# ekinakyurek/Long-Term-Recurrent-Convolutional-NN

Measured on AMD Instinct MI355X. Metric: training images/sec (VGG16+LSTM, COCO, batch 256) at 1/2/4/8 MI355X, higher is better.
Workload: dtype bf16

## Files before the change

### long-term-recurrent-convolutional-nn_amd/csrc/gemm.h

```cpp
#pragma once
#include <hip/hip_runtime.h>
#include <stdint.h>

enum { GEMM_A_PLAIN = 0, GEMM_A_CONV3 = 1 };
enum { GEMM_OUT_PLAIN = 0, GEMM_OUT_CONV = 1, GEMM_OUT_POOL = 2, GEMM_OUT_LSTM_FWD = 3, GEMM_OUT_LSTM_BWD = 4, GEMM_OUT_SMAX_TOPK = 5,
       GEMM_OUT_SMAX_GUMBEL = 6, GEMM_OUT_SMAX_PICK = 7 };

enum { SMAX_KC = 6, SMAX_REC = 16 };
enum { SMAX_MAX_NREC = 256 };
struct SmaxEpi {
    float *part;
    int nrec;
    float temp;
    uint32_t key0, key1;
    int current, S;
    const int32_t *tgt;
};

struct LstmEpi {
    int H;
    int64_t ld_a, ld_h;
    const float *Gx;
    const float *c_prev;
    const int *c_prev_idx;
    const float *c_new;
    float *c_out;
    void *acts;
    void *h_new;
    int gx_bcast;
    const int *gx_idx;
    float *h_f32;
    const float *dh_ext;
    float *dc;
    void *dz_out;
};
enum { GEMM_T_F32 = 0, GEMM_T_BF16 = 1, GEMM_T_F8 = 2 };

struct GemmArgs {
    int dtype;
    const void *A;
    int64_t lda;
    const void *B;
    int64_t ldb;
    void *C;
    int64_t ldc;
    int M, N, K;
    const float *bias;
    const float *scale;
    int c_f32;
    int beta;
    int c_is_zero;
    int relu;
    int a_mode, out_mode;
    int H, W, Cin;
    unsigned inv_w2, inv_h2;
    int wg_cap;
    LstmEpi lstm;
    SmaxEpi smax;
    int cfg_pref;
    int free_cus;
    int bg_cus;
    int *tile_ctr;
    unsigned long long *stamps;
    int splitk_forced;
    int splitk_no_reduce;
    int deterministic;
    int dbg;
    const void *zero_page;
    void *ws;
    size_t ws_bytes;
};

constexpr int kBgMinRows = 256, kBgMaxRows = 512;
inline bool bg_row_window(int rows) { return rows >= kBgMinRows && rows <= kBgMaxRows; }

hipError_t launch_gemm(hipStream_t stream, const GemmArgs &g);
hipError_t launch_gemm_nt(hipStream_t stream, const GemmArgs &g);

void gemm_debug_note_route(const char *route, int cfg);
const char *gemm_debug_last_route();

bool gemm_glds_eligible(const GemmArgs &g);
hipError_t launch_gemm_glds(hipStream_t stream, const GemmArgs &g);
int64_t gemm_glds_blocks(const GemmArgs &g);

int gemm_8p_config(const GemmArgs &g, int64_t *blocks);
int gemm_8p_splitk(const GemmArgs &g, int64_t *blocks);
hipError_t launch_gemm_8p(hipStream_t stream, const GemmArgs &g, int splitk = 1);
hipError_t launch_splitk_reduce(hipStream_t stream, const GemmArgs &g, int splits);

bool gemm_skinny_eligible(const GemmArgs &g);
hipError_t launch_gemm_skinny(hipStream_t stream, const GemmArgs &g);

bool conv64_eligible(int dtype, int Cin, int Cout, int H, int W);
hipError_t launch_conv64(hipStream_t stream, const void *in, const void *w, const float *bias, void *out, int N, int H, int W, int Cout,
                         int relu, int pool, const void *zero_page, float f8_inv_scale = 0.0f, int wg_cap = 0, unsigned long long *stamps = nullptr);
hipError_t launch_conv64_fused11(hipStream_t stream, const void *img16, const void *w11, const float *b11, const void *w,
                                 const float *bias, void *out, int N, int S, const void *zero_page, int wg_cap = 0, unsigned long long *stamps = nullptr);
hipError_t launch_conv64f(hipStream_t stream, const void *img16, const void *w11, const void *w, const float *bias, void *out, int N, int S,
                          const void *zero_page, int wg_cap = 0, unsigned long long *stamps = nullptr);
```

### long-term-recurrent-convolutional-nn_amd/csrc/gemm_8p.hip

```cpp
#include <type_traits>

#include "common.h"
#include "gemm.h"
#include "knob.h"
#include "philox.h"

namespace {

typedef __attribute__((address_space(3))) void lds_void;
typedef const __attribute__((address_space(1))) void glb_void;
typedef float f32x4v __attribute__((ext_vector_type(4)));

template <int N> __device__ __forceinline__ void wait_vmcnt() { asm volatile("s_waitcnt vmcnt(%0)" ::"n"(N) : "memory"); }
__device__ __forceinline__ void wait_lgkm0() { asm volatile("s_waitcnt lgkmcnt(0)" ::: "memory"); }

struct KStep {
    int tap, koff, kb;
};

template <int I, int N, class F> __device__ __forceinline__ void static_for(F &&f) {
    if constexpr (I < N) {
        f(std::integral_constant<int, I>{});
        static_for<I + 1, N>(f);
    }
}
template <int OFF> __device__ __forceinline__ uint4 lds_read16(unsigned addr) {
    uint4 r;
    asm volatile("ds_read_b128 %0, %1 offset:%2" : "=v"(r) : "v"(addr), "n"(OFF) : "memory");
    return r;
}

typedef int i32x8v __attribute__((ext_vector_type(8)));
__device__ __forceinline__ i32x8v pack8(const uint4 &lo, const uint4 &hi) {
    return i32x8v{(int)lo.x, (int)lo.y, (int)lo.z, (int)lo.w, (int)hi.x, (int)hi.y, (int)hi.z, (int)hi.w};
}
__device__ __forceinline__ unsigned pack_fp8x4(float a, float b, float c, float d) {
    a = fminf(fmaxf(a, -448.f), 448.f); b = fminf(fmaxf(b, -448.f), 448.f);
    c = fminf(fmaxf(c, -448.f), 448.f); d = fminf(fmaxf(d, -448.f), 448.f);
    unsigned w = 0;
    w = __builtin_amdgcn_cvt_pk_fp8_f32(a, b, w, false);
    w = __builtin_amdgcn_cvt_pk_fp8_f32(c, d, w, true);
    return w;
}

__device__ __forceinline__ float relu_bits(float x, int lo) {
    const int b = __builtin_bit_cast(int, x);
    return __builtin_bit_cast(float, b > lo ? b : lo);
}
__device__ __forceinline__ float sigm8p(float x) { return 1.0f / (1.0f + expf(-x)); }

template <int APW, int BPW> struct TileAddr {
    int m0, n0;
    unsigned a_voff[2][APW];
    unsigned a_mask[2][APW];
    unsigned b_voff[2][BPW];
};

template <int WM, int WN, int MT, int NT, int AMODE, bool SWAP, bool F8, int EPI = 0>
__device__ __forceinline__ bool gemm8p_tile(const GemmArgs &g, unsigned char *smem, const int tile, const int ntiles_xy, const int next_tile,
                                            TileAddr<WM * (2 * MT * 16) / 128, WN * (2 * NT * 16) / 128> &ta, const bool pre) {
    constexpr int ES = F8 ? 1 : 2;
    constexpr int KE = 128 / ES;
    static_assert(WM * WN == 8, "8 waves");
    constexpr int QM = MT * 16, QN = NT * 16;
    constexpr int WTM = 2 * QM, WTN = 2 * QN;
    constexpr int BM = WM * WTM, BN = WN * WTN;
    constexpr int A_BYTES = BM * 128, B_BYTES = BN * 128, BUF = A_BYTES + B_BYTES;
    constexpr int APW = BM / 128, BPW = BN / 128;
    static_assert(APW >= 1 && BPW >= 1 && APW * 128 == BM && BPW * 128 == BN, "tile must be a multiple of 128");
    constexpr int CPR = BN / 8;
    static_assert(CPR >= 16, "epilogue swizzle needs >= 16 chunks per row");
    const int tid = threadIdx.x, lane = tid & 63;
    const int wave = __builtin_amdgcn_readfirstlane(tid >> 6);
    const int wr = wave / WN, wc = wave % WN;
    const int grp = wave >> 2;
    auto stamp = [&](int k) {
        if (g.stamps && tid == 0) g.stamps[(size_t)tile * 8 + k] = k >= 6 ? __builtin_amdgcn_s_memrealtime() : __builtin_amdgcn_s_memtime();
    };
    stamp(7);
    stamp(0);
    const int M = g.M, N = g.N;
    const int tiles_n = (N + BN - 1) / BN;

    constexpr unsigned OOB = 0xFFFFFFFFu, NREC = 0xFFFFFF00u;
    const unsigned conv_back = (AMODE == GEMM_A_CONV3) ? (unsigned)((g.W + 1) * g.Cin * ES) : 0u;
    const unsigned char *Abase = reinterpret_cast<const unsigned char *>(g.A) - conv_back;
    const unsigned char *Bbase = reinterpret_cast<const unsigned char *>(g.B);
    auto rsrc_of = [](const unsigned char *base, bool live) {
        return __builtin_amdgcn_make_buffer_rsrc(const_cast<unsigned char *>(base), 0, live ? NREC : 0u, 0x00020000);
    };

    const int kpt = (AMODE == GEMM_A_CONV3) ? g.Cin / KE : g.K / KE;
    const int KT_all = (AMODE == GEMM_A_CONV3) ? 9 * kpt : kpt;
    const int kbeg = (int)((int64_t)KT_all * blockIdx.y / gridDim.y);
    const int KT = (int)((int64_t)KT_all * (blockIdx.y + 1) / gridDim.y) - kbeg;

    auto a_piece_row = [&](int hf, int j) {
        const int hr = (wave * APW + j) * 8;
        return (hr / QM) * WTM + hf * QM + (hr % QM);
    };
    auto b_piece_row = [&](int hf, int j) {
        const int hr = (wave * BPW + j) * 8;
        return (hr / QN) * WTN + hf * QN + (hr % QN);
    };
    auto setup = [&](int t, TileAddr<APW, BPW> &o) {
        int bid = t;
        {
            const int nwg = ntiles_xy, q = nwg >> 3, r = nwg & 7, xcd = bid & 7;
            bid = (xcd < r ? xcd * (q + 1) : r * (q + 1) + (xcd - r) * q) + (bid >> 3);
        }
        const int nt = bid % tiles_n, mt = bid / tiles_n;
        o.m0 = mt * BM;
        o.n0 = nt * BN;
#pragma unroll
        for (int hf = 0; hf < 2; ++hf) {
#pragma unroll
            for (int j = 0; j < APW; ++j) {
                const int row = a_piece_row(hf, j) + (lane >> 3);
                const int m = o.m0 + row;
                const int src_chunk = (lane & 7) ^ ((row >> 1) & 7);
                o.a_voff[hf][j] = OOB;
                o.a_mask[hf][j] = ~0u;
                if (m < M) {
                    if (AMODE == GEMM_A_CONV3) {
                        const PixDecode p = decode_pixel_fast(m, g.H, g.W, g.inv_w2, g.inv_h2);
                        o.a_voff[hf][j] = (unsigned)((uint64_t)((p.n * g.H + p.y) * g.W + p.x) * (uint64_t)(g.Cin * ES) + src_chunk * 16);
                        o.a_mask[hf][j] = (p.y == 0 ? 0x007u : 0u) | (p.y == g.H - 1 ? 0x1C0u : 0u) | (p.x == 0 ? 0x049u : 0u) |
                                          (p.x == g.W - 1 ? 0x124u : 0u) | ~0x1FFu;
                    } else {
                        o.a_voff[hf][j] = (unsigned)((uint64_t)m * (uint64_t)(g.lda * ES) + src_chunk * 16);
                    }
                }
            }
#pragma unroll
            for (int j = 0; j < BPW; ++j) {
                const int row = b_piece_row(hf, j) + (lane >> 3);
                const int n = o.n0 + row;
                const int src_chunk = (lane & 7) ^ ((row >> 1) & 7);
                o.b_voff[hf][j] = n < N ? (unsigned)((uint64_t)n * (uint64_t)(g.ldb * ES) + src_chunk * 16) : OOB;
            }
        }
    };

    auto kstep_of = [&](int kt) {
        KStep k;
        if (AMODE == GEMM_A_CONV3) {
            const int slice = kt / 9;
            k.tap = kt - 9 * slice;
            const int kh = k.tap / 3, kw = k.tap - 3 * kh;
            k.koff = ((kh - 1) * g.W + (kw - 1)) * g.Cin + slice * KE;
            k.kb = k.tap * g.Cin + slice * KE;
        } else {
            k.tap = 0;
            k.koff = kt * KE;
            k.kb = k.koff;
        }
        return k;
    };
    const unsigned char *Aflat = reinterpret_cast<const unsigned char *>(g.A);
    const unsigned char *Zp = reinterpret_cast<const unsigned char *>(g.zero_page) + (lane & 7) * 16;
    auto stage_a = [&](int buf, int hf, const KStep &k, bool live) {
        if constexpr (AMODE == GEMM_A_CONV3) {
            const __amdgpu_buffer_rsrc_t rs = rsrc_of(Abase, live);
            const int soff = (int)(conv_back + (unsigned)(k.koff * ES));
#pragma unroll
            for (int j = 0; j < APW; ++j) {
                const unsigned vo = ta.a_voff[hf][j] | (unsigned)__builtin_amdgcn_sbfe((int)ta.a_mask[hf][j], k.tap, 1);
                __builtin_amdgcn_raw_ptr_buffer_load_lds(rs, (lds_void *)(smem + buf * BUF + a_piece_row(hf, j) * 128), 16, (int)vo, soff, 0, 0);
            }
        } else {
#pragma unroll
            for (int j = 0; j < APW; ++j) {
                const bool ok = live && ta.a_voff[hf][j] != OOB;
                const unsigned char *src = ok ? Aflat + ((int64_t)ta.a_voff[hf][j] + (int64_t)k.koff * ES) : Zp;
                __builtin_amdgcn_global_load_lds((glb_void *)src, (lds_void *)(smem + buf * BUF + a_piece_row(hf, j) * 128), 16, 0, 0);
            }
        }
    };
    auto stage_b = [&](int buf, int hf, const KStep &k, bool live) {
        if constexpr (AMODE == GEMM_A_CONV3) {
            const __amdgpu_buffer_rsrc_t rs = rsrc_of(Bbase, live);
            const int soff = k.kb * ES;
#pragma unroll
            for (int j = 0; j < BPW; ++j)
                __builtin_amdgcn_raw_ptr_buffer_load_lds(rs, (lds_void *)(smem + buf * BUF + A_BYTES + b_piece_row(hf, j) * 128), 16,
                                                         (int)ta.b_voff[hf][j], soff, 0, 0);
        } else {
#pragma unroll
            for (int j = 0; j < BPW; ++j) {
                const bool ok = live && ta.b_voff[hf][j] != OOB;
                const unsigned char *src = ok ? Bbase + ((int64_t)ta.b_voff[hf][j] + (int64_t)k.kb * ES) : Zp;
                __builtin_amdgcn_global_load_lds((glb_void *)src, (lds_void *)(smem + buf * BUF + A_BYTES + b_piece_row(hf, j) * 128), 16, 0, 0);
            }
        }
    };

    unsigned fa[2], fb[2];
#pragma unroll
    for (int s = 0; s < 2; ++s) {
        const int kch = F8 ? 2 * (lane >> 4) + s : s * 4 + (lane >> 4);
        const unsigned fo = (lane & 15) * 128 + ((kch ^ (((lane & 15) >> 1) & 7)) << 4);
        const unsigned base = (unsigned)(uintptr_t)(__attribute__((address_space(3))) unsigned char *)smem;
        fa[s] = base + (wr * WTM) * 128 + fo;
        fb[s] = base + A_BYTES + (wc * WTN) * 128 + fo;
    }

    auto issue_first = [&]() {
        const KStep k0 = kstep_of(kbeg);
        stage_a(0, 0, k0, true);
        stage_b(0, 0, k0, true);
        stage_b(0, 1, k0, true);
        stage_a(0, 1, k0, true);
    };
    if (!pre) {
        setup(tile, ta);
        issue_first();
    }
    stamp(1);
    const int m0 = ta.m0, n0 = ta.n0;

    const bool staged = !F8 && EPI == 0 && !g.c_f32 && !g.beta && gridDim.y == 1 && (g.ldc % 8) == 0 && ((uintptr_t)g.C & 15) == 0 &&
                        (N % 8) == 0 && (!SWAP || (N % 4) == 0);
    const bool bias_init = staged && g.bias != nullptr;
    f32x4v acc[2][MT][2][NT];
#pragma unroll
    for (int b = 0; b < 2; ++b)
#pragma unroll
        for (int n = 0; n < NT; ++n) {
            f32x4v bv = f32x4v{0.f, 0.f, 0.f, 0.f};
            if (bias_init) {
                if constexpr (SWAP) {
                    const int col = n0 + wc * WTN + b * QN + n * 16 + (lane >> 4) * 4;
                    if (col < N) bv = *reinterpret_cast<const f32x4v *>(g.bias + col);
                } else {
                    const int col = n0 + wc * WTN + b * QN + n * 16 + (lane & 15);
                    const float sb = col < N ? g.bias[col] : 0.0f;
                    bv = f32x4v{sb, sb, sb, sb};
                }
            }
#pragma unroll
            for (int a = 0; a < 2; ++a)
#pragma unroll
                for (int i = 0; i < MT; ++i) acc[a][i][b][n] = bv;
        }

    uint4 af[MT][2], bf0[NT][2], bf1[NT][2];
    auto read_a = [&](int buf, auto mhc) {
        constexpr int mh = decltype(mhc)::value;
        const unsigned a0 = fa[0] + buf * BUF, a1 = fa[1] + buf * BUF;
        static_for<0, MT>([&](auto ic) {
            constexpr int i = decltype(ic)::value;
            af[i][0] = lds_read16<(mh * QM + i * 16) * 128>(a0);
            af[i][1] = lds_read16<(mh * QM + i * 16) * 128>(a1);
        });
    };
    auto read_b = [&](int buf, auto nhc, uint4 (&bf)[NT][2]) {
        constexpr int nh = decltype(nhc)::value;
        const unsigned b0 = fb[0] + buf * BUF, b1 = fb[1] + buf * BUF;
        static_for<0, NT>([&](auto ic) {
            constexpr int n = decltype(ic)::value;
            bf[n][0] = lds_read16<(nh * QN + n * 16) * 128>(b0);
            bf[n][1] = lds_read16<(nh * QN + n * 16) * 128>(b1);
        });
    };
    constexpr std::integral_constant<int, 0> I0{};
    constexpr std::integral_constant<int, 1> I1{};
#define MFMA_BODY(mh, nh, BF)                                                                                              \
    do {                                                                                                                   \
        if constexpr (F8) {                                                                                                \
            _Pragma("unroll") for (int i = 0; i < MT; ++i) _Pragma("unroll") for (int n = 0; n < NT; ++n) {                \
                const i32x8v av = pack8(af[i][0], af[i][1]);                                                               \
                const i32x8v bv = pack8(BF[n][0], BF[n][1]);                                                               \
                acc[mh][i][nh][n] = SWAP ? __builtin_amdgcn_mfma_scale_f32_16x16x128_f8f6f4(bv, av, acc[mh][i][nh][n], 0, 0, 0, 0, 0, 0) \
                                         : __builtin_amdgcn_mfma_scale_f32_16x16x128_f8f6f4(av, bv, acc[mh][i][nh][n], 0, 0, 0, 0, 0, 0); \
            }                                                                                                              \
        } else {                                                                                                           \
            _Pragma("unroll") for (int s = 0; s < 2; ++s) _Pragma("unroll") for (int i = 0; i < MT; ++i) _Pragma("unroll") for (int n = 0; \
                                                                                                                   n < NT; ++n) { \
                const bf16x8 av = __builtin_bit_cast(bf16x8, af[i][s]);                                                    \
                const bf16x8 bv = __builtin_bit_cast(bf16x8, BF[n][s]);                                                    \
                acc[mh][i][nh][n] = SWAP ? __builtin_amdgcn_mfma_f32_16x16x32_bf16(bv, av, acc[mh][i][nh][n], 0, 0, 0)     \
                                         : __builtin_amdgcn_mfma_f32_16x16x32_bf16(av, bv, acc[mh][i][nh][n], 0, 0, 0);    \
            }                                                                                                              \
        }                                                                                                                  \
    } while (0)
#define MFMA_PAIR(mh1, nh1, BF1, mh2, nh2, BF2, LGKM1)                                                                     \
    do {                                                                                                                   \
        __builtin_amdgcn_s_barrier();                                                                                      \
        asm volatile("s_waitcnt lgkmcnt(%0)" ::"n"(LGKM1) : "memory");                                                     \
        __builtin_amdgcn_sched_barrier(0);                                                                                 \
        __builtin_amdgcn_s_setprio(1);                                                                                     \
        MFMA_BODY(mh1, nh1, BF1);                                                                                          \
        __builtin_amdgcn_sched_barrier(0);                                                                                 \
        wait_lgkm0();                                                                                                      \
        __builtin_amdgcn_sched_barrier(0);                                                                                 \
        MFMA_BODY(mh2, nh2, BF2);                                                                                          \
        __builtin_amdgcn_s_setprio(0);                                                                                     \
        __builtin_amdgcn_sched_barrier(0);                                                                                 \
        __builtin_amdgcn_s_barrier();                                                                                      \
    } while (0)

    {
        wait_vmcnt<0>();
        __builtin_amdgcn_s_barrier();
        stamp(2);
        if (grp == 1) __builtin_amdgcn_s_barrier();
    }
    KStep kn = kstep_of(kbeg + (KT > 1 ? 1 : 0));
    auto k_tile = [&](int t, auto curc) {
        constexpr int cur = decltype(curc)::value, nxt = cur ^ 1;
        const bool live1 = t + 1 < KT;
        read_a(cur, I0);
        read_b(cur, I0, bf0);
        read_b(cur, I1, bf1);
        stage_a(nxt, 0, kn, live1);
        stage_b(nxt, 0, kn, live1);
        stage_b(nxt, 1, kn, live1);
        wait_vmcnt<APW + 2 * BPW>();
        MFMA_PAIR(0, 0, bf0, 0, 1, bf1, 2 * NT);
        read_a(cur, I1);
        stage_a(nxt, 1, kn, live1);
        wait_vmcnt<APW>();
        MFMA_PAIR(1, 1, bf1, 1, 0, bf0, 0);
        kn = kstep_of(kbeg + (t + 2 < KT ? t + 2 : 0));
    };
    for (int t = 0; t < KT; t += 2) {
        k_tile(t, I0);
        if (t + 1 < KT) k_tile(t + 1, I1);
    }
#undef MFMA_PAIR
#undef MFMA_BODY
    if (grp == 0) __builtin_amdgcn_s_barrier();
    wait_vmcnt<0>();
    __builtin_amdgcn_s_barrier();
    stamp(3);

    const int l15 = lane & 15, lq = lane >> 4;
    if constexpr (EPI == GEMM_OUT_LSTM_FWD || EPI == GEMM_OUT_LSTM_BWD) {
        constexpr int CPRF = BN / 4;
        static_assert(CPRF == 32, "LSTM epilogues are built for the 256 x 128 tile");
        const LstmEpi &e = g.lstm;
        const int H = e.H;
        typedef __bf16 bf16x4e __attribute__((ext_vector_type(4)));
        const int q8 = tid & 7, r64 = tid >> 3;
        const int u0 = (n0 >> 2) + 4 * q8;
        const bool uok = u0 < H;
        [[maybe_unused]] f32x4v cpv[4], gxv[4][4];
        if constexpr (EPI == GEMM_OUT_LSTM_FWD) {
            const f32x4v z4 = f32x4v{0.f, 0.f, 0.f, 0.f};
            if (e.gx_bcast) {
#pragma unroll
                for (int gt = 0; gt < 4; ++gt) gxv[0][gt] = uok ? *reinterpret_cast<const f32x4v *>(e.Gx + (int64_t)gt * H + u0) : z4;
            }
#pragma unroll
            for (int j = 0; j < 4; ++j) {
                const int row = m0 + r64 + 64 * j;
                const bool ok = uok && row < M;
                const int64_t grow = (ok && e.gx_idx) ? e.gx_idx[row] : row;
                if (ok && e.c_prev) {
                    const int64_t prow = e.c_prev_idx ? e.c_prev_idx[row] : row;
                    cpv[j] = *reinterpret_cast<const f32x4v *>(e.c_prev + prow * H + u0);
                } else {
                    cpv[j] = z4;
                }
#pragma unroll
                for (int gt = 0; gt < 4; ++gt) {
                    if (!e.gx_bcast) gxv[j][gt] = ok ? *reinterpret_cast<const f32x4v *>(e.Gx + grow * 4 * H + (int64_t)gt * H + u0) : z4;
                    else if (j > 0) gxv[j][gt] = gxv[0][gt];
                }
            }
        }
#pragma unroll
        for (int mh = 0; mh < 2; ++mh)
#pragma unroll
            for (int i = 0; i < MT; ++i)
#pragma unroll
                for (int nh = 0; nh < 2; ++nh)
#pragma unroll
                    for (int n = 0; n < NT; ++n) {
                        const int lrow = wr * WTM + mh * QM + i * 16 + l15;
                        const int ch = (wc * WTN + nh * QN + n * 16 + 4 * lq) >> 2;
                        *reinterpret_cast<f32x4v *>(smem + lrow * (BN * 4) + ((ch ^ (lrow & 31)) << 4)) = acc[mh][i][nh][n];
                    }
        __syncthreads();
        if constexpr (EPI == GEMM_OUT_LSTM_FWD) {
#pragma unroll
            for (int j = 0; j < 4; ++j) {
                const int lrow = r64 + 64 * j, row = m0 + lrow;
                if (!uok || row >= M) continue;
                f32x4v fv, iv, ov, gv, cn, hv;
#pragma unroll
                for (int k = 0; k < 4; ++k) {
                    const f32x4v a = *reinterpret_cast<const f32x4v *>(smem + lrow * (BN * 4) + (((4 * q8 + k) ^ (lrow & 31)) << 4));
                    const float f = sigm8p(a[0] + gxv[j][0][k]), in = sigm8p(a[1] + gxv[j][1][k]), o = sigm8p(a[2] + gxv[j][2][k]),
                                chg = tanhf(a[3] + gxv[j][3][k]);
                    const float c = cpv[j][k] * f + in * chg;
                    fv[k] = f; iv[k] = in; ov[k] = o; gv[k] = chg; cn[k] = c;
                    hv[k] = o * tanhf(c);
                }
                if (e.acts) {
                    bf16_t *ac = reinterpret_cast<bf16_t *>(e.acts) + (int64_t)row * e.ld_a + u0;
                    bf16x4e t;
#pragma unroll
                    for (int k = 0; k < 4; ++k) t[k] = (bf16_t)fv[k];
                    *reinterpret_cast<bf16x4e *>(ac) = t;
#pragma unroll
                    for (int k = 0; k < 4; ++k) t[k] = (bf16_t)iv[k];
                    *reinterpret_cast<bf16x4e *>(ac + H) = t;
#pragma unroll
                    for (int k = 0; k < 4; ++k) t[k] = (bf16_t)ov[k];
                    *reinterpret_cast<bf16x4e *>(ac + 2 * H) = t;
#pragma unroll
                    for (int k = 0; k < 4; ++k) t[k] = (bf16_t)gv[k];
                    *reinterpret_cast<bf16x4e *>(ac + 3 * H) = t;
                }
                *reinterpret_cast<f32x4v *>(e.c_out + (int64_t)row * H + u0) = cn;
                bf16x4e hb;
#pragma unroll
                for (int k = 0; k < 4; ++k) hb[k] = (bf16_t)hv[k];
                *reinterpret_cast<bf16x4e *>(reinterpret_cast<bf16_t *>(e.h_new) + (int64_t)row * e.ld_h + u0) = hb;
                if (e.h_f32) *reinterpret_cast<f32x4v *>(e.h_f32 + (int64_t)row * H + u0) = hv;
            }
            return false;
        }
        for (int idx = tid; idx < BM * CPRF; idx += 512) {
            const int lrow = idx / CPRF, ch = idx - lrow * CPRF;
            const int row = m0 + lrow, col0 = n0 + 4 * ch;
            if (row >= M || col0 >= N) continue;
            const f32x4v a = *reinterpret_cast<const f32x4v *>(smem + lrow * (BN * 4) + ((ch ^ (lrow & 31)) << 4));
            {
                const int u = col0;
                const int64_t o = (int64_t)row * H + u;
                const f32x4v dhe = *reinterpret_cast<const f32x4v *>(e.dh_ext + o), cn = *reinterpret_cast<const f32x4v *>(e.c_new + o),
                             dci = *reinterpret_cast<const f32x4v *>(e.dc + o);
                f32x4v cp = f32x4v{0.f, 0.f, 0.f, 0.f};
                if (e.c_prev) cp = *reinterpret_cast<const f32x4v *>(e.c_prev + o);
                const bf16_t *ac = reinterpret_cast<const bf16_t *>(e.acts) + (int64_t)row * e.ld_a + u;
                const bf16x4e fv = *reinterpret_cast<const bf16x4e *>(ac), iv = *reinterpret_cast<const bf16x4e *>(ac + H),
                              ov = *reinterpret_cast<const bf16x4e *>(ac + 2 * H), gv = *reinterpret_cast<const bf16x4e *>(ac + 3 * H);
                bf16x4e zf, zi, zo, zg;
                f32x4v dco;
#pragma unroll
                for (int r = 0; r < 4; ++r) {
                    const float dh = a[r] + dhe[r];
                    const float f = (float)fv[r], in = (float)iv[r], og = (float)ov[r], gg = (float)gv[r];
                    const float tc = tanhf(cn[r]);
                    const float dov = dh * tc;
                    const float dcv = dci[r] + dh * og * (1.0f - tc * tc);
                    zf[r] = (bf16_t)(dcv * cp[r] * f * (1.0f - f));
                    zi[r] = (bf16_t)(dcv * gg * in * (1.0f - in));
                    zo[r] = (bf16_t)(dov * og * (1.0f - og));
                    zg[r] = (bf16_t)(dcv * in * (1.0f - gg * gg));
                    dco[r] = dcv * f;
                }
                bf16_t *z = reinterpret_cast<bf16_t *>(e.dz_out) + (int64_t)row * e.ld_a + u;
                *reinterpret_cast<bf16x4e *>(z) = zf;
                *reinterpret_cast<bf16x4e *>(z + H) = zi;
                *reinterpret_cast<bf16x4e *>(z + 2 * H) = zo;
                *reinterpret_cast<bf16x4e *>(z + 3 * H) = zg;
                *reinterpret_cast<f32x4v *>(e.dc + o) = dco;
            }
        }
        return false;
    }
    if constexpr (EPI == GEMM_OUT_SMAX_TOPK || EPI == GEMM_OUT_SMAX_GUMBEL || EPI == GEMM_OUT_SMAX_PICK) {
        static_assert(BM == 256 && BN == 256 && SWAP && !F8, "built for the 256 x 256 tile");
        constexpr bool GUM = EPI == GEMM_OUT_SMAX_GUMBEL, PICK = EPI == GEMM_OUT_SMAX_PICK;
        const SmaxEpi &e = g.smax;
        const int srow = tid >> 1, part = tid & 1;
        float m_run = -INFINITY, s_run = 0.0f;
        float tv[SMAX_KC];
        int ti[SMAX_KC];
#pragma unroll
        for (int k = 0; k < SMAX_KC; ++k) {
            tv[k] = -INFINITY;
            ti[k] = 0x7FFFFFFF;
        }
        float gs = -INFINITY, gz = -INFINITY;
        int gc = 0x7FFFFFFF;
        [[maybe_unused]] int tcol = -1;
        [[maybe_unused]] float zt = -INFINITY;
        if constexpr (PICK) tcol = m0 + srow < M ? e.tgt[m0 + srow] : -1;
#pragma unroll
        for (int h = 0; h < 2; ++h) {
            if ((wc >> 1) == h) {
#pragma unroll
                for (int nh = 0; nh < 2; ++nh)
#pragma unroll
                    for (int n = 0; n < NT; ++n) {
                        const int lcol = (wc & 1) * WTN + nh * QN + n * 16 + 4 * lq;
                        const int col = n0 + h * 128 + lcol;
                        f32x4v bias = f32x4v{0.f, 0.f, 0.f, 0.f};
                        const bool cok = col < N;
                        if (g.bias && cok) bias = *reinterpret_cast<const f32x4v *>(g.bias + col);
#pragma unroll
                        for (int mh = 0; mh < 2; ++mh)
#pragma unroll
                            for (int i = 0; i < MT; ++i) {
                                const int lrow = wr * WTM + mh * QM + i * 16 + l15;
                                f32x4v a = acc[mh][i][nh][n] + bias;
                                if (!cok) a = f32x4v{-INFINITY, -INFINITY, -INFINITY, -INFINITY};
                                *reinterpret_cast<f32x4v *>(smem + lrow * 512 + (((lcol >> 2) ^ (lrow & 31)) << 4)) = a;
                            }
                    }
            }
            __syncthreads();
            const unsigned char *rowp = smem + srow * 512;
            const int sw = srow & 31;
            auto cid = [&](int c) { return (c & 7) | (part << 3) | ((c >> 3) << 4); };
            float cm = -INFINITY;
#pragma unroll
            for (int c = 0; c < 16; ++c) {
                const f32x4v x = *reinterpret_cast<const f32x4v *>(rowp + ((cid(c) ^ sw) << 4));
                cm = fmaxf(cm, fmaxf(fmaxf(x[0], x[1]), fmaxf(x[2], x[3])));
            }
            if (cm > m_run) {
                s_run *= __expf(m_run - cm);
                m_run = cm;
            }
            if (cm != -INFINITY) {
                float s4[4] = {0.f, 0.f, 0.f, 0.f};
#pragma unroll 4
                for (int c = 0; c < 16; ++c) {
                    const f32x4v x = *reinterpret_cast<const f32x4v *>(rowp + ((cid(c) ^ sw) << 4));
#pragma unroll
                    for (int k = 0; k < 4; ++k) s4[k] += __expf(x[k] - m_run);
                    if constexpr (GUM) {
                        const float thr = e.temp > 0.0f ? m_run - GUMBEL_PRUNE * e.temp : m_run;
                        if (fmaxf(fmaxf(x[0], x[1]), fmaxf(x[2], x[3])) >= thr) {
                            const int cbase = n0 + h * 128 + 4 * cid(c);
                            if (e.temp > 0.0f) {
                                const int grow = m0 + srow, gii = grow / e.S;
                                const Philox4 rnd = philox4x32_10((uint32_t)(cbase >> 2), (uint32_t)e.current, (uint32_t)(grow - gii * e.S), (uint32_t)gii,
                                                                  e.key0, e.key1);
#pragma unroll
                                for (int k = 0; k < 4; ++k)
                                    if (x[k] >= thr) {
                                        const float sc = x[k] / e.temp + gumbel_of(rnd.x[k]);
                                        if (sc > gs) { gs = sc; gc = cbase + k; gz = x[k]; }
                                    }
                            } else {
#pragma unroll
                                for (int k = 0; k < 4; ++k)
                                    if (x[k] > gs) { gs = x[k]; gc = cbase + k; gz = x[k]; }
                            }
                        }
                    } else if constexpr (PICK) {
                        const int d = tcol - (n0 + h * 128 + 4 * cid(c));
                        if ((unsigned)d < 4u) zt = d == 0 ? x[0] : d == 1 ? x[1] : d == 2 ? x[2] : x[3];
                    } else if (fmaxf(fmaxf(x[0], x[1]), fmaxf(x[2], x[3])) > tv[SMAX_KC - 1]) {
                        const int cbase = n0 + h * 128 + 4 * cid(c);
#pragma unroll
                        for (int k = 0; k < 4; ++k) {
                            const float xv = x[k];
                            if (xv > tv[SMAX_KC - 1]) {
                                float cv = xv;
                                int ci = cbase + k;
                                bool ins = false;
#pragma unroll
                                for (int j = 0; j < SMAX_KC; ++j) {
                                    ins = ins || cv > tv[j];
                                    if (ins) {
                                        const float ov = tv[j];
                                        const int oi = ti[j];
                                        tv[j] = cv; ti[j] = ci;
                                        cv = ov; ci = oi;
                                    }
                                }
                            }
                        }
                    }
                }
                s_run += (s4[0] + s4[1]) + (s4[2] + s4[3]);
            }
            __syncthreads();
        }
        const int row = m0 + srow;
        if (PICK && row < M) {
            float *rec = e.part + ((int64_t)row * e.nrec + (2 * (n0 >> 8) + part)) * SMAX_REC;
            *reinterpret_cast<f32x4v *>(rec) = f32x4v{m_run, s_run, zt, 0.0f};
        } else if (GUM && row < M) {
            float *rec = e.part + ((int64_t)row * e.nrec + (2 * (n0 >> 8) + part)) * SMAX_REC;
            *reinterpret_cast<f32x4v *>(rec) = f32x4v{m_run, s_run, gs, __int_as_float(gc)};
            rec[4] = gz;
        } else if (row < M) {
            float *rec = e.part + ((int64_t)row * e.nrec + (2 * (n0 >> 8) + part)) * SMAX_REC;
            *reinterpret_cast<f32x4v *>(rec) = f32x4v{m_run, s_run, tv[0], tv[1]};
            *reinterpret_cast<f32x4v *>(rec + 4) = f32x4v{tv[2], tv[3], tv[4], tv[5]};
            *reinterpret_cast<f32x4v *>(rec + 8) = f32x4v{__int_as_float(ti[0]), __int_as_float(ti[1]), __int_as_float(ti[2]), __int_as_float(ti[3])};
            *reinterpret_cast<f32x4v *>(rec + 12) = f32x4v{__int_as_float(ti[4]), __int_as_float(ti[5]), 0.0f, 0.0f};
        }
        return false;
    }
    if constexpr (F8) {
        constexpr int CSTR = BN, CPR8 = BN / 16, RPL = 256 / BN > 1 ? 256 / BN : 1;
        auto swz = [](int r) { return (r / RPL) & (CPR8 - 1); };
        if (!SWAP) {
            float scp[2][NT], biasp[2][NT];
#pragma unroll
            for (int nh = 0; nh < 2; ++nh)
#pragma unroll
                for (int n = 0; n < NT; ++n) {
                    const int col = n0 + wc * WTN + nh * QN + n * 16 + l15;
                    scp[nh][n] = (g.scale && col < N) ? g.scale[col] : 1.0f;
                    biasp[nh][n] = (g.bias && col < N) ? g.bias[col] : 0.0f;
                }
#pragma unroll
            for (int mh = 0; mh < 2; ++mh)
#pragma unroll
                for (int i = 0; i < MT; ++i)
#pragma unroll
                    for (int nh = 0; nh < 2; ++nh)
#pragma unroll
                        for (int n = 0; n < NT; ++n) {
                            const int lcol = wc * WTN + nh * QN + n * 16 + l15;
                            const float sc = scp[nh][n];
                            const float bias = biasp[nh][n];
                            const f32x4v a = acc[mh][i][nh][n];
                            float v = fmaxf(fmaxf(a[0], a[1]), fmaxf(a[2], a[3])) * sc + bias;
                            if (g.relu) v = fmaxf(v, 0.0f);
                            const int prow = (wr * WTM + mh * QM + i * 16) / 4 + lq;
                            const int pos = ((lcol >> 4) ^ swz(prow)) * 16 + (lcol & 15);
                            smem[prow * CSTR + pos] = (unsigned char)(pack_fp8x4(v, v, 0.f, 0.f) & 0xFF);
                        }
        } else {
            f32x4v biasv[2][NT], scv[2][NT];
#pragma unroll
            for (int nh = 0; nh < 2; ++nh)
#pragma unroll
                for (int n = 0; n < NT; ++n) {
                    const int col = n0 + wc * WTN + nh * QN + n * 16 + lq * 4;
                    biasv[nh][n] = f32x4v{0.f, 0.f, 0.f, 0.f};
                    scv[nh][n] = f32x4v{1.f, 1.f, 1.f, 1.f};
                    if (g.bias && col < N) biasv[nh][n] = *reinterpret_cast<const f32x4v *>(g.bias + col);
                    if (g.scale && col < N) scv[nh][n] = *reinterpret_cast<const f32x4v *>(g.scale + col);
                }
#pragma unroll
            for (int nh = 0; nh < 2; ++nh)
#pragma unroll
                for (int n = 0; n < NT; ++n) {
                    const int lcol = wc * WTN + nh * QN + n * 16 + lq * 4;
                    const f32x4v bias = biasv[nh][n], sc = scv[nh][n];
#pragma unroll
                    for (int mh = 0; mh < 2; ++mh)
#pragma unroll
                        for (int i = 0; i < MT; ++i) {
                            f32x4v a = acc[mh][i][nh][n] * sc + bias;
                            if (g.relu) {
#pragma unroll
                                for (int r = 0; r < 4; ++r) a[r] = fmaxf(a[r], 0.0f);
                            }
                            const int lrow = wr * WTM + mh * QM + i * 16 + l15;
                            const int pos = ((lcol >> 4) ^ swz(lrow)) * 16 + (lcol & 15);
                            *reinterpret_cast<unsigned *>(smem + lrow * CSTR + pos) = pack_fp8x4(a[0], a[1], a[2], a[3]);
                        }
                }
        }
        __syncthreads();
        const int rows_out = SWAP ? BM : BM / 4;
        unsigned char *C8 = reinterpret_cast<unsigned char *>(g.C);
        for (int idx = tid; idx < rows_out * CPR8; idx += 512) {
            const int lrow = idx / CPR8, ch = idx - lrow * CPR8;
            const int col = n0 + ch * 16;
            if (col >= N) continue;
            int64_t off;
            if (!SWAP) {
                const int prow = (m0 >> 2) + lrow;
                if (prow >= (M >> 2)) continue;
                off = (int64_t)prow * g.ldc + col;
            } else {
                const int row = m0 + lrow;
                if (row >= M) continue;
                if (g.out_mode == GEMM_OUT_CONV) {
                    const PixDecode p = decode_pixel_fast(row, g.H, g.W, g.inv_w2, g.inv_h2);
                    off = (((int64_t)p.n * g.H + p.y) * g.W + p.x) * g.ldc + col;
                } else {
                    off = (int64_t)row * g.ldc + col;
                }
            }
            typedef unsigned u32x4 __attribute__((ext_vector_type(4)));
            __builtin_nontemporal_store(*reinterpret_cast<const u32x4 *>(smem + lrow * CSTR + ((ch ^ swz(lrow)) << 4)),
                                        reinterpret_cast<u32x4 *>(C8 + off));
        }
        return false;
    }
    if (staged) {
        constexpr int CSTR = BN * 2;
        const int relu_lo = g.relu ? 0 : (int)0x80000000;
        unsigned char *const cst = smem + (SWAP ? 0 : BUF);
        static_assert(SWAP || (BM / 4) * BN * 2 <= BUF, "pooled tile fits one ring buffer");
        typedef short s16x2 __attribute__((ext_vector_type(2)));
        const s16x2 relu_lo2 = g.relu ? s16x2{0, 0} : s16x2{(short)0x8000, (short)0x8000};
        if (!SWAP) {
#pragma unroll
            for (int mh = 0; mh < 2; ++mh)
#pragma unroll
                for (int i = 0; i < MT; ++i)
#pragma unroll
                    for (int nh = 0; nh < 2; ++nh)
#pragma unroll
                        for (int n = 0; n < NT; ++n) {
                            const int lcol = wc * WTN + nh * QN + n * 16 + l15;
                            const f32x4v a = acc[mh][i][nh][n];
                            const float v = relu_bits(fmaxf(fmaxf(a[0], a[1]), fmaxf(a[2], a[3])), relu_lo);
                            const int prow = (wr * WTM + mh * QM + i * 16) / 4 + lq;
                            const int pos = ((lcol >> 3) ^ (prow & 15)) * 16 + (lcol & 7) * 2;
                            *reinterpret_cast<bf16_t *>(cst + prow * CSTR + pos) = (bf16_t)v;
                        }
        } else {
#pragma unroll
            for (int nh = 0; nh < 2; ++nh)
#pragma unroll
                for (int n = 0; n < NT; ++n) {
                    const int lcol = wc * WTN + nh * QN + n * 16 + lq * 4;
#pragma unroll
                    for (int mh = 0; mh < 2; ++mh)
#pragma unroll
                        for (int i = 0; i < MT; ++i) {
                            const f32x4v a = acc[mh][i][nh][n];
                            typedef short s16x4 __attribute__((ext_vector_type(4)));
                            typedef __bf16 bf16x4c __attribute__((ext_vector_type(4)));
                            uint2 pk = __builtin_bit_cast(uint2, __builtin_convertvector(a, bf16x4c));
                            asm volatile("" : "+v"(pk.x), "+v"(pk.y));
                            const s16x2 r0 = __builtin_elementwise_max(__builtin_bit_cast(s16x2, pk.x), relu_lo2),
                                        r1 = __builtin_elementwise_max(__builtin_bit_cast(s16x2, pk.y), relu_lo2);
                            const int lrow = wr * WTM + mh * QM + i * 16 + l15;
                            const int pos = ((lcol >> 3) ^ (lrow & 15)) * 16 + (lcol & 7) * 2;
                            *reinterpret_cast<s16x4 *>(cst + lrow * CSTR + pos) = s16x4{r0[0], r0[1], r1[0], r1[1]};
                        }
                }
        }
        __syncthreads();
        stamp(4);
        constexpr int rows_out = SWAP ? BM : BM / 4;
        bf16_t *Cb = reinterpret_cast<bf16_t *>(g.C);
        typedef unsigned u32x4 __attribute__((ext_vector_type(4)));
        constexpr int ITER = rows_out * CPR / 512;
        static_assert(ITER * 512 == rows_out * CPR, "whole passes of the workgroup");
        const bool early = !SWAP && next_tile >= 0;
        int tid_e = tid;
        asm volatile("" : "+v"(tid_e));
        auto store_chunk = [&](int k, const u32x4 &v) {
            const int idx = tid_e + 512 * k;
            const int lrow = idx / CPR, ch = idx - lrow * CPR;
            const int col = n0 + ch * 8;
            if (col >= N) return;
            int64_t off;
            if (!SWAP) {
                const int prow = (m0 >> 2) + lrow;
                if (prow >= (M >> 2)) return;
                off = (int64_t)prow * g.ldc + col;
            } else {
                const int row = m0 + lrow;
                if (row >= M) return;
                if (g.out_mode == GEMM_OUT_CONV) {
                    const PixDecode p = decode_pixel_fast(row, g.H, g.W, g.inv_w2, g.inv_h2);
                    off = (((int64_t)p.n * g.H + p.y) * g.W + p.x) * g.ldc + col;
                } else {
                    off = (int64_t)row * g.ldc + col;
                }
            }
            __builtin_nontemporal_store(v, reinterpret_cast<u32x4 *>(Cb + off));
        };
        auto read_chunk = [&](int k) {
            const int idx = tid_e + 512 * k, lrow = idx / CPR, ch = idx - lrow * CPR;
            return *reinterpret_cast<const u32x4 *>(cst + lrow * CSTR + ((ch ^ (lrow & 15)) << 4));
        };
        if (early) {
            setup(next_tile, ta);
            issue_first();
        }
        constexpr int HB = ITER > 4 ? 4 : ITER;
        static_assert(ITER % HB == 0, "whole batches");
        for (int kb = 0; kb < ITER; kb += HB) {
            u32x4 chunk[HB];
#pragma unroll
            for (int k = 0; k < HB; ++k) chunk[k] = read_chunk(kb + k);
#pragma unroll
            for (int k = 0; k < HB; ++k) store_chunk(kb + k, chunk[k]);
        }
        stamp(5);
        stamp(6);
        return early;
    }

    if (gridDim.y > 1) {
        if constexpr (SWAP) {
            float *slab = reinterpret_cast<float *>(g.ws) + (size_t)blockIdx.y * M * N;
#pragma unroll
            for (int mh = 0; mh < 2; ++mh)
#pragma unroll
                for (int i = 0; i < MT; ++i)
#pragma unroll
                    for (int nh = 0; nh < 2; ++nh)
#pragma unroll
                        for (int n = 0; n < NT; ++n) {
                            const int row = m0 + wr * WTM + mh * QM + i * 16 + l15, col0 = n0 + wc * WTN + nh * QN + n * 16 + 4 * lq;
                            if (row < M && col0 < N) *reinterpret_cast<f32x4v *>(slab + (size_t)row * N + col0) = acc[mh][i][nh][n];
                        }
        }
        return false;
    }

    bool early_b = false;
    if (next_tile >= 0 && gridDim.y == 1 && !(g.dbg & 16)) {
        setup(next_tile, ta);
        issue_first();
        early_b = true;
    }
#pragma unroll
    for (int mh = 0; mh < 2; ++mh)
#pragma unroll
        for (int i = 0; i < MT; ++i)
#pragma unroll
            for (int nh = 0; nh < 2; ++nh)
#pragma unroll
                for (int n = 0; n < NT; ++n) {
                    const f32x4v a = acc[mh][i][nh][n];
                    const int rb = m0 + wr * WTM + mh * QM + i * 16, cb = n0 + wc * WTN + nh * QN + n * 16;
                    if (!SWAP) {
                        const int col = cb + l15, row = rb + 4 * lq;
                        if (col >= N || row >= M) continue;
                        float v = fmaxf(fmaxf(a[0], a[1]), fmaxf(a[2], a[3])) + (g.bias ? g.bias[col] : 0.0f);
                        if (g.relu) v = fmaxf(v, 0.0f);
                        const int64_t off = (int64_t)(row >> 2) * g.ldc + col;
                        if (g.c_f32)
                            reinterpret_cast<float *>(g.C)[off] = v;
                        else
                            reinterpret_cast<bf16_t *>(g.C)[off] = (bf16_t)v;
                        continue;
                    }
                    const int row = rb + l15, col0 = cb + 4 * lq;
                    if (row >= M || col0 >= N) continue;
                    int64_t off0;
                    if (g.out_mode == GEMM_OUT_CONV) {
                        const PixDecode p = decode_pixel_fast(row, g.H, g.W, g.inv_w2, g.inv_h2);
                        off0 = (((int64_t)p.n * g.H + p.y) * g.W + p.x) * g.ldc + col0;
                    } else {
                        off0 = (int64_t)row * g.ldc + col0;
                    }
                    const bool vec = g.c_f32 && col0 + 3 < N && ((off0 & 3) == 0) && (((uintptr_t)g.C & 15) == 0);
                    if (vec) {
                        f32x4v v = a;
                        if (g.bias) v += *reinterpret_cast<const f32x4v *>(g.bias + col0);
                        float *c = reinterpret_cast<float *>(g.C) + off0;
                        if (g.beta) v += *reinterpret_cast<const f32x4v *>(c);
                        if (g.relu) {
#pragma unroll
                            for (int r = 0; r < 4; ++r) v[r] = fmaxf(v[r], 0.0f);
                        }
                        *reinterpret_cast<f32x4v *>(c) = v;
                        continue;
                    }
#pragma unroll
                    for (int r = 0; r < 4; ++r) {
                        if (col0 + r >= N) continue;
                        float v = a[r] + (g.bias ? g.bias[col0 + r] : 0.0f);
                        if (g.c_f32) {
                            float *c = reinterpret_cast<float *>(g.C) + off0 + r;
                            if (g.beta) v += *c;
                            if (g.relu) v = fmaxf(v, 0.0f);
                            *c = v;
                        } else {
                            bf16_t *c = reinterpret_cast<bf16_t *>(g.C) + off0 + r;
                            if (g.beta) v += (float)*c;
                            if (g.relu) v = fmaxf(v, 0.0f);
                            *c = (bf16_t)v;
                        }
                    }
                }
    return early_b;
}

template <int WM, int WN, int MT, int NT, int AMODE, bool SWAP, bool F8, int EPI = 0>
__global__ __launch_bounds__(512) void gemm8p_kernel(const GemmArgs g) {
    extern __shared__ __attribute__((aligned(16))) unsigned char smem[];
    constexpr int BM = WM * MT * 32, BN = WN * NT * 32;
    const int ntiles = ((g.M + BM - 1) / BM) * ((g.N + BN - 1) / BN);
    TileAddr<BM / 128, BN / 128> ta;
    if (g.tile_ctr == nullptr || gridDim.y > 1) {
        bool pre = false;
        for (int tile = blockIdx.x; tile < ntiles; tile += gridDim.x) {
            const int next = (!(g.dbg & 8) && tile + (int)gridDim.x < ntiles) ? tile + (int)gridDim.x : -1;
            pre = gemm8p_tile<WM, WN, MT, NT, AMODE, SWAP, F8, EPI>(g, smem, tile, ntiles, next, ta, pre);
            if (!pre && tile + (int)gridDim.x < ntiles) __syncthreads();
        }
        return;
    }
    auto pull = [&]() -> int {
        const int q0 = blockIdx.x & 7;
        for (int k = 0; k < 8; ++k) {
            const int q = (q0 + k) & 7;
            const int nq = (ntiles - q + 7) >> 3;
            if (nq <= 0) continue;
            const int i = atomicAdd(g.tile_ctr + q, 1);
            if (i < nq) return 8 * i + q;
        }
        return -1;
    };
    int *slot = g.tile_ctr + 8 + 2 * blockIdx.x;
    const int lane = threadIdx.x & 63;
    auto publish = [&](int *p) {
        const int old = __hip_atomic_exchange(p, pull(), __ATOMIC_RELAXED, __HIP_MEMORY_SCOPE_AGENT);
        asm volatile("s_waitcnt vmcnt(0)" ::"v"(old) : "memory");
    };
    auto fetch = [&](int *p) -> int {
        int t = 0;
        if (lane == 0) t = __hip_atomic_fetch_add(p, 0, __ATOMIC_RELAXED, __HIP_MEMORY_SCOPE_AGENT);
        return __builtin_amdgcn_readfirstlane(t);
    };
    int par = 0;
    if (threadIdx.x == 0) publish(slot);
    __syncthreads();
    int tile = fetch(slot);
    while (tile >= 0) {
        par ^= 1;
        if (threadIdx.x == 0) publish(slot + par);
        (void)gemm8p_tile<WM, WN, MT, NT, AMODE, SWAP, F8, EPI>(g, smem, tile, ntiles, -1, ta, false);
        __syncthreads();
        tile = fetch(slot + par);
    }
}

template <int WM, int WN, int MT, int NT, int AMODE, bool SWAP, bool F8 = false, int EPI = 0> hipError_t launch_one(hipStream_t s, const GemmArgs &g, int splitk) {
    constexpr int BM = WM * MT * 32, BN = WN * NT * 32;
    constexpr int ring = 2 * (BM + BN) * 128, ctile = EPI == GEMM_OUT_SMAX_TOPK || EPI == GEMM_OUT_SMAX_GUMBEL || EPI == GEMM_OUT_SMAX_PICK ? BM * 512 : BM * BN * (EPI ? 4 : 2);
    constexpr int lds = ring > ctile ? ring : ctile;
    static_assert(lds <= 160 * 1024, "LDS budget");
    static LdsAttrMask attr_done{0};
    auto kern = gemm8p_kernel<WM, WN, MT, NT, AMODE, SWAP, F8, EPI>;
    if (hipError_t e = set_max_lds(reinterpret_cast<const void *>(kern), lds, attr_done); e != hipSuccess) return e;
    const int64_t blocks = (int64_t)cdiv(g.M, BM) * cdiv(g.N, BN);
    if (blocks <= 0 || blocks > 0x7FFFFFFF) return hipErrorInvalidValue;
    int64_t grid = blocks;
    if (g.wg_cap >= 8 && grid > g.wg_cap && g.tile_ctr && splitk == 1) {
        grid = g.wg_cap & ~7;
    } else if (g.wg_cap >= 8 && grid > g.wg_cap) {
        const int64_t cap = g.wg_cap & ~7, rounds = (blocks + cap - 1) / cap;
        grid = (((blocks + rounds - 1) / rounds) + 7) & ~7ll;
        if (grid > cap) grid = cap;
    }
    hipLaunchKernelGGL(kern, dim3((unsigned)grid, (unsigned)splitk), dim3(512), lds, s, g);
    return hipGetLastError();
}

template <int AMODE, bool SWAP, bool F8 = false> hipError_t dispatch(hipStream_t s, const GemmArgs &g, int cfg, int splitk) {
    switch (cfg) {
        case 0: return launch_one<2, 4, 4, 2, AMODE, SWAP, F8>(s, g, splitk);
        case 1: return launch_one<4, 2, 2, 2, AMODE, SWAP, F8>(s, g, splitk);
        case 2: return launch_one<4, 2, 4, 2, AMODE, SWAP, F8>(s, g, splitk);
        default: return hipErrorInvalidValue;
    }
}

}

static bool gemm_8p_f8_ok(const GemmArgs &g) {
    if (g.dtype != GEMM_T_F8 || !g.zero_page || g.a_mode != GEMM_A_CONV3 || g.out_mode == GEMM_OUT_PLAIN) return false;
    if (((uintptr_t)g.A & 15) || ((uintptr_t)g.B & 15) || ((uintptr_t)g.C & 15) || (g.ldb % 16) || (g.ldc % 16) || (g.N % 16)) return false;
    if (g.Cin % 128 || g.K != 9 * g.Cin || (g.H & 1) || (g.W & 1) || g.H <= 0 || g.W <= 0 || g.M % (g.H * g.W)) return false;
    if ((int64_t)g.M * g.Cin >= (1ll << 31) || (int64_t)g.N * g.ldb >= (1ll << 31)) return false;
    if (g.c_f32 || g.beta || (g.out_mode == GEMM_OUT_POOL && (g.M & 3))) return false;
    return true;
}

int gemm_8p_config(const GemmArgs &g, int64_t *blocks) {
    if (g.dtype == GEMM_T_F8) {
        if (!gemm_8p_f8_ok(g)) return -1;
    } else if (g.dtype != GEMM_T_BF16 || !gemm_glds_eligible(g)) {
        return -1;
    }
    {
        const int64_t es = g.dtype == GEMM_T_F8 ? 1 : 2;
        const int64_t a_bytes = (g.a_mode == GEMM_A_CONV3 ? (int64_t)g.M * g.Cin + (int64_t)(g.W + 1) * g.Cin : (int64_t)g.M * g.lda) * es;
        if (a_bytes >= 0xFFFF0000ll || (int64_t)g.N * g.ldb * es >= 0xFFFF0000ll) return -1;
    }
    if ((g.M < 256 && g.dtype != GEMM_T_F8) || g.N < 128) return -1;
    const int ke = g.dtype == GEMM_T_F8 ? 128 : 64;
    const int kt = (g.a_mode == GEMM_A_CONV3) ? 9 * (g.Cin / ke) : g.K / ke;
    if (kt < 2) return -1;
    const int64_t b0 = (int64_t)cdiv(g.M, 256) * cdiv(g.N, 256), b1 = (int64_t)cdiv(g.M, 256) * cdiv(g.N, 128);
    int cfg = (g.N > 128 && (b0 >= 200 || g.N % 256 == 0 || g.N > 384)) ? 0 : 1;
    if (cfg == 0 && ((b0 < 200 && b1 >= 200) || (b0 < 128 && b1 >= 128))) cfg = 1;
    if (g.cfg_pref == 2 && g.N >= 128) cfg = 1;
    if (g.free_cus > 0 && g.N > 128 && b0 <= g.free_cus && b1 > g.free_cus) cfg = 0;
    *blocks = cfg == 0 ? b0 : b1;
    if (cfg == 1 && g.N <= 128 && cdiv(g.M, 512) >= 400) {
        cfg = 2;
        *blocks = cdiv(g.M, 512);
    }
    return cfg;
}

int gemm_8p_splitk(const GemmArgs &g, int64_t *blocks) {
    if (g.dtype != GEMM_T_BF16 || !gemm_glds_eligible(g) || g.M < 256 || g.N < 128 || (g.N % 4)) return 0;
    const bool conv = g.a_mode == GEMM_A_CONV3 && g.out_mode != GEMM_OUT_PLAIN && !g.c_f32 && !g.beta && (g.M & 3) == 0;
    if (!conv && (g.a_mode != GEMM_A_PLAIN || g.out_mode != GEMM_OUT_PLAIN)) return 0;
    if (!g.ws || (g.ldc % 4) || ((uintptr_t)g.C & 15)) return 0;
    const int kt = conv ? 9 * (g.Cin / 64) : g.K / 64;
    const int64_t b1 = (int64_t)cdiv(g.M, 256) * cdiv(g.N, 128);
    int s = (int)((g.free_cus > 0 ? g.free_cus : 256) / b1);
    const int min_slice = conv ? 12 : 8;
    if (s > kt / min_slice) s = kt / min_slice;
    if (s > 16) s = 16;
    while (s >= 2 && (size_t)s * g.M * g.N * sizeof(float) > g.ws_bytes) --s;
    if (s < 2) return 0;
    *blocks = b1 * s;
    return s;
}

namespace {
template <typename T> __global__ void splitk_reduce_kernel(const float *ws, int S, int M, int N, const float *bias, int beta, int relu,
                                                            void *C, int64_t ldc, int c_f32) {
    const int n4 = N >> 2;
    const int64_t total = (int64_t)M * n4;
    for (int64_t idx = (int64_t)blockIdx.x * blockDim.x + threadIdx.x; idx < total; idx += (int64_t)gridDim.x * blockDim.x) {
        const int m = (int)(idx / n4), c4 = (int)(idx - (int64_t)m * n4) * 4;
        f32x4v v = *reinterpret_cast<const f32x4v *>(ws + (size_t)m * N + c4);
        for (int s = 1; s < S; ++s) v += *reinterpret_cast<const f32x4v *>(ws + ((size_t)s * M + m) * N + c4);
        if (bias) v += *reinterpret_cast<const f32x4v *>(bias + c4);
        if (c_f32) {
            float *c = reinterpret_cast<float *>(C) + (int64_t)m * ldc + c4;
            if (beta) v += *reinterpret_cast<const f32x4v *>(c);
            if (relu)
                for (int r = 0; r < 4; ++r) v[r] = fmaxf(v[r], 0.0f);
            *reinterpret_cast<f32x4v *>(c) = v;
        } else {
            T *c = reinterpret_cast<T *>(C) + (int64_t)m * ldc + c4;
            for (int r = 0; r < 4; ++r) {
                float x = v[r] + (beta ? to_f32(c[r]) : 0.0f);
                if (relu) x = fmaxf(x, 0.0f);
                c[r] = from_f32<T>(x);
            }
        }
    }
}
__global__ void splitk_reduce_conv_kernel(const float *ws, int S, int M, int N, const float *bias, int relu, bf16_t *C, int64_t ldc, int H,
                                          int W, int pool) {
    typedef __bf16 bf16x4 __attribute__((ext_vector_type(4)));
    const int n4 = N >> 2;
    const int64_t total = (int64_t)(M >> 2) * n4;
    for (int64_t idx = (int64_t)blockIdx.x * blockDim.x + threadIdx.x; idx < total; idx += (int64_t)gridDim.x * blockDim.x) {
        const int w = (int)(idx / n4), c4 = (int)(idx - (int64_t)w * n4) * 4;
        const f32x4v b = bias ? *reinterpret_cast<const f32x4v *>(bias + c4) : f32x4v{0.f, 0.f, 0.f, 0.f};
        f32x4v best = f32x4v{0.f, 0.f, 0.f, 0.f};
#pragma unroll
        for (int sub = 0; sub < 4; ++sub) {
            const int m = 4 * w + sub;
            f32x4v v = *reinterpret_cast<const f32x4v *>(ws + (size_t)m * N + c4);
            for (int s = 1; s < S; ++s) v += *reinterpret_cast<const f32x4v *>(ws + ((size_t)s * M + m) * N + c4);
            v += b;
            if (relu)
                for (int r = 0; r < 4; ++r) v[r] = fmaxf(v[r], 0.0f);
            if (pool) {
                if (sub == 0) best = v;
                else
                    for (int r = 0; r < 4; ++r) best[r] = fmaxf(best[r], v[r]);
            } else {
                const PixDecode p = decode_pixel(m, H, W);
                bf16_t *c = C + (((int64_t)p.n * H + p.y) * W + p.x) * ldc + c4;
                bf16x4 o;
                for (int r = 0; r < 4; ++r) o[r] = (bf16_t)v[r];
                *reinterpret_cast<bf16x4 *>(c) = o;
            }
        }
        if (pool) {
            bf16x4 o;
            for (int r = 0; r < 4; ++r) o[r] = (bf16_t)best[r];
            *reinterpret_cast<bf16x4 *>(C + (int64_t)w * ldc + c4) = o;
        }
    }
}
}

hipError_t launch_splitk_reduce(hipStream_t stream, const GemmArgs &g, int splits) {
    if (g.a_mode == GEMM_A_CONV3) {
        const int64_t total = (int64_t)(g.M >> 2) * (g.N >> 2);
        const int grid = (int)((total + 255) / 256 > 2048 ? 2048 : (total + 255) / 256);
        hipLaunchKernelGGL(splitk_reduce_conv_kernel, dim3(grid), dim3(256), 0, stream, reinterpret_cast<const float *>(g.ws), splits, g.M, g.N,
                           g.bias, g.relu, reinterpret_cast<bf16_t *>(g.C), g.ldc, g.H, g.W, g.out_mode == GEMM_OUT_POOL ? 1 : 0);
        return hipGetLastError();
    }
    const int64_t total = (int64_t)g.M * (g.N >> 2);
    const int grid = (int)((total + 255) / 256 > 2048 ? 2048 : (total + 255) / 256);
    hipLaunchKernelGGL(splitk_reduce_kernel<bf16_t>, dim3(grid), dim3(256), 0, stream, reinterpret_cast<const float *>(g.ws), splits, g.M,
                       g.N, g.bias, g.beta, g.relu, g.C, g.ldc, g.c_f32);
    return hipGetLastError();
}

hipError_t launch_gemm_8p(hipStream_t stream, const GemmArgs &g0, int splitk) {
    GemmArgs g = g0;
    const int epi = g0.out_mode;
    if (epi == GEMM_OUT_LSTM_FWD || epi == GEMM_OUT_LSTM_BWD) {
        g.out_mode = GEMM_OUT_PLAIN;
        g.cfg_pref = 2;
    }
    if (epi == GEMM_OUT_SMAX_TOPK || epi == GEMM_OUT_SMAX_GUMBEL || epi == GEMM_OUT_SMAX_PICK) {
        static_assert(SMAX_KC == 6 && SMAX_REC == 16, "record layout of the epilogue's four 16-byte stores");
        g.out_mode = GEMM_OUT_PLAIN;
        g.c_f32 = 1;
        g.C = g.smax.part;
        g.ldc = g.N;
        if (g.dtype != GEMM_T_BF16 || g.a_mode != GEMM_A_PLAIN || splitk > 1 || (g.N & 3) || g.M < 256 || g.N < 256 || !g.smax.part ||
            g.smax.nrec != 2 * cdiv(g.N, 256) || ((uintptr_t)g.smax.part & 15) || (g.bias && ((uintptr_t)g.bias & 15)) || !gemm_glds_eligible(g))
            return hipErrorInvalidValue;
        g.dbg = knob_int("LRCN_DBG", 0);
        g.inv_w2 = g.inv_h2 = 0;
        gemm_debug_note_route(nullptr, 0);
        if (epi == GEMM_OUT_SMAX_GUMBEL) {
            if (g.smax.S < 1 || !(g.smax.temp >= 0.0f)) return hipErrorInvalidValue;
            return launch_one<2, 4, 4, 2, GEMM_A_PLAIN, true, false, GEMM_OUT_SMAX_GUMBEL>(stream, g, 1);
        }
        if (epi == GEMM_OUT_SMAX_PICK) {
            if (!g.smax.tgt) return hipErrorInvalidValue;
            return launch_one<2, 4, 4, 2, GEMM_A_PLAIN, true, false, GEMM_OUT_SMAX_PICK>(stream, g, 1);
        }
        return launch_one<2, 4, 4, 2, GEMM_A_PLAIN, true, false, GEMM_OUT_SMAX_TOPK>(stream, g, 1);
    }
    g.dbg = knob_int("LRCN_DBG", 0);
    g.inv_w2 = g.inv_h2 = 0;
    if ((g.a_mode == GEMM_A_CONV3 || g.out_mode == GEMM_OUT_CONV || g.out_mode == GEMM_OUT_POOL) && g.W >= 4 && g.H >= 4) {
        const uint64_t wmax = (uint64_t)((g.M + 511) >> 2) + 128, dmax = (uint64_t)(g.W > g.H ? g.W : g.H) >> 1;
        if (wmax * dmax < (1ull << 32)) {
            g.inv_w2 = fastdiv_inv((unsigned)g.W >> 1);
            g.inv_h2 = fastdiv_inv((unsigned)g.H >> 1);
        }
    }
    int64_t blocks = 0;
    int cfg = gemm_8p_config(g, &blocks);
    if (cfg < 0) return hipErrorInvalidValue;
    gemm_debug_note_route(nullptr, splitk > 1 ? splitk : cfg);
    if (epi == GEMM_OUT_LSTM_FWD || epi == GEMM_OUT_LSTM_BWD) {
        if (g.dtype != GEMM_T_BF16 || g.a_mode != GEMM_A_PLAIN || splitk > 1 || cfg != 1 || (g.N & 3) ||
            (!g.lstm.acts && epi == GEMM_OUT_LSTM_BWD) || g.lstm.H < 1 || (g.lstm.H & 3) || (g.lstm.ld_a & 3))
            return hipErrorInvalidValue;
        return epi == GEMM_OUT_LSTM_FWD ? launch_one<4, 2, 2, 2, GEMM_A_PLAIN, true, false, GEMM_OUT_LSTM_FWD>(stream, g, 1)
                                               : launch_one<4, 2, 2, 2, GEMM_A_PLAIN, true, false, GEMM_OUT_LSTM_BWD>(stream, g, 1);
    }
    if (splitk > 1) {
        if (!g.splitk_forced && gemm_8p_splitk(g, &blocks) != splitk) return hipErrorInvalidValue;
        hipError_t e = g.a_mode == GEMM_A_CONV3 ? dispatch<GEMM_A_CONV3, true>(stream, g, 1, splitk) : dispatch<GEMM_A_PLAIN, true>(stream, g, 1, splitk);
        if (e != hipSuccess) return e;
        if (g.splitk_no_reduce) return hipSuccess;
        return launch_splitk_reduce(stream, g, splitk);
    } else {
        splitk = 1;
    }
    const bool swap = g.out_mode != GEMM_OUT_POOL;
    if (g.dtype == GEMM_T_F8)
        return swap ? dispatch<GEMM_A_CONV3, true, true>(stream, g, cfg, 1) : dispatch<GEMM_A_CONV3, false, true>(stream, g, cfg, 1);
    if (g.a_mode == GEMM_A_CONV3)
        return swap ? dispatch<GEMM_A_CONV3, true>(stream, g, cfg, splitk) : dispatch<GEMM_A_CONV3, false>(stream, g, cfg, splitk);
    return swap ? dispatch<GEMM_A_PLAIN, true>(stream, g, cfg, splitk) : dispatch<GEMM_A_PLAIN, false>(stream, g, cfg, splitk);
}
```

### long-term-recurrent-convolutional-nn_amd/csrc/gemm_route.hip

```cpp
#include <cstdio>

#include "common.h"
#include "gemm.h"
#include "knob.h"

static thread_local char g_route[48] = "";
static thread_local int g_route_cfg = -1;
void gemm_debug_note_route(const char *route, int cfg) {
    if (route) {
        if (cfg >= 0) snprintf(g_route, sizeof(g_route), "%s:%d", route, cfg);
        else snprintf(g_route, sizeof(g_route), "%s", route);
    } else {
        g_route_cfg = cfg;
    }
}
const char *gemm_debug_last_route() { return g_route; }

constexpr int kFree8pMinPct = 75;
constexpr int kBgMinCols = 512;

static int64_t blocks_8p(const GemmArgs &g) {
    int64_t b = 0;
    return gemm_8p_config(g, &b) >= 0 ? b : 0;
}
static GemmArgs bg_args(const GemmArgs &g) {
    GemmArgs h = g;
    h.cfg_pref = 2;
    return h;
}
static bool bg_fits(const GemmArgs &g) {
    if (g.bg_cus <= 0 || g.a_mode != GEMM_A_PLAIN || !bg_row_window(g.M) || g.N < kBgMinCols) return false;
    const int64_t b = blocks_8p(bg_args(g));
    return b > 0 && b <= 2 * g.bg_cus;
}

static hipError_t launch_gemm_routed(hipStream_t stream, const GemmArgs &g, const char **route) {
    if (g.dtype == GEMM_T_F8) {
        if (g.M <= 0 || !g.A || !g.B || !g.C || blocks_8p(g) == 0) return hipErrorInvalidValue;
        *route = "8p-f8";
        return launch_gemm_8p(stream, g);
    }
    if (g.M <= 0 || g.N <= 0 || g.K <= 0 || !g.A || !g.B || !g.C) return hipErrorInvalidValue;
    const char glds = knob_char("LRCN_GLDS"), p8 = knob_char("LRCN_8P");
    const bool glds_on = glds != '0', p8_on = glds_on && p8 != '0';
    const bool skinny_ok = glds_on && !knob_off("LRCN_SKINNY") && gemm_skinny_eligible(g);
    const bool splitk_on = p8_on && !knob_off("LRCN_8P_SPLITK");
    const int splitk_min = knob_int("LRCN_8P_SPLITK_MIN", 96);

    const int64_t b8 = p8_on ? blocks_8p(g) : 0;
    const bool fills_free = g.free_cus > 0 && b8 * 100 >= (int64_t)g.free_cus * kFree8pMinPct && b8 <= g.free_cus;
    if (b8 > 0 && (p8 == 'f' || b8 >= 128 || fills_free)) { *route = "8p"; return launch_gemm_8p(stream, g); }
    if (p8_on && bg_fits(g)) { *route = "8p-bg"; return launch_gemm_8p(stream, bg_args(g)); }
    if (p8_on && skinny_ok && g.M <= 128) { *route = "skinny"; return launch_gemm_skinny(stream, g); }
    int64_t bsk = 0;
    const int sk = splitk_on ? gemm_8p_splitk(g, &bsk) : 0;
    if (sk > 1 && bsk >= splitk_min) { *route = "8p-splitk"; return launch_gemm_8p(stream, g, sk); }
    const int64_t bgl = glds_on && gemm_glds_eligible(g) ? gemm_glds_blocks(g) : 0;
    if (bgl > 0 && (glds == 'f' || bgl >= 96)) { *route = "glds"; return launch_gemm_glds(stream, g); }
    if (skinny_ok) { *route = "skinny-last"; return launch_gemm_skinny(stream, g); }
    if (bgl >= 16) { *route = "glds-small"; return launch_gemm_glds(stream, g); }

    const int ce = g.dtype == GEMM_T_BF16 ? 8 : 4;
    if (((uintptr_t)g.A & 15) || ((uintptr_t)g.B & 15) || (g.ldb % ce)) return hipErrorInvalidValue;
    if (g.a_mode == GEMM_A_CONV3) {
        const int bk = g.dtype == GEMM_T_BF16 ? 64 : 32;
        if (g.Cin % bk || g.K != 9 * g.Cin || (g.H & 1) || (g.W & 1) || g.M % (g.H * g.W)) return hipErrorInvalidValue;
    } else if (g.lda % ce) {
        return hipErrorInvalidValue;
    }
    if (g.out_mode != GEMM_OUT_PLAIN && ((g.H & 1) || (g.W & 1) || g.H <= 0 || g.W <= 0)) return hipErrorInvalidValue;
    if (g.out_mode == GEMM_OUT_POOL && (g.beta || (g.M & 3))) return hipErrorInvalidValue;
    *route = "gemm_nt";
    return launch_gemm_nt(stream, g);
}

hipError_t launch_gemm(hipStream_t stream, const GemmArgs &g) {
    const char *route = "?";
    g_route_cfg = -1;
    const hipError_t e = launch_gemm_routed(stream, g, &route);
    gemm_debug_note_route(route, g_route_cfg);
    return e;
}
```

### long-term-recurrent-convolutional-nn_amd/csrc/lrcn_api.hip

```cpp
#include <algorithm>
#include <cmath>
#include <cstring>

#include "ctx.h"
#include "../../include/lrcn_varlen.h"

static thread_local std::string g_create_err;
using namespace lrcn_impl;

constexpr int kBgWgsPerFreeCu = 4;

int lrcn_impl::gemm(lrcn_ctx *c, int dtype, const void *A, int64_t lda, const void *B, int64_t ldb, void *C, int64_t ldc, int M, int N,
         int K, const float *bias, bool c_f32, bool beta, bool relu, bool c_is_zero, bool on_wg_stream) {
    GemmArgs g{};
    g.dtype = dtype;
    g.A = A;
    g.lda = lda;
    g.B = B;
    g.ldb = ldb;
    g.C = C;
    g.ldc = ldc;
    g.M = M;
    g.N = N;
    g.K = gemm_k(dtype, lda, ldb, K);
    g.bias = bias;
    g.c_f32 = c_f32;
    g.beta = beta;
    g.c_is_zero = c_is_zero;
    g.relu = relu;
    g.a_mode = GEMM_A_PLAIN;
    g.out_mode = GEMM_OUT_PLAIN;
    g.zero_page = c->zero_page;
    g.deterministic = c->opt_det;
    g.ws = on_wg_stream ? c->wg_ws : c->gemm_ws;
    g.ws_bytes = c->gemm_ws_bytes;
    if (!lstm_alone(c)) {
        const int free_cus = std::max(c->ncu - c->vgg_wg_cap, 0);
        if (c->cur_B < kBgMinRows) {
            g.free_cus = free_cus;
        } else {
            g.bg_cus = free_cus;
            if (free_cus >= 8) g.wg_cap = free_cus * kBgWgsPerFreeCu;
        }
    }
    hipError_t e = launch_gemm(on_wg_stream ? c->wg_stream : c->stream, g);
    if (e != hipSuccess) FAIL(c, LRCN_EHIP, "gemm M=%d N=%d K=%d: %s", M, N, K, hipGetErrorString(e));
    if (knob_char("LRCN_TRACE_ROUTES") == '1') {
        fprintf(stderr, "gemm M=%d N=%d K=%d %s-> %s\n", M, N, K, on_wg_stream ? "(wg stream) " : "", gemm_debug_last_route());
    }
    return LRCN_OK;
}

namespace {

DropSpec make_drop(const lrcn_dropout *d, int which) {
    DropSpec s{};
    s.which = which;
    if (d) {
        s.p = d->pdrop;
        s.seed = d->seed;
        s.mask = which == 1 ? d->mask1 : d->mask2;
        if (s.mask) s.p = 0.0f;
    }
    return s;
}

void ctx_sizes(const lrcn_ctx *c, int64_t sz[9]);
struct ShadowSet {
    void *W1x, *W1h, *W1xT, *W1hT, *W2x, *W2h, *W2xT, *W2hT, *Wpd, *WpT, *Wcd, *WeT, *Wod, *WoT;
};
ShadowSet cur_shadows(const lrcn_ctx *c) {
    return ShadowSet{c->W1x, c->W1h, c->W1xT, c->W1hT, c->W2x, c->W2h, c->W2xT, c->W2hT, c->Wpd, c->WpT, c->Wcd, c->WeT, c->Wod, c->WoT};
}
ShadowSet alt_shadows(const lrcn_ctx *c) {
    void *const *a = c->alt;
    return ShadowSet{a[0], a[1], a[2], a[3], a[4], a[5], a[6], a[7], a[8], a[9], a[10], a[11], a[12], a[13]};
}
void swap_shadow_sets(lrcn_ctx *c) {
    void **cur[14] = {&c->W1x, &c->W1h, &c->W1xT, &c->W1hT, &c->W2x, &c->W2h, &c->W2xT, &c->W2hT, &c->Wpd, &c->WpT, &c->Wcd, &c->WeT, &c->Wod, &c->WoT};
    for (int i = 0; i < 14; ++i) std::swap(*cur[i], c->alt[i]);
    if (c->alt_gi[0]) {
        std::swap(c->W1h_gi, c->alt_gi[0]);
        std::swap(c->W2h_gi, c->alt_gi[1]);
    }
}
int ensure_alt_shadows(lrcn_ctx *c) {
    if (c->alt[0]) return LRCN_OK;
    const size_t es = c->esz;
    const int E = c->E, H1 = c->H1, H2 = c->H2, h = c->h, V = c->V, X1 = c->X1;
    const size_t bytes[14] = {es * 4 * H1 * c->ldX1, es * 4 * H1 * c->ldH1, es * X1 * c->ld4H1, es * H1 * c->ld4H1,
                              es * 4 * H2 * c->ldH2, es * 4 * H2 * c->ldH2, es * H2 * c->ld4H2, es * H2 * c->ld4H2,
                              es * h * c->ldH1, es * H1 * c->ldh, es * h * LRCN_CNNOUT, es * V * c->ldE, es * V * c->ldH2, es * H2 * c->ldV};
    (void)E;
    for (int i = 0; i < 14; ++i) DALLOC(c, c->alt[i], bytes[i]);
    return LRCN_OK;
}
int ensure_gi_sets(lrcn_ctx *c) {
    const bool two = c->nl == 2;
    if (!c->W1h_gi) DALLOC(c, c->W1h_gi, c->esz * 4 * c->H1 * c->ldH1);
    if (two && !c->W2h_gi) DALLOC(c, c->W2h_gi, c->esz * 4 * c->H2 * c->ldH2);
    if (c->opt_fused) {
        if (!c->alt_gi[0]) DALLOC(c, c->alt_gi[0], c->esz * 4 * c->H1 * c->ldH1);
        if (two && !c->alt_gi[1]) DALLOC(c, c->alt_gi[1], c->esz * 4 * c->H2 * c->ldH2);
    }
    return LRCN_OK;
}

void plan_matrices(const lrcn_ctx *c, const float *const p[9], const ShadowSet &w, bool b, PrepPlan &plan, int only_a = -1, int only_b = -1,
                   void *const *gi = nullptr) {
    const int E = c->E, H1 = c->H1, H2 = c->H2, h = c->h, V = c->V, X1 = c->X1;
    const bool two = c->nl == 2;
    auto add = [&](int k, int R, int C, int cs, void *dA, int64_t ldA, void *dB, int64_t ldB, void *tA, int64_t ldtA, void *tB, int64_t ldtB) {
        if (only_a >= 0 && k != only_a && k != only_b) return;
        PrepDesc &d = plan.d[plan.n++];
        d = PrepDesc{};
        d.src = p[k]; d.R = R; d.C = C; d.cs = cs;
        d.dA = dA; d.ldA = ldA; d.dB = dB; d.ldB = ldB;
        d.tA = tA; d.ldtA = ldtA; d.tB = tB; d.ldtB = ldtB;
    };
    (void)E;
    auto with_gi = [&](int k, void *dst, int64_t ld, int H) {
        if (!dst || (only_a >= 0 && k != only_a && k != only_b)) return;
        PrepDesc &d = plan.d[plan.n - 1];
        d.dG = dst; d.ldG = ld; d.giH = H;
    };
    add(0, 4 * H1, X1 + H1, X1, w.W1x, c->ldX1, w.W1h, c->ldH1, b ? w.W1xT : nullptr, c->ld4H1, b ? w.W1hT : nullptr, c->ld4H1);
    with_gi(0, gi ? gi[0] : nullptr, c->ldH1, H1);
    if (two) {
        add(2, 4 * H2, 2 * H2, H2, w.W2x, c->ldH2, w.W2h, c->ldH2, b ? w.W2xT : nullptr, c->ld4H2, b ? w.W2hT : nullptr, c->ld4H2);
        with_gi(2, gi ? gi[1] : nullptr, c->ldH2, H2);
        add(4, h, H1, H1, w.Wpd, c->ldH1, nullptr, 0, b ? w.WpT : nullptr, c->ldh, nullptr, 0);
    }
    add(5, h, LRCN_CNNOUT, LRCN_CNNOUT, w.Wcd, LRCN_CNNOUT, nullptr, 0, nullptr, 0, nullptr, 0);
    add(6, E, V, V, nullptr, 0, nullptr, 0, w.WeT, c->ldE, nullptr, 0);
    add(7, V, H2, H2, w.Wod, c->ldH2, nullptr, 0, b ? w.WoT : nullptr, c->ldV, nullptr, 0);
}

const int kGradGroup[LRCN_GRAD_GROUPS][2] = {{7, 8}, {2, 3}, {4, 5}, {0, 1}, {6, 6}};

int adam_fused(lrcn_ctx *c, float *const p[9], const float *const g[9], float *const m[9], float *const v[9], int group, int step, float lr,
               float b1, float b2, float eps, hipStream_t st) {
    int r = ensure_alt_shadows(c);
    if (r) return r;
    int64_t sz[9];
    ctx_sizes(c, sz);
    PrepPlan plan{};
    const int ka = group < 0 ? -1 : kGradGroup[group][0], kb = group < 0 ? -1 : kGradGroup[group][1];
    if (c->gi_live && (r = ensure_gi_sets(c))) return r;
    plan_matrices(c, p, alt_shadows(c), true, plan, ka, kb, c->gi_live ? c->alt_gi : nullptr);
    for (int i = 0; i < plan.n; ++i) {
        PrepDesc &d = plan.d[i];
        int k = 0;
        while (k < 9 && p[k] != d.src) ++k;
        d.g = g[k]; d.m = m[k]; d.v = v[k];
    }
    for (int k : {1, 3, 8}) {
        if (sz[k] == 0 || (group >= 0 && k != ka && k != kb)) continue;
        PrepDesc &d = plan.d[plan.n++];
        d = PrepDesc{};
        d.src = p[k]; d.g = g[k]; d.m = m[k]; d.v = v[k];
        d.R = 1; d.C = (int)sz[k]; d.cs = (int)sz[k];
    }
    k_adam_shadows(st, c->dt, plan, step, lr, b1, b2, eps);
    KCHK(c, "adam (fused with the shadow pass)");
    return LRCN_OK;
}
void fused_update_done(lrcn_ctx *c, float *const p[9]) {
    swap_shadow_sets(c);
    for (int k = 0; k < 9; ++k) c->shadow_p[k] = p[k];
    c->shadow_valid = true;
    c->shadow_has_gi = c->gi_live && c->alt_gi[0] != nullptr;
}

bool lstm_epi_on(lrcn_ctx *c, int B) {
    const char k = knob_char("LRCN_LSTM_EPI");
    return c->dt == GEMM_T_BF16 && !lstm_alone(c) && bg_row_window(B) && !(c->H1 & 3) && !(c->H2 & 3) && (k == '1' || k == 'f');
}
bool lstm_epi_bwd_on(lrcn_ctx *c, int B, int H) {
    return lstm_epi_on(c, B) && knob_char("LRCN_LSTM_EPI") == '1' && H >= 128;
}
auto rec_gemm(lrcn_ctx *c) {
    return [c](const void *A, int64_t lda, const void *B, int64_t ldb, float *C, int64_t ldc, int M, int N, int K, bool beta, bool c_is_zero) {
        return gemm(c, c->dt, A, lda, B, ldb, C, ldc, M, N, K, nullptr, true, beta, false, c_is_zero);
    };
}

int lstm_layer_fwd(lrcn_ctx *c, int S, int B, int H, int64_t ldH, int64_t ld4H, float *Gx, const void *Wh, void *acts,
                   float *Call, void *Hall, const void *Wh_gi = nullptr) {
    const int dt = c->dt;
    const bool epi = !lstm_fused_on(dt, B, H, ldH, ld4H) && Wh_gi && lstm_epi_on(c, B);
    SegScope seg(c, LRCN_SEG_REC_FWD, c->stream, (double)(S - 1) * 4.0 * H * H * c->esz);
    if (!epi) {
        if (int r = lstm_recurrence_fwd(c, lstm_alone(c), rec_gemm(c), S, B, H, ldH, ld4H, Gx, Wh, acts, Call, Hall)) return r;
        KCHK(c, "lstm_layer_fwd");
        return LRCN_OK;
    }
    k_lstm_fwd(c->stream, dt, Gx, 4 * H, nullptr, B, H, acts, ld4H, Call, Hall, ldH, nullptr);
    for (int s = 1; s < S; ++s) {
        GemmArgs g{};
        g.dtype = dt;
        g.A = boff(Hall, (int64_t)(s - 1) * B * ldH, c->esz); g.lda = ldH;
        g.B = Wh_gi; g.ldb = ldH;
        g.M = B; g.N = 4 * H; g.K = (int)ldH;
        g.a_mode = GEMM_A_PLAIN;
        g.out_mode = GEMM_OUT_LSTM_FWD;
        g.zero_page = c->zero_page;
        g.lstm.H = H; g.lstm.ld_a = ld4H; g.lstm.ld_h = ldH;
        g.lstm.Gx = Gx + (int64_t)s * B * 4 * H;
        g.lstm.c_prev = Call + (int64_t)(s - 1) * B * H;
        g.lstm.c_out = Call + (int64_t)s * B * H;
        g.lstm.acts = boff(acts, (int64_t)s * B * ld4H, c->esz);
        g.lstm.h_new = boff(Hall, (int64_t)s * B * ldH, c->esz);
        hipError_t e = launch_gemm_8p(c->stream, g);
        if (e != hipSuccess) FAIL(c, LRCN_EHIP, "lstm fwd step (GEMM + cell epilogue): %s", hipGetErrorString(e));
    }
    KCHK(c, "lstm_layer_fwd");
    return LRCN_OK;
}

int lstm_layer_bwd(lrcn_ctx *c, int S, int B, int H, int64_t ld4H, const void *acts, const float *Call, const float *dHall,
                   const void *WhT, void *dZ) {
    const int dt = c->dt;
    const bool fused = lstm_fused_on(dt, B, H, ld64(H), ld4H);
    SegScope seg(c, LRCN_SEG_REC_BWD, c->stream, (double)(S - 1) * 4.0 * H * H * c->esz);
    if (!fused && lstm_epi_bwd_on(c, B, H)) {
        k_lstm_bwd(c->stream, dt, boff(acts, (int64_t)(S - 1) * B * ld4H, c->esz), ld4H, S > 1 ? Call + (int64_t)(S - 2) * B * H : nullptr,
                   Call + (int64_t)(S - 1) * B * H, dHall + (int64_t)(S - 1) * B * H, H, nullptr, 0, c->dc, 1, B, H,
                   boff(dZ, (int64_t)(S - 1) * B * ld4H, c->esz), ld4H);
        for (int s = S - 1; s >= 1; --s) {
            GemmArgs g{};
            g.dtype = dt;
            g.A = boff(dZ, (int64_t)s * B * ld4H, c->esz); g.lda = ld4H;
            g.B = WhT; g.ldb = ld4H;
            g.M = B; g.N = H; g.K = (int)ld4H;
            g.a_mode = GEMM_A_PLAIN;
            g.out_mode = GEMM_OUT_LSTM_BWD;
            g.zero_page = c->zero_page;
            g.lstm.H = H; g.lstm.ld_a = ld4H;
            g.lstm.acts = const_cast<char *>(boff(acts, (int64_t)(s - 1) * B * ld4H, c->esz));
            g.lstm.c_prev = s > 1 ? Call + (int64_t)(s - 2) * B * H : nullptr;
            g.lstm.c_new = Call + (int64_t)(s - 1) * B * H;
            g.lstm.dh_ext = dHall + (int64_t)(s - 1) * B * H;
            g.lstm.dc = c->dc;
            g.lstm.dz_out = boff(dZ, (int64_t)(s - 1) * B * ld4H, c->esz);
            hipError_t e = launch_gemm_8p(c->stream, g);
            if (e != hipSuccess) FAIL(c, LRCN_EHIP, "lstm bwd step (GEMM + cell epilogue): %s", hipGetErrorString(e));
        }
        KCHK(c, "lstm_layer_bwd (epilogue)");
        return LRCN_OK;
    }
    {
        const int nsl = knob_int("LRCN_BWD_SLABS", 0);
        const int Kp = (int)round_up64(4 * H, 64);
        if (!fused && nsl >= 2 && nsl <= 8 && dt == GEMM_T_BF16 && !lstm_alone(c) && bg_row_window(B) && !(H & 3) && H >= 128 &&
            Kp / 64 >= 8 * nsl && Kp <= ld4H && (size_t)nsl * B * H * sizeof(float) <= c->gemm_ws_bytes && c->gemm_ws) {
            float *slabs = reinterpret_cast<float *>(c->gemm_ws);
            for (int s = S - 1; s >= 0; --s) {
                k_lstm_bwd(c->stream, dt, boff(acts, (int64_t)s * B * ld4H, c->esz), ld4H, s ? Call + (int64_t)(s - 1) * B * H : nullptr,
                           Call + (int64_t)s * B * H, dHall + (int64_t)s * B * H, H, slabs, s < S - 1, c->dc, s == S - 1, B, H,
                           boff(dZ, (int64_t)s * B * ld4H, c->esz), ld4H, nsl);
                if (s > 0) {
                    GemmArgs g{};
                    g.dtype = dt;
                    g.A = boff(dZ, (int64_t)s * B * ld4H, c->esz); g.lda = ld4H;
                    g.B = WhT; g.ldb = ld4H;
                    g.M = B; g.N = H; g.K = Kp;
                    g.C = slabs; g.ldc = H; g.c_f32 = 1;
                    g.a_mode = GEMM_A_PLAIN; g.out_mode = GEMM_OUT_PLAIN;
                    g.zero_page = c->zero_page;
                    g.ws = c->gemm_ws; g.ws_bytes = c->gemm_ws_bytes;
                    g.cfg_pref = 2;
                    g.splitk_forced = 1; g.splitk_no_reduce = 1;
                    hipError_t e = launch_gemm_8p(c->stream, g, nsl);
                    if (e != hipSuccess) FAIL(c, LRCN_EHIP, "lstm bwd step (split-K slabs): %s", hipGetErrorString(e));
                }
            }
            KCHK(c, "lstm_layer_bwd (K slices summed by the cell kernel)");
            return LRCN_OK;
        }
    }
    if (int r = lstm_recurrence_bwd(c, lstm_alone(c), rec_gemm(c), S, B, H, ld4H, acts, Call, dHall, WhT, dZ)) return r;
    KCHK(c, fused ? "lstm_layer_bwd (fused)" : "lstm_layer_bwd");
    return LRCN_OK;
}

int check_shapes(lrcn_ctx *c, int T, int B, int norm_B) {
    if (T < 0 || T + 1 > c->maxS) FAIL(c, LRCN_EINVAL, "T=%d outside [0,%d]", T, c->maxS - 1);
    if (B < 1 || B > c->maxB) FAIL(c, LRCN_EINVAL, "B=%d outside [1,%d]", B, c->maxB);
    if (norm_B < 1) FAIL(c, LRCN_EINVAL, "norm_B=%d must be >= 1", norm_B);
    return LRCN_OK;
}

int upload_lens(lrcn_ctx *c, const int32_t *lens, int B) {
    if (!c->lens_dev) DALLOC(c, c->lens_dev, sizeof(int32_t) * (size_t)c->maxB);
    if (!c->lens_pin)
        HIPCHK(c, hipHostMalloc((void **)&c->lens_pin, sizeof(int32_t) * (size_t)c->maxB * lrcn_ctx::kLenSlots, hipHostMallocDefault));
    for (auto &e : c->lens_up)
        if (!e) HIPCHK(c, hipEventCreateWithFlags(&e, hipEventDisableTiming));
    const int k = c->lens_slot;
    c->lens_slot = (k + 1) % lrcn_ctx::kLenSlots;
    HIPCHK(c, hipEventSynchronize(c->lens_up[k]));
    int32_t *slot = c->lens_pin + (size_t)k * c->maxB;
    std::memcpy(slot, lens, sizeof(int32_t) * (size_t)B);
    HIPCHK(c, hipMemcpyAsync(c->lens_dev, slot, sizeof(int32_t) * (size_t)B, hipMemcpyHostToDevice, c->stream));
    HIPCHK(c, hipEventRecord(c->lens_up[k], c->stream));
    return LRCN_OK;
}

int loss_impl(lrcn_ctx *c, const float *const p[9], const float *feats, const int32_t *tokens, int T, int B, int norm_B,
              const lrcn_dropout *drop, float *const grads[9], float *logits_out, const int32_t *lens = nullptr, int64_t norm_tokens = 0) {
    int r = check_shapes(c, T, B, norm_B);
    if (r) return r;
    if (lens) {
        if (norm_tokens < 1) FAIL(c, LRCN_EINVAL, "norm_tokens=%lld must be >= 1", (long long)norm_tokens);
        for (int b = 0; b < B; ++b)
            if (lens[b] < 0 || lens[b] > T) FAIL(c, LRCN_EINVAL, "lens[%d]=%d outside [0,%d]", b, lens[b], T);
    }
    if (drop && (drop->pdrop < 0.0f || drop->pdrop >= 1.0f)) FAIL(c, LRCN_EINVAL, "pdrop=%g outside [0,1)", drop->pdrop);
    if (drop && c->nl == 2 && ((drop->mask1 == nullptr) != (drop->mask2 == nullptr))) FAIL(c, LRCN_EINVAL, "mask1/mask2 must both be set");
    const int dt = c->dt, E = c->E, H1 = c->H1, H2 = c->H2, h = c->h, V = c->V, X1 = c->X1;
    const int S = T + 1, M = S * B;
    const size_t es = c->esz;
    hipStream_t st = c->stream;
    const bool bwd = grads != nullptr, two = c->nl == 2;
    if (bwd && (!grads[0] || !grads[1] || !grads[5] || !grads[6] || !grads[7] || !grads[8] || (two && (!grads[2] || !grads[3] || !grads[4]))))
        FAIL(c, LRCN_EINVAL, "null gradient tensor");
    const DropSpec d1 = make_drop(drop, 1), d2 = make_drop(drop, 2);
    const DropSpec none{};

    c->cur_B = B;
    const bool epi = lstm_epi_on(c, B) && !lstm_fused_on(c->dt, B, H1, c->ldH1, c->ld4H1);
    r = prepare_weights(c, p, bwd, false, epi);
    if (r) return r;
    if (lens) {
        if ((r = upload_lens(c, lens, B))) return r;
        k_build_tokens_var(st, tokens, c->lens_dev, T, B, V, c->tok_in, c->tok_tgt, c->logp);
    } else {
        k_build_tokens(st, tokens, T, B, V, c->tok_in, c->tok_tgt, c->logp);
    }
    const bool beside_vgg = !lstm_alone(c) && B >= kBgMinRows;
    const bool par = knob_set("LRCN_WG_STREAM") ? !knob_off("LRCN_WG_STREAM") : !beside_vgg;
    const bool xfork = two && par;
    auto image_embedding = [&](hipStream_t s_, bool on_wg) -> int {
        k_transpose(s_, dt, 1, feats, B, LRCN_CNNOUT, B, c->F, LRCN_CNNOUT, 0);
        return gemm(c, dt, c->F, LRCN_CNNOUT, c->Wcd, LRCN_CNNOUT, c->xcnn, c->ldh, B, h, LRCN_CNNOUT, nullptr, true, false, false, false, on_wg);
    };
    int rx = LRCN_OK;
    if (xfork) {
        HIPCHK(c, hipEventRecord(c->xc_fork, st));
        HIPCHK(c, hipStreamWaitEvent(c->wg_stream, c->xc_fork, 0));
        rx = image_embedding(c->wg_stream, true);
        (void)hipEventRecord(c->xc_done, c->wg_stream);
    } else {
        rx = image_embedding(st, false);
        if (rx) return rx;
    }
    auto first_layer = [&]() -> int {
        {
            SegScope seg(c, LRCN_SEG_EMBED_GATHER, st, 2.0 * M * E * es);
            k_embed_gather(st, dt, c->WeT, c->ldE, c->tok_in, S, B, E, two ? d1 : none, c->Xemb, c->ldX1);
        }
        if (!two) k_concat_x2(st, dt, c->Xemb, c->ldX1, c->xcnn, c->ldh, S, B, E, h, d1);
        GEMM(c, dt, c->Xemb, c->ldX1, c->W1x, c->ldX1, c->G1, 4 * H1, M, 4 * H1, X1, p[1], true);
        return lstm_layer_fwd(c, S, B, H1, c->ldH1, c->ld4H1, c->G1, c->W1h, c->A1, c->C1, c->H1all, epi ? c->W1h_gi : nullptr);
    };
    r = first_layer();
    if (xfork) {
        if (hipStreamWaitEvent(st, c->xc_done, 0) != hipSuccess) (void)hipStreamSynchronize(c->wg_stream);
        if (rx) return rx;
    }
    if (r) return r;
    const void *Htop = c->H1all;
    if (two) {
        GEMM(c, dt, c->H1all, c->ldH1, c->Wpd, c->ldH1, c->X2, c->ldH2, M, h, H1, nullptr, false);
        k_concat_x2(st, dt, c->X2, c->ldH2, c->xcnn, c->ldh, S, B, h, h, d2);
        GEMM(c, dt, c->X2, c->ldH2, c->W2x, c->ldH2, c->G2, 4 * H2, M, 4 * H2, H2, p[3], true);
        r = lstm_layer_fwd(c, S, B, H2, c->ldH2, c->ld4H2, c->G2, c->W2h, c->A2, c->C2, c->H2all, epi ? c->W2h_gi : nullptr);
        if (r) return r;
        Htop = c->H2all;
    }
    GEMM(c, dt, Htop, c->ldH2, c->Wod, c->ldH2, c->Logits, c->ldV, M, V, H2, p[8], true);
    if (logits_out) {
        for (int s = 0; s < S; ++s)
            k_transpose_f32(st, c->Logits + (int64_t)s * B * c->ldV, c->ldV, B, V, logits_out + (int64_t)s * B * V, B);
    }
    const float scale = (float)(1.0 / (lens ? (double)norm_tokens : (double)norm_B * (double)S));
    if (c->opt_det && !c->logp_rows) DALLOC(c, c->logp_rows, sizeof(double) * (size_t)c->maxS * c->maxB);
    (lens ? k_softmax_xent_masked : k_softmax_xent)(st, dt, c->Logits, c->ldV, c->tok_tgt, M, V, scale, c->logp, bwd ? c->dLog : nullptr, c->ldV,
                                                    c->opt_det ? c->logp_rows : nullptr);
    c->last_norm = norm_B;
    c->last_S = S;
    c->last_tokens = lens ? norm_tokens : 0;
    KCHK(c, "forward");
    if (!bwd) return LRCN_OK;

    const int64_t ldM = ld64(M), ldB = ld64(B);
    auto tr = [&](TrPlan &pl, const void *src, int64_t ld_src, int R, int C, void *dst, int shift) {
        TrDesc &d = pl.d[pl.n++];
        d.src = src; d.ld_src = ld_src; d.R = R; d.C = C; d.dst = dst; d.ld_dst = ldM; d.shift = shift;
    };
    hipStream_t sw = par ? c->wg_stream : st;
    int nfork = 0;
    auto fork = [&]() -> int {
        if (!par) return LRCN_OK;
        HIPCHK(c, hipEventRecord(c->wg_fork[nfork], st));
        HIPCHK(c, hipStreamWaitEvent(sw, c->wg_fork[nfork], 0));
        ++nfork;
        return LRCN_OK;
    };
#define FORK()                  \
    do {                        \
        int _r = fork();        \
        if (_r) return _r;      \
    } while (0)
    auto backward = [&]() -> int {
        FORK();
        {
            TrPlan pl{};
            tr(pl, c->dLog, c->ldV, M, V, c->TA, 0);
            tr(pl, Htop, c->ldH2, M, H2, c->TB, 0);
            k_transpose_multi(sw, dt, pl);
        }
        GEMM(c, dt, c->TA, ldM, c->TB, ldM, grads[7], H2, V, H2, M, nullptr, true, false, false, false, par);
        k_colsum(sw, dt, c->dLog, c->ldV, M, V, grads[8], c->opt_det);
        HIPCHK(c, hipEventRecord(c->grad_ev[0], sw));
        GEMM(c, dt, c->dLog, c->ldV, c->WoT, c->ldV, two ? c->dH2all : c->dH1all, H2, M, H2, V, nullptr, true);
        if (two) {
            r = lstm_layer_bwd(c, S, B, H2, c->ld4H2, c->A2, c->C2, c->dH2all, c->W2hT, c->dZ2);
            if (r) return r;
            FORK();
            {
                TrPlan pl{};
                tr(pl, c->dZ2, c->ld4H2, M, 4 * H2, c->TA, 0);
                tr(pl, c->X2, c->ldH2, M, H2, c->TB, 0);
                tr(pl, c->H2all, c->ldH2, M - B, H2, boff(c->TB, (int64_t)H2 * ldM, es), M > B ? B : 0);
                k_transpose_multi(sw, dt, pl);
            }
            GEMM(c, dt, c->TA, ldM, c->TB, ldM, grads[2], 2 * H2, 4 * H2, 2 * H2, M, nullptr, true, false, false, false, par);
            k_colsum(sw, dt, c->dZ2, c->ld4H2, M, 4 * H2, grads[3], c->opt_det);
        }
        HIPCHK(c, hipEventRecord(c->grad_ev[1], sw));
        if (two) {
            GEMM(c, dt, c->dZ2, c->ld4H2, c->W2xT, c->ld4H2, c->dX2, c->ldH2, M, H2, 4 * H2, nullptr, false);
            k_dx2_mask_reduce(st, dt, c->dX2, c->ldH2, S, B, h, h, d2, c->dxcnn, c->ldh);
            FORK();
            {
                TrPlan pl{};
                tr(pl, c->dX2, c->ldH2, M, h, c->TA, 0);
                tr(pl, c->H1all, c->ldH1, M, H1, c->TB, 0);
                k_transpose_multi(sw, dt, pl);
            }
            GEMM(c, dt, c->TA, ldM, c->TB, ldM, grads[4], H1, h, H1, M, nullptr, true, false, false, false, par);
            GEMM(c, dt, c->dX2, c->ldH2, c->WpT, c->ldh, c->dH1all, H1, M, H1, h, nullptr, true);
            k_transpose(sw, dt, 1, c->dxcnn, c->ldh, B, h, c->dxcT, ldB, 0);
            k_cast_rows(sw, dt, feats, B, LRCN_CNNOUT, B, c->FT, ldB);
            GEMM(c, dt, c->dxcT, ldB, c->FT, ldB, grads[5], LRCN_CNNOUT, h, LRCN_CNNOUT, B, nullptr, true, false, false, false, par);
            HIPCHK(c, hipEventRecord(c->grad_ev[2], sw));
        }
        r = lstm_layer_bwd(c, S, B, H1, c->ld4H1, c->A1, c->C1, c->dH1all, c->W1hT, c->dZ1);
        if (r) return r;
        FORK();
        {
            TrPlan pl{};
            tr(pl, c->dZ1, c->ld4H1, M, 4 * H1, c->TA, 0);
            tr(pl, c->Xemb, c->ldX1, M, X1, c->TB, 0);
            tr(pl, c->H1all, c->ldH1, M - B, H1, boff(c->TB, (int64_t)X1 * ldM, es), M > B ? B : 0);
            k_transpose_multi(sw, dt, pl);
        }
        GEMM(c, dt, c->TA, ldM, c->TB, ldM, grads[0], X1 + H1, 4 * H1, X1 + H1, M, nullptr, true, false, false, false, par);
        k_colsum(sw, dt, c->dZ1, c->ld4H1, M, 4 * H1, grads[1], c->opt_det);
        HIPCHK(c, hipEventRecord(c->grad_ev[3], sw));
        GEMM(c, dt, c->dZ1, c->ld4H1, c->W1xT, c->ld4H1, c->dXemb, c->ldX1, M, X1, 4 * H1, nullptr, true);
        if (!two) {
            k_dx2_mask_reduce(st, GEMM_T_F32, c->dXemb, c->ldX1, S, B, E, h, d1, c->dxcnn, c->ldh);
            FORK();
            k_transpose(sw, dt, 1, c->dxcnn, c->ldh, B, h, c->dxcT, ldB, 0);
            k_cast_rows(sw, dt, feats, B, LRCN_CNNOUT, B, c->FT, ldB);
            GEMM(c, dt, c->dxcT, ldB, c->FT, ldB, grads[5], LRCN_CNNOUT, h, LRCN_CNNOUT, B, nullptr, true, false, false, false, par);
            HIPCHK(c, hipEventRecord(c->grad_ev[2], sw));
        }
        SegScope seg_eg(c, LRCN_SEG_EMBED_GRAD, st, 4.0 * M * E + 4.0 * (double)V * E);
        if (c->emb_rows_out) {
            if (M > c->emb_rows_cap) FAIL(c, LRCN_EINVAL, "embedding-row buffer holds %d rows, this call has %d", c->emb_rows_cap, M);
            k_embed_rows_export(st, c->dXemb, c->ldX1, S, B, E, two ? d1 : none, c->emb_rows_out);
            HIPCHK(c, hipMemcpyAsync(c->emb_tok_out, c->tok_in, sizeof(int32_t) * (size_t)M, hipMemcpyDeviceToDevice, st));
        } else {
            if (!c->dWe_rm) DALLOC(c, c->dWe_rm, sizeof(float) * (size_t)V * c->ldE);
            unsigned long long *keys = nullptr;
            if (c->opt_det) {
                if (!c->sort_keys) DALLOC(c, c->sort_keys, sizeof(unsigned long long) * (size_t)c->maxS * c->maxB);
                keys = c->sort_keys;
            }
            const bool done = k_embed_scatter_rm(st, c->dXemb, c->ldX1, c->tok_in, S, B, E, V, two ? d1 : none, c->dWe_rm, c->ldE, grads[6], keys);
            if (!done && c->opt_det) FAIL(c, LRCN_EINVAL, "LRCN_OPT_DETERMINISTIC supports (T+1)*B <= 8192 rows per call (got %d)", M);
            if (!done) {
                HIPCHK(c, hipMemsetAsync(grads[6], 0, sizeof(float) * (size_t)V * E, st));
                k_embed_scatter(st, c->dXemb, c->ldX1, c->tok_in, S, B, E, V, two ? d1 : none, grads[6]);
            }
        }
        HIPCHK(c, hipEventRecord(c->grad_ev[4], st));
        return LRCN_OK;
    };
    r = backward();
    if (par && nfork > 0) {
        const hipError_t e1 = hipEventRecord(c->wg_done, sw);
        const hipError_t e2 = e1 == hipSuccess ? hipStreamWaitEvent(st, c->wg_done, 0) : e1;
        if (e2 != hipSuccess) {
            (void)hipStreamSynchronize(sw);
            if (!r) FAIL(c, LRCN_EHIP, "joining the weight-gradient stream: %s", hipGetErrorString(e2));
        }
    }
    if (r) return r;
#undef FORK
    KCHK(c, "backward");
    return LRCN_OK;
}

int fetch_loss(lrcn_ctx *c, double *out) {
    double s[2] = {0.0, 0.0};
    HIPCHK(c, hipMemcpyAsync(s, c->logp, 2 * sizeof(double), hipMemcpyDeviceToHost, c->stream));
    HIPCHK(c, hipStreamSynchronize(c->stream));
    if (s[1] != 0.0) {
        HIPCHK(c, hipMemsetAsync(c->logp + 1, 0, sizeof(double), c->stream));
        FAIL(c, LRCN_EINVAL, "a token id was outside [0, V=%d) (ids are 0-based at the ABI: eos=0, bos=1, unk=2; the reference raises BoundsError, lrcn.jl:556/569)", c->V);
    }
    if (out) *out = -s[0] / (c->last_tokens > 0 ? (double)c->last_tokens : (double)c->last_norm * (double)c->last_S);
    return LRCN_OK;
}

void ctx_sizes(const lrcn_ctx *c, int64_t sz[9]) { lrcn_param_sizes_n(c->nl, c->E, c->H1, c->H2, c->V, sz); }


bool dp_force_pipeline() {
    return knob_char("LRCN_DP_FORCE_PIPELINE") == '1';
}

int ensure_buckets(lrcn_ctx *c) {
    if (!c->comm_stream) {
        HIPCHK(c, hipStreamCreateWithFlags(&c->comm_stream, hipStreamNonBlocking));
        c->comm_stream_owned = true;
    }
    for (int g = 0; g < LRCN_GRAD_GROUPS; ++g) {
        c->bucket[g] = c->comm_stream;
        if (!c->bucket_done[g]) HIPCHK(c, hipEventCreateWithFlags(&c->bucket_done[g], hipEventDisableTiming));
        if (!c->ar_done[g]) HIPCHK(c, hipEventCreateWithFlags(&c->ar_done[g], hipEventDisableTiming));
    }
    return LRCN_OK;
}

int allreduce_group(lrcn_ctx *c, float *const grads[9], int group) {
    int64_t sz[9];
    ctx_sizes(c, sz);
    hipStream_t s = c->comm_stream;
    HIPCHK(c, hipStreamWaitEvent(s, c->grad_ev[group], 0));
    if (c->comm && (comm_world(c->comm) > 1 || dp_force_pipeline())) {
        char err[256] = "";
        const int k0 = kGradGroup[group][0], k1 = kGradGroup[group][1];
        int rc = 0;
        if (k0 == k1 || sz[k1] == 0) {
            rc = comm_allreduce_f32(c->comm, grads[k0], (size_t)sz[k0], s, err, sizeof(err));
        } else if (sz[k0] == 0) {
            rc = comm_allreduce_f32(c->comm, grads[k1], (size_t)sz[k1], s, err, sizeof(err));
        } else if (grads[k0] + sz[k0] == grads[k1]) {
            rc = comm_allreduce_f32(c->comm, grads[k0], (size_t)(sz[k0] + sz[k1]), s, err, sizeof(err));
        } else {
            comm_group_begin(c->comm);
            rc = comm_allreduce_f32(c->comm, grads[k0], (size_t)sz[k0], s, err, sizeof(err));
            if (!rc) rc = comm_allreduce_f32(c->comm, grads[k1], (size_t)sz[k1], s, err, sizeof(err));
            comm_group_end(c->comm);
        }
        if (rc) FAIL(c, LRCN_EHIP, "%s", err);
    }
    HIPCHK(c, hipEventRecord(c->ar_done[group], s));
    HIPCHK(c, hipStreamWaitEvent(c->bucket[group], c->ar_done[group], 0));
    c->bucket_pending[group] = true;
    return LRCN_OK;
}

int join_buckets(lrcn_ctx *c) {
    for (int g = 0; g < LRCN_GRAD_GROUPS; ++g)
        if (c->bucket_pending[g]) {
            HIPCHK(c, hipEventRecord(c->bucket_done[g], c->bucket[g]));
            HIPCHK(c, hipStreamWaitEvent(c->stream, c->bucket_done[g], 0));
            c->bucket_pending[g] = false;
        }
    return LRCN_OK;
}

}

int lrcn_impl::prepare_weights(lrcn_ctx *c, const float *const p[9], bool need_bwd, bool cat, bool gi, bool cat_perm,
                    bool dec_tables) {
    const int dt = c->dt, H1 = c->H1, H2 = c->H2, X1 = c->X1;
    if (!p[0] || !p[1] || !p[5] || !p[6] || !p[7] || !p[8] || (c->nl == 2 && (!p[2] || !p[3] || !p[4]))) FAIL(c, LRCN_EINVAL, "null parameter tensor");
    hipStream_t st = c->stream;
    const bool two = c->nl == 2;
    if (gi || dec_tables) {
        int rg = ensure_gi_sets(c);
        if (rg) return rg;
        if (gi) c->gi_live = true;
    }
    if (dec_tables) gi = true;
    if (c->opt_fused && c->shadow_valid && !cat && (!gi || c->shadow_has_gi)) {
        bool same = true;
        for (int k = 0; k < 9; ++k) same = same && c->shadow_p[k] == p[k];
        if (same) return LRCN_OK;
    }
    c->shadow_valid = false;
    c->refresh_groups = 0;
    PrepPlan plan{};
    void *const gi_cur[2] = {c->W1h_gi, c->W2h_gi};
    plan_matrices(c, p, cur_shadows(c), need_bwd, plan, -1, -1, gi ? gi_cur : nullptr);
    if (dec_tables && c->nl == 2) {
        const int64_t ld = c->ldh + c->ldH2;
        PrepDesc &a = plan.d[plan.n++];
        a = PrepDesc{};
        a.src = p[2]; a.R = 4 * H2; a.C = 2 * H2; a.cs = c->h; a.dA = c->dec_W2c; a.ldA = ld; a.permH = H2;
        PrepDesc &b = plan.d[plan.n++];
        b = PrepDesc{};
        b.src = p[2]; b.R = 4 * H2; b.C = 2 * H2; b.cs = H2; b.dB = boff(c->dec_W2c, c->ldh, c->esz); b.ldB = ld; b.permH = H2;
    }
    if (cat) {
        auto add = [&](const float *src, int R, int C, int cs, void *dA, int64_t ldA, void *dB, int64_t ldB, int permH) {
            PrepDesc &d = plan.d[plan.n++];
            d = PrepDesc{};
            d.src = src; d.R = R; d.C = C; d.cs = cs; d.dA = dA; d.ldA = ldA; d.dB = dB; d.ldB = ldB;
            d.permH = cat_perm ? permH : 0;
        };
        add(p[0], 4 * H1, X1 + H1, X1, c->W1cat, c->ldXH1, boff(c->W1cat, c->ldX1, c->esz), c->ldXH1, H1);
        if (two) add(p[2], 4 * H2, 2 * H2, H2, c->W2cat, c->ldXH2, boff(c->W2cat, c->ldH2, c->esz), c->ldXH2, H2);
    }
    k_prepare_weights(st, dt, plan);
    KCHK(c, "prepare_weights");
    return LRCN_OK;
}

int lrcn_impl::step_internal(lrcn_ctx *c, const float *const p[9], int B, const DropSpec &d2, bool h_ready) {
    const int dt = c->dt, E = c->E, H1 = c->H1, H2 = c->H2, h = c->h, V = c->V, X1 = c->X1;
    hipStream_t st = c->stream;
    const bool two = c->nl == 2;
    if (!two) k_concat_x2(st, dt, c->st_x, c->ldX1, c->xcnn, c->ldh, 1, B, E, h, d2);
    if (!h_ready) k_cast_rows(st, dt, c->st_f32[0], H1, B, H1, c->st_h1, c->ldH1);
    GEMM(c, dt, c->st_x, c->ldX1, c->W1x, c->ldX1, c->st_g, 4 * H1, B, 4 * H1, X1, p[1], true);
    GEMM(c, dt, c->st_h1, c->ldH1, c->W1h, c->ldH1, c->st_g, 4 * H1, B, 4 * H1, H1, nullptr, true, true);
    k_lstm_fwd(st, dt, c->st_g, 4 * H1, c->st_f32[1], B, H1, c->st_a, c->ld4H1, c->st_f32[1], c->st_h1, c->ldH1, c->st_f32[0]);
    if (!two) {
        GEMM(c, dt, c->st_h1, c->ldH1, c->Wod, c->ldH2, c->st_logits, c->ldV, B, V, H2, p[8], true);
        KCHK(c, "step (1 layer)");
        return LRCN_OK;
    }
    GEMM(c, dt, c->st_h1, c->ldH1, c->Wpd, c->ldH1, c->st_x2, c->ldH2, B, h, H1, nullptr, false);
    k_concat_x2(st, dt, c->st_x2, c->ldH2, c->xcnn, c->ldh, 1, B, h, h, d2);
    if (!h_ready) k_cast_rows(st, dt, c->st_f32[2], H2, B, H2, c->st_h2, c->ldH2);
    GEMM(c, dt, c->st_x2, c->ldH2, c->W2x, c->ldH2, c->st_g, 4 * H2, B, 4 * H2, H2, p[3], true);
    GEMM(c, dt, c->st_h2, c->ldH2, c->W2h, c->ldH2, c->st_g, 4 * H2, B, 4 * H2, H2, nullptr, true, true);
    k_lstm_fwd(st, dt, c->st_g, 4 * H2, c->st_f32[3], B, H2, c->st_a, c->ld4H2, c->st_f32[3], c->st_h2, c->ldH2, c->st_f32[2]);
    GEMM(c, dt, c->st_h2, c->ldH2, c->Wod, c->ldH2, c->st_logits, c->ldV, B, V, H2, p[8], true);
    KCHK(c, "step");
    return LRCN_OK;
}

extern "C" {

const char *lrcn_version(void) { return "lrcn-hip 0.4 (gfx950)"; }
int lrcn_abi_version(void) { return LRCN_ABI_VERSION; }

int lrcn_set_option(lrcn_ctx *c, int option, int64_t value) {
    if (!c) return LRCN_EINVAL;
    switch (option) {
    case LRCN_OPT_FUSED_UPDATE:
        if (value != 0 && value != 1) FAIL(c, LRCN_EINVAL, "LRCN_OPT_FUSED_UPDATE takes 0 or 1");
        c->opt_fused = value != 0;
        c->shadow_valid = false;
        c->fused_groups = 0;
        if (c->opt_fused) {
            DeviceGuard dg(c);
            return ensure_alt_shadows(c);
        }
        return LRCN_OK;
    case LRCN_OPT_DETERMINISTIC:
        if (value != 0 && value != 1) FAIL(c, LRCN_EINVAL, "LRCN_OPT_DETERMINISTIC takes 0 or 1");
        c->opt_det = value != 0;
        return LRCN_OK;
    case LRCN_OPT_CONV_CHUNK_BYTES:
        if (value < 0) FAIL(c, LRCN_EINVAL, "LRCN_OPT_CONV_CHUNK_BYTES must be >= 0");
        c->conv_chunk_bytes = value;
        return LRCN_OK;
    default:
        FAIL(c, LRCN_EINVAL, "unknown option %d", option);
    }
}

int lrcn_params_touched(lrcn_ctx *c) {
    if (!c) return LRCN_EINVAL;
    c->shadow_valid = false;
    c->fused_groups = 0;
    c->refresh_groups = 0;
    return LRCN_OK;
}

const char *lrcn_last_error(const lrcn_ctx *ctx) { return ctx ? ctx->err.c_str() : g_create_err.c_str(); }

int lrcn_param_sizes_n(int n_layers, int E, int H1, int H2, int V, int64_t s[9]) {
    if (E < 1 || H1 < 1 || H2 < 2 || (H2 & 1) || V < 3 || !s) return LRCN_EINVAL;
    if (n_layers != 0 && n_layers != 1 && n_layers != 2) return LRCN_EINVAL;
    const int h = H2 / 2;
    if (n_layers == 1) {
        if (H1 != H2) return LRCN_EINVAL;
        s[0] = (int64_t)(E + h + H1) * 4 * H1;
        s[2] = s[3] = s[4] = 0;
    } else {
        s[0] = (int64_t)(E + H1) * 4 * H1;
        s[2] = (int64_t)(2 * H2) * 4 * H2;
        s[3] = 4 * H2;
        s[4] = (int64_t)H1 * h;
    }
    s[1] = 4 * H1;
    s[5] = (int64_t)LRCN_CNNOUT * h;
    s[6] = (int64_t)V * E;
    s[7] = (int64_t)H2 * V;
    s[8] = V;
    return LRCN_OK;
}
int lrcn_param_sizes(int E, int H1, int H2, int V, int64_t s[9]) { return lrcn_param_sizes_n(2, E, H1, H2, V, s); }

int lrcn_malloc(void **p, size_t bytes) { return hipMalloc(p, bytes ? bytes : 16) == hipSuccess ? LRCN_OK : LRCN_ENOMEM; }
int lrcn_free(void *p) { return hipFree(p) == hipSuccess ? LRCN_OK : LRCN_EHIP; }
int lrcn_memcpy_h2d(void *d, const void *s, size_t n) { return hipMemcpy(d, s, n, hipMemcpyHostToDevice) == hipSuccess ? LRCN_OK : LRCN_EHIP; }
int lrcn_memcpy_d2h(void *d, const void *s, size_t n) { return hipMemcpy(d, s, n, hipMemcpyDeviceToHost) == hipSuccess ? LRCN_OK : LRCN_EHIP; }

void lrcn_destroy(lrcn_ctx *c) {
    if (!c) return;
    DeviceGuard dg(c);
    (void)hipDeviceSynchronize();
    for (void *p : c->allocs) (void)hipFree(p);
    if (c->sc_arena) (void)hipFree(c->sc_arena);
    for (auto &e : c->grad_ev)
        if (e) (void)hipEventDestroy(e);
    for (auto &e : c->wg_fork)
        if (e) (void)hipEventDestroy(e);
    if (c->wg_done) (void)hipEventDestroy(c->wg_done);
    if (c->xc_fork) (void)hipEventDestroy(c->xc_fork);
    if (c->xc_done) (void)hipEventDestroy(c->xc_done);
    if (c->pin) (void)hipHostFree(c->pin);
    if (c->lens_pin) (void)hipHostFree(c->lens_pin);
    for (auto &e : c->lens_up)
        if (e) (void)hipEventDestroy(e);
    if (c->wg_stream && c->wg_stream_owned) (void)hipStreamDestroy(c->wg_stream);
    if (c->copy_stream) (void)hipStreamDestroy(c->copy_stream);
    for (int j = 0; j < lrcn_ctx::kStage; ++j) {
        if (c->up_done[j]) (void)hipEventDestroy(c->up_done[j]);
        if (c->rd_done[j]) (void)hipEventDestroy(c->rd_done[j]);
    }
    comm_destroy(c->comm);
    for (auto &e : c->bucket_done)
        if (e) (void)hipEventDestroy(e);
    for (auto &e : c->ar_done)
        if (e) (void)hipEventDestroy(e);
    if (c->comm_stream && c->comm_stream_owned) (void)hipStreamDestroy(c->comm_stream);
    for (auto &sp : c->seg)
        for (auto &e : sp.ev) {
            (void)hipEventDestroy(e.first);
            (void)hipEventDestroy(e.second);
        }
    for (auto &e : c->prof_ev) {
        (void)hipEventDestroy(e.first);
        (void)hipEventDestroy(e.second);
    }
    delete c;
}

int lrcn_create(const lrcn_config *cfg, lrcn_ctx **out) {
    if (!cfg || !out) {
        g_create_err = "null argument";
        return LRCN_EINVAL;
    }
    *out = nullptr;
    int64_t sz[9];
    if (lrcn_param_sizes_n(cfg->n_layers, cfg->E, cfg->H1, cfg->H2, cfg->V, sz) != LRCN_OK || cfg->max_B < 1 || cfg->max_T < 0 ||
        cfg->max_T > LRCN_MAX_T || (cfg->lstm_dtype != LRCN_F32 && cfg->lstm_dtype != LRCN_BF16) ||
        (cfg->vgg_dtype != LRCN_F32 && cfg->vgg_dtype != LRCN_BF16 && cfg->vgg_dtype != LRCN_FP8) || cfg->max_images < 0) {
        g_create_err = "invalid lrcn_config (need E,H1>=1, even H2>=2, V>=3, max_B>=1, 0<=max_T<=28, lstm_dtype in {F32,BF16}, vgg_dtype in {F32,BF16,FP8}, n_layers in {0,1,2} with H1 == H2 when n_layers == 1)";
        return LRCN_EINVAL;
    }
    int ndev = 0;
    if (hipGetDeviceCount(&ndev) != hipSuccess || cfg->device < 0 || cfg->device >= ndev) {
        g_create_err = "no such HIP device (is a GPU visible?)";
        return LRCN_EHIP;
    }
    lrcn_ctx *c = new lrcn_ctx();
    c->cfg = *cfg;
    DeviceGuard dg(c);
    {
        int cur = -1;
        if (hipGetDevice(&cur) != hipSuccess || cur != cfg->device) {
            g_create_err = "hipSetDevice failed";
            delete c;
            return LRCN_EHIP;
        }
    }
    c->opt_det = knob_char("LRCN_DETERMINISTIC") == '1';
    if (hipDeviceGetAttribute(&c->ncu, hipDeviceAttributeMultiprocessorCount, cfg->device) != hipSuccess || c->ncu < 1) c->ncu = 256;
    c->dt = cfg->lstm_dtype == LRCN_BF16 ? GEMM_T_BF16 : GEMM_T_F32;
    c->vdt = cfg->vgg_dtype == LRCN_F32 ? GEMM_T_F32 : GEMM_T_BF16;
    c->vgg_fp8 = cfg->vgg_dtype == LRCN_FP8;
    c->esz = c->dt == GEMM_T_BF16 ? 2 : 4;
    c->vesz = c->vdt == GEMM_T_BF16 ? 2 : 4;
    c->E = cfg->E; c->H1 = cfg->H1; c->H2 = cfg->H2; c->h = cfg->H2 / 2; c->V = cfg->V;
    c->nl = cfg->n_layers == 1 ? 1 : 2;
    c->X1 = c->nl == 1 ? c->E + c->h : c->E;
    c->maxB = cfg->max_B; c->maxS = cfg->max_T + 1;
    const int E = c->E, H1 = c->H1, H2 = c->H2, h = c->h, V = c->V, B = c->maxB, S = c->maxS;
    const int64_t M = (int64_t)S * B;
    const int X1 = c->X1;
    c->ldX1 = ld64(X1);
    c->ldE = ld64(E); c->ldH1 = ld64(H1); c->ldH2 = ld64(H2); c->ldh = ld64(h); c->ld4H1 = ld64(4 * H1); c->ld4H2 = ld64(4 * H2);
    c->ldV = ld64(V); c->ldM = ld64(M); c->ldB = ld64(B);
    const size_t es = c->esz;
    int rc = [&]() -> int {
        c->ldXH1 = c->ldX1 + c->ldH1; c->ldXH2 = 2 * c->ldH2;
        DALLOC(c, c->W1cat, es * 4 * H1 * c->ldXH1); DALLOC(c, c->W2cat, es * 4 * H2 * c->ldXH2);
        DALLOC(c, c->st_xh1, es * B * c->ldXH1);     DALLOC(c, c->st_xh2, es * B * c->ldXH2);
        DALLOC(c, c->W1x, es * 4 * H1 * c->ldX1);  DALLOC(c, c->W1h, es * 4 * H1 * c->ldH1);
        DALLOC(c, c->W1xT, es * X1 * c->ld4H1);    DALLOC(c, c->W1hT, es * H1 * c->ld4H1);
        DALLOC(c, c->W2x, es * 4 * H2 * c->ldH2);  DALLOC(c, c->W2h, es * 4 * H2 * c->ldH2);
        DALLOC(c, c->W2xT, es * H2 * c->ld4H2);    DALLOC(c, c->W2hT, es * H2 * c->ld4H2);
        DALLOC(c, c->Wpd, es * h * c->ldH1);       DALLOC(c, c->WpT, es * H1 * c->ldh);
        DALLOC(c, c->Wcd, es * h * LRCN_CNNOUT);   DALLOC(c, c->WeT, es * V * c->ldE);
        DALLOC(c, c->Wod, es * V * c->ldH2);       DALLOC(c, c->WoT, es * H2 * c->ldV);
        DALLOC(c, c->tok, sizeof(int32_t) * M);    DALLOC(c, c->tok_in, sizeof(int32_t) * M);
        DALLOC(c, c->tok_tgt, sizeof(int32_t) * M);
        DALLOC(c, c->F, es * B * LRCN_CNNOUT);     DALLOC(c, c->FT, es * LRCN_CNNOUT * c->ldB);
        DALLOC(c, c->xcnn, sizeof(float) * B * c->ldh);
        DALLOC(c, c->Xemb, es * M * c->ldX1);
        DALLOC(c, c->G1, sizeof(float) * M * 4 * H1); DALLOC(c, c->A1, es * M * c->ld4H1);
        DALLOC(c, c->C1, sizeof(float) * M * H1);     DALLOC(c, c->H1all, es * M * c->ldH1);
        DALLOC(c, c->X2, es * M * c->ldH2);
        DALLOC(c, c->G2, sizeof(float) * M * 4 * H2); DALLOC(c, c->A2, es * M * c->ld4H2);
        DALLOC(c, c->C2, sizeof(float) * M * H2);     DALLOC(c, c->H2all, es * M * c->ldH2);
        DALLOC(c, c->Logits, sizeof(float) * M * c->ldV);
        DALLOC(c, c->dLog, es * M * c->ldV);
        DALLOC(c, c->dZ1, es * M * c->ld4H1);      DALLOC(c, c->dZ2, es * M * c->ld4H2);
        DALLOC(c, c->dX2, es * M * c->ldH2);
        DALLOC(c, c->dH1all, sizeof(float) * M * H1); DALLOC(c, c->dH2all, sizeof(float) * M * H2);
        DALLOC(c, c->dXemb, sizeof(float) * M * c->ldX1);
        const int Hm = H1 > H2 ? H1 : H2;
        DALLOC(c, c->dhrec, sizeof(float) * B * Hm); DALLOC(c, c->dc, sizeof(float) * B * Hm);
        DALLOC(c, c->dxcnn, sizeof(float) * B * c->ldh); DALLOC(c, c->dxcT, es * h * c->ldB);
        int64_t ra = 4 * Hm; if (V > ra) ra = V;
        int64_t rb = 2 * H2; if (X1 + H1 > rb) rb = X1 + H1;
        DALLOC(c, c->TA, es * ra * c->ldM);        DALLOC(c, c->TB, es * rb * c->ldM);
        DALLOC(c, c->logp, sizeof(double) * 2);
        DALLOC(c, c->zero_page, 256);
        if (hipMemset(c->zero_page, 0, 256) != hipSuccess) return LRCN_EHIP;
        for (auto &e : c->grad_ev)
            if (hipEventCreateWithFlags(&e, hipEventDisableTiming) != hipSuccess) return LRCN_EHIP;
        c->gemm_ws_bytes = 48u << 20;
        DALLOC(c, c->gemm_ws, c->gemm_ws_bytes);
        DALLOC(c, c->wg_ws, c->gemm_ws_bytes);
        if (hipStreamCreateWithFlags(&c->wg_stream, hipStreamNonBlocking) != hipSuccess) return LRCN_EHIP;
        for (auto &e : c->wg_fork)
            if (hipEventCreateWithFlags(&e, hipEventDisableTiming) != hipSuccess) return LRCN_EHIP;
        if (hipEventCreateWithFlags(&c->wg_done, hipEventDisableTiming) != hipSuccess) return LRCN_EHIP;
        if (hipEventCreateWithFlags(&c->xc_fork, hipEventDisableTiming) != hipSuccess) return LRCN_EHIP;
        if (hipEventCreateWithFlags(&c->xc_done, hipEventDisableTiming) != hipSuccess) return LRCN_EHIP;
        if (cfg->max_images > 0) DALLOC(c, c->vgg_ws, c->gemm_ws_bytes);
        for (int i = 0; i < 4; ++i) {
            DALLOC(c, c->st_f32[i], sizeof(float) * B * Hm);
            DALLOC(c, c->st2_f32[i], sizeof(float) * B * Hm);
        }
        DALLOC(c, c->st_h1, es * B * c->ldH1);     DALLOC(c, c->st_h2, es * B * c->ldH2);
        DALLOC(c, c->st_x, es * B * c->ldX1);      DALLOC(c, c->st_x2, es * B * c->ldH2);
        DALLOC(c, c->st_a, es * B * (c->ld4H1 > c->ld4H2 ? c->ld4H1 : c->ld4H2));
        DALLOC(c, c->st_g, sizeof(float) * B * 4 * Hm);
        DALLOC(c, c->st_logits, sizeof(float) * B * c->ldV); DALLOC(c, c->st_prob, sizeof(float) * B * c->ldV);
        int64_t io = (int64_t)B * (V > 4 * Hm ? V : 4 * Hm); if (io < (int64_t)B * (X1 + Hm)) io = (int64_t)B * (X1 + Hm);
        DALLOC(c, c->st_io, sizeof(float) * io);
        DALLOC(c, c->st_topi, sizeof(int32_t) * B * 32); DALLOC(c, c->st_topv, sizeof(float) * B * 32);
        DALLOC(c, c->st_parent, sizeof(int32_t) * B);
        for (int i = 0; i < 2; ++i) DALLOC(c, c->bs_seq[i], sizeof(int32_t) * B * LRCN_BEAM_MAXLEN);
        DALLOC(c, c->bs_last, sizeof(int32_t) * B);      DALLOC(c, c->bs_done, sizeof(int32_t) * B);
        DALLOC(c, c->bs_ndone, sizeof(int32_t) * 4);     DALLOC(c, c->bs_res_tok, sizeof(int32_t) * B * LRCN_BEAM_MAXLEN);
        DALLOC(c, c->bs_res_len, sizeof(int32_t) * B);   DALLOC(c, c->bs_p, sizeof(float) * B);
        DALLOC(c, c->bs_res_p, sizeof(float) * B);
        if (cfg->max_images > 0) {
            const int64_t N = cfg->max_images;
            const size_t ve = c->vesz;
            if (c->vdt != GEMM_T_BF16) DALLOC(c, c->im2col, ve * N * 224 * 224 * 32);
            DALLOC(c, c->actA, ve * N * 224 * 224 * 64);
            if (c->vdt == GEMM_T_BF16) DALLOC(c, c->img16, 2 * (N * 228 * 228 * 3 + 8));
            DALLOC(c, c->actB, ve * N * 112 * 112 * 128);
            DALLOC(c, c->f6, ve * N * 4096);
            DALLOC(c, c->featsRM, sizeof(float) * N * 4096);
            if (c->vgg_fp8) DALLOC(c, c->amax_dev, sizeof(float) * 16);
        }
        return LRCN_OK;
    }();
    if (rc) {
        g_create_err = c->err;
        lrcn_destroy(c);
        return rc;
    }
    *out = c;
    return LRCN_OK;
}

int lrcn_vgg_set_wg_cap(lrcn_ctx *c, int cap) {
    DeviceGuard dg(c);
    if (!c) return LRCN_EINVAL;
    if (cap < 0 || (cap > 0 && cap < 8)) FAIL(c, LRCN_EINVAL, "wg_cap=%d must be 0 (off) or >= 8", cap);
    c->vgg_wg_cap = cap;
    return LRCN_OK;
}

int lrcn_set_stream(lrcn_ctx *c, void *s) {
    DeviceGuard dg(c);
    if (!c) return LRCN_EINVAL;
    c->stream = reinterpret_cast<hipStream_t>(s);
    return LRCN_OK;
}
int lrcn_set_wg_stream(lrcn_ctx *c, void *s) {
    DeviceGuard dg(c);
    if (!c || !s) return LRCN_EINVAL;
    if (c->wg_stream) {
        HIPCHK(c, hipStreamSynchronize(c->wg_stream));
        if (c->wg_stream_owned) (void)hipStreamDestroy(c->wg_stream);
    }
    c->wg_stream = reinterpret_cast<hipStream_t>(s);
    c->wg_stream_owned = false;
    return LRCN_OK;
}
int lrcn_sync(lrcn_ctx *c) {
    if (!c) return LRCN_EINVAL;
    DeviceGuard dg(c);
    return fetch_loss(c, nullptr);
}

int lrcn_init_weights(lrcn_ctx *c, float *const p[9], uint64_t seed) {
    DeviceGuard dg(c);
    if (!c || !p) return LRCN_EINVAL;
    int64_t sz[9];
    ctx_sizes(c, sz);
    const int E = c->E, H1 = c->H1, H2 = c->H2, h = c->h, V = c->V;
    const int rows[9] = {c->X1 + H1, 1, 2 * H2, 1, H1, LRCN_CNNOUT, V, H2, 1};
    const int cols[9] = {4 * H1, 4 * H1, 4 * H2, 4 * H2, h, h, E, V, V};
    for (int k = 0; k < 9; ++k) {
        if (sz[k] == 0) continue;
        if (!p[k]) FAIL(c, LRCN_EINVAL, "null parameter tensor %d", k);
        if (k == 1 || k == 3 || k == 8) {
            k_fill(c->stream, p[k], sz[k], 0.0f);
            if (k != 8) k_fill(c->stream, p[k], k == 1 ? H1 : H2, 1.0f);
        } else {
            k_init_uniform(c->stream, p[k], sz[k], (float)std::sqrt(2.0 / ((double)rows[k] + (double)cols[k])), seed, k);
        }
    }
    KCHK(c, "init_weights");
    c->shadow_valid = false;
    c->fused_groups = 0;
    return LRCN_OK;
}

int lrcn_loss(lrcn_ctx *c, const float *const p[9], const float *feats, const int32_t *tokens, int T, int B, int norm_B,
              const lrcn_dropout *drop, double *loss_host) {
    DeviceGuard dg(c);
    if (!c || !p || !feats || (!tokens && T > 0)) return LRCN_EINVAL;
    int r = loss_impl(c, p, feats, tokens, T, B, norm_B, drop, nullptr, nullptr);
    if (r) return r;
    return loss_host ? fetch_loss(c, loss_host) : LRCN_OK;
}

int lrcn_loss_grad(lrcn_ctx *c, const float *const p[9], const float *feats, const int32_t *tokens, int T, int B, int norm_B,
                   const lrcn_dropout *drop, float *const grads[9], double *loss_host) {
    DeviceGuard dg(c);
    if (!c || !p || !feats || (!tokens && T > 0) || !grads) return LRCN_EINVAL;
    int r = loss_impl(c, p, feats, tokens, T, B, norm_B, drop, grads, nullptr);
    if (r) return r;
    return loss_host ? fetch_loss(c, loss_host) : LRCN_OK;
}

int lrcn_loss_var(lrcn_ctx *c, const float *const p[9], const float *feats, const int32_t *tokens, const int32_t *lens, int T, int B,
                  int64_t norm_tokens, const lrcn_dropout *drop, double *loss_host) {
    DeviceGuard dg(c);
    if (!c || !p || !feats || (!tokens && T > 0)) return LRCN_EINVAL;
    if (!lens) FAIL(c, LRCN_EINVAL, "lens is NULL");
    int r = loss_impl(c, p, feats, tokens, T, B, 1, drop, nullptr, nullptr, lens, norm_tokens);
    if (r) return r;
    return loss_host ? fetch_loss(c, loss_host) : LRCN_OK;
}

int lrcn_loss_grad_var(lrcn_ctx *c, const float *const p[9], const float *feats, const int32_t *tokens, const int32_t *lens, int T, int B,
                       int64_t norm_tokens, const lrcn_dropout *drop, float *const grads[9], double *loss_host) {
    DeviceGuard dg(c);
    if (!c || !p || !feats || (!tokens && T > 0) || !grads) return LRCN_EINVAL;
    if (!lens) FAIL(c, LRCN_EINVAL, "lens is NULL");
    int r = loss_impl(c, p, feats, tokens, T, B, 1, drop, grads, nullptr, lens, norm_tokens);
    if (r) return r;
    return loss_host ? fetch_loss(c, loss_host) : LRCN_OK;
}

int lrcn_grad_group_wait(lrcn_ctx *c, int group, void *stream) {
    DeviceGuard dg(c);
    if (!c || group < 0 || group >= LRCN_GRAD_GROUPS) return LRCN_EINVAL;
    HIPCHK(c, hipStreamWaitEvent(reinterpret_cast<hipStream_t>(stream), c->grad_ev[group], 0));
    return LRCN_OK;
}

int lrcn_last_loss(lrcn_ctx *c, double *loss_host) {
    DeviceGuard dg(c);
    if (!c || !loss_host) return LRCN_EINVAL;
    return fetch_loss(c, loss_host);
}

int lrcn_forward_logits(lrcn_ctx *c, const float *const p[9], const float *feats, const int32_t *tokens, int T, int B,
                        float *logits_out) {
    DeviceGuard dg(c);
    if (!c || !p || !feats || (!tokens && T > 0) || !logits_out) return LRCN_EINVAL;
    return loss_impl(c, p, feats, tokens, T, B, B, nullptr, nullptr, logits_out);
}

int lrcn_adam_update(lrcn_ctx *c, float *const p[9], const float *const g[9], float *const m[9], float *const v[9], int step,
                     float lr, float b1, float b2, float eps) {
    DeviceGuard dg(c);
    if (!c || !p || !g || !m || !v || step < 1) return LRCN_EINVAL;
    c->fused_groups = 0;
    int64_t nparam = 0;
    {
        int64_t szp[9];
        ctx_sizes(c, szp);
        for (int k = 0; k < 9; ++k) nparam += szp[k];
    }
    SegScope seg(c, LRCN_SEG_UPDATE, c->stream, 28.0 * (double)nparam);
    if (c->opt_fused) {
        c->shadow_valid = false;
        int r = adam_fused(c, p, g, m, v, -1, step, lr, b1, b2, eps, c->stream);
        if (r) return r;
        fused_update_done(c, p);
        return LRCN_OK;
    }
    c->shadow_valid = false;
    AdamTensors t;
    int64_t sz[9];
    ctx_sizes(c, sz);
    for (int k = 0; k < 9; ++k) {
        t.w[k] = p[k];
        t.g[k] = g[k];
        t.m[k] = m[k];
        t.v[k] = v[k];
        t.n[k] = sz[k];
    }
    k_adam(c->stream, t, step, lr, b1, b2, eps);
    KCHK(c, "adam");
    return LRCN_OK;
}

int lrcn_adam_update_group(lrcn_ctx *c, float *const p[9], const float *const g[9], float *const m[9], float *const v[9], int group,
                           int step, float lr, float b1, float b2, float eps, void *stream) {
    DeviceGuard dg(c);
    if (!c || !p || !g || !m || !v || step < 1) return LRCN_EINVAL;
    if (group < 0 || group >= LRCN_GRAD_GROUPS) FAIL(c, LRCN_EINVAL, "group=%d outside [0,%d)", group, LRCN_GRAD_GROUPS);
    int64_t szg[9];
    ctx_sizes(c, szg);
    SegScope seg(c, LRCN_SEG_UPDATE, stream ? reinterpret_cast<hipStream_t>(stream) : c->stream,
                 28.0 * (double)(szg[kGradGroup[group][0]] + (kGradGroup[group][1] != kGradGroup[group][0] ? szg[kGradGroup[group][1]] : 0)));
    if (c->opt_fused) {
        if (step != c->fused_step) {
            c->fused_groups = 0;
            c->fused_step = step;
        }
        c->shadow_valid = false;
        int r = adam_fused(c, p, g, m, v, group, step, lr, b1, b2, eps, stream ? reinterpret_cast<hipStream_t>(stream) : c->stream);
        if (r) {
            c->fused_groups = 0;
            return r;
        }
        c->fused_groups |= 1u << group;
        if (c->fused_groups == (1u << LRCN_GRAD_GROUPS) - 1) {
            c->fused_groups = 0;
            fused_update_done(c, p);
        }
        return LRCN_OK;
    }
    c->shadow_valid = false;
    AdamTensors t;
    int64_t sz[9];
    ctx_sizes(c, sz);
    for (int k = 0; k < 9; ++k) {
        const bool in = k == kGradGroup[group][0] || k == kGradGroup[group][1];
        t.w[k] = p[k];
        t.g[k] = g[k];
        t.m[k] = m[k];
        t.v[k] = v[k];
        t.n[k] = in ? sz[k] : 0;
    }
    k_adam(stream ? reinterpret_cast<hipStream_t>(stream) : c->stream, t, step, lr, b1, b2, eps);
    KCHK(c, "adam (group)");
    return LRCN_OK;
}

int lrcn_refresh_shadows_group(lrcn_ctx *c, const float *const p[9], int group, void *stream) {
    DeviceGuard dg(c);
    if (!c || !p) return LRCN_EINVAL;
    if (group < 0 || group >= LRCN_GRAD_GROUPS) FAIL(c, LRCN_EINVAL, "group=%d outside [0,%d)", group, LRCN_GRAD_GROUPS);
    if (!c->opt_fused) FAIL(c, LRCN_ESTATE, "lrcn_refresh_shadows_group needs LRCN_OPT_FUSED_UPDATE = 1 (the second shadow set)");
    int r = ensure_alt_shadows(c);
    if (r) return r;
    if (c->refresh_groups == 0) c->shadow_valid = false;
    PrepPlan plan{};
    if (c->gi_live && (r = ensure_gi_sets(c))) return r;
    plan_matrices(c, p, alt_shadows(c), true, plan, kGradGroup[group][0], kGradGroup[group][1], c->gi_live ? c->alt_gi : nullptr);
    if (plan.n > 0) {
        k_prepare_weights(stream ? reinterpret_cast<hipStream_t>(stream) : c->stream, c->dt, plan);
        KCHK(c, "refresh_shadows_group");
    }
    c->refresh_groups |= 1u << group;
    if (c->refresh_groups == (1u << LRCN_GRAD_GROUPS) - 1) {
        c->refresh_groups = 0;
        float *pp[9];
        for (int k = 0; k < 9; ++k) pp[k] = const_cast<float *>(p[k]);
        fused_update_done(c, pp);
    }
    return LRCN_OK;
}

int lrcn_adam_update_flat(lrcn_ctx *c, float *w, const float *g, float *m, float *v, int64_t n, int step, float lr, float b1, float b2,
                          float eps, void *stream) {
    DeviceGuard dg(c);
    if (!c || step < 1 || n < 0) return LRCN_EINVAL;
    if (n == 0) return LRCN_OK;
    if (!w || !g || !m || !v) return LRCN_EINVAL;
    c->shadow_valid = false;
    SegScope seg(c, LRCN_SEG_UPDATE, stream ? reinterpret_cast<hipStream_t>(stream) : c->stream, 28.0 * (double)n);
    AdamTensors t{};
    t.w[0] = w; t.g[0] = g; t.m[0] = m; t.v[0] = v; t.n[0] = n;
    k_adam(stream ? reinterpret_cast<hipStream_t>(stream) : c->stream, t, step, lr, b1, b2, eps);
    KCHK(c, "adam (flat)");
    return LRCN_OK;
}

int lrcn_train_step(lrcn_ctx *c, float *const p[9], float *const g[9], float *const m[9], float *const v[9], const float *feats,
                    const int32_t *tokens, int T, int B, int norm_B, const lrcn_dropout *drop, int step, float lr, float b1,
                    float b2, float eps, double *loss_host) {
    DeviceGuard dg(c);
    if (!c || !p || !g || !m || !v) return LRCN_EINVAL;
    int r = lrcn_loss_grad(c, p, feats, tokens, T, B, norm_B, drop, g, nullptr);
    if (r) return r;
    r = lrcn_adam_update(c, p, g, m, v, step, lr, b1, b2, eps);
    if (r) return r;
    return loss_host ? fetch_loss(c, loss_host) : LRCN_OK;
}

int lrcn_train_step_var(lrcn_ctx *c, float *const p[9], float *const g[9], float *const m[9], float *const v[9], const float *feats,
                        const int32_t *tokens, const int32_t *lens, int T, int B, int64_t norm_tokens, const lrcn_dropout *drop, int step,
                        float lr, float b1, float b2, float eps, double *loss_host) {
    DeviceGuard dg(c);
    if (!c || !p || !g || !m || !v) return LRCN_EINVAL;
    int r = lrcn_loss_grad_var(c, p, feats, tokens, lens, T, B, norm_tokens, drop, g, nullptr);
    if (r) return r;
    r = lrcn_adam_update(c, p, g, m, v, step, lr, b1, b2, eps);
    if (r) return r;
    return loss_host ? fetch_loss(c, loss_host) : LRCN_OK;
}

int lrcn_comm_unique_id(void *id_out) {
    if (!id_out) return LRCN_EINVAL;
    char err[256] = "";
    if (comm_unique_id(id_out, err, sizeof(err))) {
        g_create_err = err;
        return LRCN_EHIP;
    }
    return LRCN_OK;
}

int lrcn_comm_probe(lrcn_ctx *c) {
    if (!c) return LRCN_EINVAL;
    if (c->comm) FAIL(c, LRCN_ESTATE, "the context already has a communicator");
    char err[256] = "";
    if (comm_available(err, sizeof(err))) FAIL(c, LRCN_EHIP, "%s", err);
    return LRCN_OK;
}

int lrcn_comm_init(lrcn_ctx *c, int world, int rank, const void *unique_id) {
    DeviceGuard dg(c);
    if (!c) return LRCN_EINVAL;
    if (world < 1 || rank < 0 || rank >= world || !unique_id) FAIL(c, LRCN_EINVAL, "comm_init: world=%d rank=%d", world, rank);
    if (c->comm) FAIL(c, LRCN_ESTATE, "the context already has a communicator");
    char err[256] = "";
    c->comm = comm_create(world, rank, unique_id, err, sizeof(err));
    if (!c->comm) FAIL(c, LRCN_EHIP, "%s", err);
    return ensure_buckets(c);
}

int lrcn_set_embed_rows_buffer(lrcn_ctx *c, float *rows, int32_t *tok, int capacity_rows) {
    if (!c) return LRCN_EINVAL;
    if ((rows == nullptr) != (tok == nullptr) || capacity_rows < 0) FAIL(c, LRCN_EINVAL, "rows and tok must both be given (capacity >= 0) or both NULL");
    c->emb_rows_out = rows;
    c->emb_tok_out = tok;
    c->emb_rows_cap = rows ? capacity_rows : 0;
    return LRCN_OK;
}

int lrcn_embed_grad_from_rows(lrcn_ctx *c, const float *rows, const int32_t *tok, int n_rows, float *grad_wembed, void *stream) {
    DeviceGuard dg(c);
    if (!c || !rows || !tok || !grad_wembed) return LRCN_EINVAL;
    if (n_rows < 1 || n_rows > 8192) FAIL(c, LRCN_EINVAL, "n_rows=%d outside [1, 8192] (the ordered sum ranks at most 8192 keys)", n_rows);
    if (!c->dWe_rm) DALLOC(c, c->dWe_rm, sizeof(float) * (size_t)c->V * c->ldE);
    if (!c->imp_keys) DALLOC(c, c->imp_keys, sizeof(unsigned long long) * 8192);
    hipStream_t st = stream ? reinterpret_cast<hipStream_t>(stream) : c->stream;
    DropSpec none{};
    if (!k_embed_scatter_rm(st, rows, c->E, tok, n_rows, 1, c->E, c->V, none, c->dWe_rm, c->ldE, grad_wembed, c->imp_keys))
        FAIL(c, LRCN_EINVAL, "embed_grad_from_rows: too many rows (%d)", n_rows);
    KCHK(c, "embed_grad_from_rows");
    return LRCN_OK;
}

int lrcn_comm_set_stream(lrcn_ctx *c, void *hip_stream) {
    DeviceGuard dg(c);
    if (!c || !hip_stream) return LRCN_EINVAL;
    for (bool p : c->bucket_pending)
        if (p) FAIL(c, LRCN_ESTATE, "a gradient exchange is in flight: call lrcn_comm_join first");
    if (c->comm_stream && c->comm_stream_owned) {
        HIPCHK(c, hipStreamSynchronize(c->comm_stream));
        (void)hipStreamDestroy(c->comm_stream);
    }
    c->comm_stream = reinterpret_cast<hipStream_t>(hip_stream);
    c->comm_stream_owned = false;
    return ensure_buckets(c);
}

int lrcn_comm_destroy(lrcn_ctx *c) {
    DeviceGuard dg(c);
    if (!c) return LRCN_EINVAL;
    HIPCHK(c, hipDeviceSynchronize());
    comm_destroy(c->comm);
    c->comm = nullptr;
    return LRCN_OK;
}

int lrcn_allreduce_grads(lrcn_ctx *c, float *const grads[9], int group) {
    DeviceGuard dg(c);
    if (!c || !grads) return LRCN_EINVAL;
    if (group < -1 || group >= LRCN_GRAD_GROUPS) FAIL(c, LRCN_EINVAL, "group=%d outside [-1,%d)", group, LRCN_GRAD_GROUPS);
    int r = ensure_buckets(c);
    if (r) return r;
    for (int g = (group < 0 ? 0 : group); g < (group < 0 ? LRCN_GRAD_GROUPS : group + 1); ++g) {
        r = allreduce_group(c, grads, g);
        if (r) return r;
    }
    return LRCN_OK;
}

int lrcn_comm_join(lrcn_ctx *c) {
    DeviceGuard dg(c);
    if (!c) return LRCN_EINVAL;
    return join_buckets(c);
}

int lrcn_lstm(lrcn_ctx *c, const float *W, const float *b, int X, int H, int B, const float *x, const float *h, const float *cc,
              float *h_out, float *c_out) {
    DeviceGuard dg(c);
    if (!c || !W || !b || !x || !h || !cc || !h_out || !c_out) return LRCN_EINVAL;
    void *Wx, *Wh, *xb, *hb;
    if (X == c->X1 && H == c->H1) {
        Wx = c->W1x; Wh = c->W1h; xb = c->st_x; hb = c->st_h1;
    } else if (c->nl == 2 && X == c->H2 && H == c->H2) {
        Wx = c->W2x; Wh = c->W2h; xb = c->st_x2; hb = c->st_h2;
    } else {
        FAIL(c, LRCN_EINVAL, "lrcn_lstm: (X=%d,H=%d) must be the context's LSTM-1 (%d,%d) or (two layers) LSTM-2 (%d,%d)", X, H, c->X1, c->H1,
             c->H2, c->H2);
    }
    if (B < 1 || B > c->maxB) FAIL(c, LRCN_EINVAL, "B=%d outside [1,%d]", B, c->maxB);
    const int dt = c->dt;
    hipStream_t st = c->stream;
    const int64_t ldX = ld64(X), ldH = ld64(H);
    c->shadow_valid = false;
    k_cast_rows(st, dt, W, X + H, 4 * H, X, Wx, ldX);
    k_cast_rows(st, dt, W + X, X + H, 4 * H, H, Wh, ldH);
    k_transpose(st, dt, 1, x, B, X, B, xb, ldX, 0);
    k_transpose(st, dt, 1, h, B, H, B, hb, ldH, 0);
    k_transpose_f32(st, cc, B, H, B, c->st_f32[1], H);
    GEMM(c, dt, xb, ldX, Wx, ldX, c->st_g, 4 * H, B, 4 * H, X, b, true);
    GEMM(c, dt, hb, ldH, Wh, ldH, c->st_g, 4 * H, B, 4 * H, H, nullptr, true, true);
    k_lstm_fwd(st, dt, c->st_g, 4 * H, c->st_f32[1], B, H, c->st_a, ld64(4 * H), c->st_f32[1], hb, ldH, c->st_f32[0]);
    k_transpose_f32(st, c->st_f32[0], H, B, H, h_out, B);
    k_transpose_f32(st, c->st_f32[1], H, B, H, c_out, B);
    KCHK(c, "lrcn_lstm");
    return LRCN_OK;
}

int lrcn_step(lrcn_ctx *c, const float *const p[9], float *const state[4], int B, const float *x_cnn, const float *x_lstm,
              const float *mask1, const float *mask2, float *logits) {
    DeviceGuard dg(c);
    if (!c || !p || !state || !x_cnn || !x_lstm || !logits) return LRCN_EINVAL;
    if (B < 1 || B > c->maxB) FAIL(c, LRCN_EINVAL, "B=%d outside [1,%d]", B, c->maxB);
    const int dt = c->dt, E = c->E, H1 = c->H1, H2 = c->H2, h = c->h, V = c->V;
    hipStream_t st = c->stream;
    int r = prepare_weights(c, p, false);
    if (r) return r;
    const int Hs[4] = {H1, H1, H2, H2};
    const int ns = c->nl == 1 ? 2 : 4;
    for (int i = 0; i < ns; ++i) {
        if (!state[i]) FAIL(c, LRCN_EINVAL, "null state tensor %d", i);
        k_transpose_f32(st, state[i], B, Hs[i], B, c->st_f32[i], Hs[i]);
    }
    k_transpose_f32(st, x_cnn, B, h, B, c->xcnn, c->ldh);
    DropSpec d2{};
    d2.which = c->nl == 1 ? 1 : 2;
    d2.mask = c->nl == 1 ? mask1 : mask2;
    const float *xsrc = x_lstm;
    if (mask1 && c->nl == 2) {
        k_mul_f32(st, x_lstm, mask1, (int64_t)B * E, c->st_io);
        xsrc = c->st_io;
    }
    k_transpose(st, dt, 1, xsrc, B, E, B, c->st_x, c->ldX1, 0);
    r = step_internal(c, p, B, d2);
    if (r) return r;
    for (int i = 0; i < ns; ++i) k_transpose_f32(st, c->st_f32[i], Hs[i], B, Hs[i], state[i], B);
    k_transpose_f32(st, c->st_logits, c->ldV, B, V, logits, B);
    KCHK(c, "lrcn_step");
    return LRCN_OK;
}

int lrcn_train_step_dp(lrcn_ctx *c, float *const p[9], float *const g[9], float *const m[9], float *const v[9], const uint8_t *img_u8,
                       const float mean[3], int normalize, float *feats, const int32_t *tokens, int T, int B, int norm_B,
                       const lrcn_dropout *drop, int step, float lr, float b1, float b2, float eps, double *loss_host) {
    DeviceGuard dg(c);
    if (!c || !p || !g || !m || !v || !feats || step < 1) return LRCN_EINVAL;
    int r;
    if (img_u8) {
        if (!mean && !c->avg_on) FAIL(c, LRCN_EINVAL, "img_u8 given without channel means or an averageImage");
        r = vgg_check(c, B);
        if (r) return r;
        r = vgg_body(c, B, img_u8, true, mean);
        if (r) return r;
        k_transpose_f32(c->stream, c->featsRM, 4096, B, 4096, feats, B);
        if (normalize) k_normalize_rows(c->stream, feats, B, LRCN_CNNOUT);
        KCHK(c, "train_step_dp (vgg)");
    }
    r = loss_impl(c, p, feats, tokens, T, B, norm_B, drop, g, nullptr);
    if (r) return r;
    if (!c->comm || (comm_world(c->comm) == 1 && !dp_force_pipeline())) {
        r = lrcn_adam_update(c, p, g, m, v, step, lr, b1, b2, eps);
        if (r) return r;
        return loss_host ? fetch_loss(c, loss_host) : LRCN_OK;
    }
    r = ensure_buckets(c);
    if (r) return r;
    for (int grp = 0; grp < LRCN_GRAD_GROUPS; ++grp) {
        r = allreduce_group(c, g, grp);
        if (r) return r;
        r = lrcn_adam_update_group(c, p, g, m, v, grp, step, lr, b1, b2, eps, c->bucket[grp]);
        if (r) return r;
    }
    r = join_buckets(c);
    if (r) return r;
    return loss_host ? fetch_loss(c, loss_host) : LRCN_OK;
}

int lrcn_debug_stamps(lrcn_ctx *c, unsigned long long *host_out, int64_t n) {
    DeviceGuard dg(c);
    if (!c || !host_out || n < 1) return LRCN_EINVAL;
    if (!c->stamps || n > c->stamps_n) FAIL(c, LRCN_ESTATE, "no stamps recorded (LRCN_STAMPS=1 and lrcn_bench_conv first), or n > %lld", (long long)c->stamps_n);
    HIPCHK(c, hipStreamSynchronize(c->stream));
    HIPCHK(c, hipMemcpy(host_out, c->stamps, sizeof(unsigned long long) * (size_t)n, hipMemcpyDeviceToHost));
    return LRCN_OK;
}

const char *lrcn_debug_route(lrcn_ctx *c, int which) {
    if (which == 1) return c ? c->vgg_routes.c_str() : "";
    return gemm_debug_last_route();
}

int lrcn_profile(lrcn_ctx *c, int enable) {
    DeviceGuard dg(c);
    if (!c) return LRCN_EINVAL;
    c->prof = enable != 0;
    c->prof_level = enable;
    c->prof_used = 0;
    c->prof_ms = 0.0;
    c->prof_launches = 0;
    for (auto &sp : c->seg) {
        sp.used = 0;
        sp.ms = sp.bytes = 0.0;
        sp.n = 0;
    }
    return LRCN_OK;
}

int lrcn_profile_segment(lrcn_ctx *c, int segment, double *ms, int64_t *brackets, double *bytes) {
    DeviceGuard dg(c);
    if (!c || !ms || !brackets || !bytes || segment < 0 || segment >= LRCN_SEG_COUNT) return LRCN_EINVAL;
    HIPCHK(c, hipDeviceSynchronize());
    auto &sp = c->seg[segment];
    for (size_t i = 0; i < sp.used; ++i) {
        float t = 0.0f;
        HIPCHK(c, hipEventElapsedTime(&t, sp.ev[i].first, sp.ev[i].second));
        sp.ms += t;
    }
    sp.used = 0;
    *ms = sp.ms;
    *brackets = sp.n;
    *bytes = sp.bytes;
    return LRCN_OK;
}

int lrcn_avg_loss_batch(lrcn_ctx *c, const float *const p[9], const float *feats, const int32_t *tokens, int T, int B, double *loss_host) {
    return lrcn_loss(c, p, feats, tokens, T, B, B, nullptr, loss_host);
}

int lrcn_profile_get(lrcn_ctx *c, double *conv_ms, int64_t *conv_launches) {
    DeviceGuard dg(c);
    if (!c || !conv_ms || !conv_launches) return LRCN_EINVAL;
    HIPCHK(c, hipStreamSynchronize(c->stream));
    for (size_t i = 0; i < c->prof_used; ++i) {
        float ms = 0.0f;
        HIPCHK(c, hipEventElapsedTime(&ms, c->prof_ev[i].first, c->prof_ev[i].second));
        c->prof_ms += ms;
        c->prof_launches += 12;
    }
    c->prof_used = 0;
    *conv_ms = c->prof_ms;
    *conv_launches = c->prof_launches;
    return LRCN_OK;
}

}
```

Measured before the change: 37530.

## Add contract-over-rows GEMM mode to skip transposes in weight gradients

Adds a GEMM_A_ROWS operand mode in the 8-wave GEMM kernel. Both operands are loaded row-major along K into swizzled LDS and read with ds_read_b64_tr_b16 transpose reads, so the weight-gradient GEMMs (dW = dZ^T X) can use activations directly. The backward pass uses this route for the LSTM and output weight gradients instead of k_transpose_multi plus a plain GEMM. This removes the transpose kernels and their scratch TA/TB traffic, now allocated lazily only on fallback. The cost is a new LDS layout and read path that may be less efficient than the tuned plain path, and it relaxes the tile-size eligibility checks.

```diff
diff --git a/long-term-recurrent-convolutional-nn_amd/csrc/gemm.h b/long-term-recurrent-convolutional-nn_amd/csrc/gemm.h
--- a/long-term-recurrent-convolutional-nn_amd/csrc/gemm.h
+++ b/long-term-recurrent-convolutional-nn_amd/csrc/gemm.h
@@ -2,7 +2,7 @@
 #include <hip/hip_runtime.h>
 #include <stdint.h>
 
-enum { GEMM_A_PLAIN = 0, GEMM_A_CONV3 = 1 };
+enum { GEMM_A_PLAIN = 0, GEMM_A_CONV3 = 1, GEMM_A_ROWS = 2 };
 enum { GEMM_OUT_PLAIN = 0, GEMM_OUT_CONV = 1, GEMM_OUT_POOL = 2, GEMM_OUT_LSTM_FWD = 3, GEMM_OUT_LSTM_BWD = 4, GEMM_OUT_SMAX_TOPK = 5,
        GEMM_OUT_SMAX_GUMBEL = 6, GEMM_OUT_SMAX_PICK = 7 };
 
@@ -86,6 +86,8 @@
 
 int gemm_8p_config(const GemmArgs &g, int64_t *blocks);
 int gemm_8p_splitk(const GemmArgs &g, int64_t *blocks);
+bool gemm_8p_rows_ok(const GemmArgs &g);
+bool gemm_rows_route_ok(const GemmArgs &g);
 hipError_t launch_gemm_8p(hipStream_t stream, const GemmArgs &g, int splitk = 1);
 hipError_t launch_splitk_reduce(hipStream_t stream, const GemmArgs &g, int splits);
 
diff --git a/long-term-recurrent-convolutional-nn_amd/csrc/gemm_8p.hip b/long-term-recurrent-convolutional-nn_amd/csrc/gemm_8p.hip
--- a/long-term-recurrent-convolutional-nn_amd/csrc/gemm_8p.hip
+++ b/long-term-recurrent-convolutional-nn_amd/csrc/gemm_8p.hip
@@ -29,6 +29,13 @@
     asm volatile("ds_read_b128 %0, %1 offset:%2" : "=v"(r) : "v"(addr), "n"(OFF) : "memory");
     return r;
 }
+
+template <int OFF> __device__ __forceinline__ uint2 lds_read_tr8(unsigned addr) {
+    uint2 r;
+    asm volatile("ds_read_b64_tr_b16 %0, %1 offset:%2" : "=v"(r) : "v"(addr), "n"(OFF) : "memory");
+    return r;
+}
+template <int RB> __device__ __forceinline__ int rows_swz(int k) { return RB >= 256 ? (k & 7) << 1 : ((k >> 1) & 3) << 1; }
 
 typedef int i32x8v __attribute__((ext_vector_type(8)));
 __device__ __forceinline__ i32x8v pack8(const uint4 &lo, const uint4 &hi) {
@@ -60,6 +67,8 @@
 __device__ __forceinline__ bool gemm8p_tile(const GemmArgs &g, unsigned char *smem, const int tile, const int ntiles_xy, const int next_tile,
                                             TileAddr<WM * (2 * MT * 16) / 128, WN * (2 * NT * 16) / 128> &ta, const bool pre) {
     constexpr int ES = F8 ? 1 : 2;
+    constexpr bool ROWS = AMODE == GEMM_A_ROWS;
+    static_assert(!ROWS || (!F8 && SWAP && EPI == 0), "contract-over-rows: bf16 operands, f32 / split-K epilogues");
     constexpr int KE = 128 / ES;
     static_assert(WM * WN == 8, "8 waves");
     constexpr int QM = MT * 16, QN = NT * 16;
@@ -90,7 +99,7 @@
         return __builtin_amdgcn_make_buffer_rsrc(const_cast<unsigned char *>(base), 0, live ? NREC : 0u, 0x00020000);
     };
 
-    const int kpt = (AMODE == GEMM_A_CONV3) ? g.Cin / KE : g.K / KE;
+    const int kpt = (AMODE == GEMM_A_CONV3) ? g.Cin / KE : ROWS ? (g.K + KE - 1) / KE : g.K / KE;
     const int KT_all = (AMODE == GEMM_A_CONV3) ? 9 * kpt : kpt;
     const int kbeg = (int)((int64_t)KT_all * blockIdx.y / gridDim.y);
     const int KT = (int)((int64_t)KT_all * (blockIdx.y + 1) / gridDim.y) - kbeg;
@@ -112,6 +121,27 @@
         const int nt = bid % tiles_n, mt = bid / tiles_n;
         o.m0 = mt * BM;
         o.n0 = nt * BN;
+        if constexpr (ROWS) {
+#pragma unroll
+            for (int hf = 0; hf < 2; ++hf) {
+#pragma unroll
+                for (int j = 0; j < APW; ++j) {
+                    const int krow = (wave * APW + j) * (1024 / BM) + (lane * 16) / BM;
+                    const int lf = ((((lane * 16) % BM) >> 4) ^ rows_swz<BM>(krow)) * 8;
+                    const int m = o.m0 + (lf / QM) * WTM + hf * QM + (lf % QM);
+                    o.a_voff[hf][j] = m < M ? (unsigned)((int64_t)krow * g.lda * 2 + (int64_t)m * 2) : OOB;
+                    o.a_mask[hf][j] = ~0u;
+                }
+#pragma unroll
+                for (int j = 0; j < BPW; ++j) {
+                    const int krow = (wave * BPW + j) * (1024 / BN) + (lane * 16) / BN;
+                    const int lf = ((((lane * 16) % BN) >> 4) ^ rows_swz<BN>(krow)) * 8;
+                    const int n = o.n0 + (lf / QN) * WTN + hf * QN + (lf % QN);
+                    o.b_voff[hf][j] = n < N ? (unsigned)((int64_t)krow * g.ldb * 2 + (int64_t)n * 2) : OOB;
+                }
+            }
+            return;
+        }
 #pragma unroll
         for (int hf = 0; hf < 2; ++hf) {
 #pragma unroll
@@ -168,6 +198,15 @@
                 const unsigned vo = ta.a_voff[hf][j] | (unsigned)__builtin_amdgcn_sbfe((int)ta.a_mask[hf][j], k.tap, 1);
                 __builtin_amdgcn_raw_ptr_buffer_load_lds(rs, (lds_void *)(smem + buf * BUF + a_piece_row(hf, j) * 128), 16, (int)vo, soff, 0, 0);
             }
+        } else if constexpr (ROWS) {
+            const int krem = g.K - k.koff - wave * APW * (1024 / BM);
+            const int64_t kbyte = (int64_t)k.koff * g.lda * 2;
+#pragma unroll
+            for (int j = 0; j < APW; ++j) {
+                const bool ok = live && ta.a_voff[hf][j] != OOB && j * (1024 / BM) + (lane * 16) / BM < krem;
+                const unsigned char *src = ok ? Aflat + ((int64_t)ta.a_voff[hf][j] + kbyte) : Zp;
+                __builtin_amdgcn_global_load_lds((glb_void *)src, (lds_void *)(smem + buf * BUF + hf * (A_BYTES / 2) + (wave * APW + j) * 1024), 16, 0, 0);
+            }
         } else {
 #pragma unroll
             for (int j = 0; j < APW; ++j) {
@@ -185,6 +224,15 @@
             for (int j = 0; j < BPW; ++j)
                 __builtin_amdgcn_raw_ptr_buffer_load_lds(rs, (lds_void *)(smem + buf * BUF + A_BYTES + b_piece_row(hf, j) * 128), 16,
                                                          (int)ta.b_voff[hf][j], soff, 0, 0);
+        } else if constexpr (ROWS) {
+            const int krem = g.K - k.koff - wave * BPW * (1024 / BN);
+            const int64_t kbyte = (int64_t)k.koff * g.ldb * 2;
+#pragma unroll
+            for (int j = 0; j < BPW; ++j) {
+                const bool ok = live && ta.b_voff[hf][j] != OOB && j * (1024 / BN) + (lane * 16) / BN < krem;
+                const unsigned char *src = ok ? Bbase + ((int64_t)ta.b_voff[hf][j] + kbyte) : Zp;
+                __builtin_amdgcn_global_load_lds((glb_void *)src, (lds_void *)(smem + buf * BUF + A_BYTES + hf * (B_BYTES / 2) + (wave * BPW + j) * 1024), 16, 0, 0);
+            }
         } else {
 #pragma unroll
             for (int j = 0; j < BPW; ++j) {
@@ -203,6 +251,18 @@
         const unsigned base = (unsigned)(uintptr_t)(__attribute__((address_space(3))) unsigned char *)smem;
         fa[s] = base + (wr * WTM) * 128 + fo;
         fb[s] = base + A_BYTES + (wc * WTN) * 128 + fo;
+    }
+
+    [[maybe_unused]] unsigned fta[MT], ftb[NT];
+    if constexpr (ROWS) {
+        const int kl = lane >> 2, p = lane & 3;
+        const unsigned base = (unsigned)(uintptr_t)(__attribute__((address_space(3))) unsigned char *)smem;
+#pragma unroll
+        for (int i = 0; i < MT; ++i)
+            fta[i] = base + kl * BM + ((((wr * QM + i * 16) >> 3) + (p >> 1)) ^ rows_swz<BM>(kl)) * 16 + 8 * (p & 1);
+#pragma unroll
+        for (int n = 0; n < NT; ++n)
+            ftb[n] = base + A_BYTES + kl * BN + ((((wc * QN + n * 16) >> 3) + (p >> 1)) ^ rows_swz<BN>(kl)) * 16 + 8 * (p & 1);
     }
 
     auto issue_first = [&]() {
@@ -244,41 +304,68 @@
                 for (int i = 0; i < MT; ++i) acc[a][i][b][n] = bv;
         }
 
-    uint4 af[MT][2], bf0[NT][2], bf1[NT][2];
+    struct Frag {
+        uint4 q;
+        uint2 t[2];
+    };
+    Frag af[MT][2], bf0[NT][2], bf1[NT][2];
     auto read_a = [&](int buf, auto mhc) {
         constexpr int mh = decltype(mhc)::value;
+        if constexpr (ROWS) {
+            static_for<0, MT>([&](auto ic) {
+                constexpr int i = decltype(ic)::value;
+                const unsigned a = fta[i] + buf * BUF;
+                af[i][0].t[0] = lds_read_tr8<mh * (A_BYTES / 2)>(a);
+                af[i][0].t[1] = lds_read_tr8<mh * (A_BYTES / 2) + 16 * BM>(a);
+                af[i][1].t[0] = lds_read_tr8<mh * (A_BYTES / 2) + 32 * BM>(a);
+                af[i][1].t[1] = lds_read_tr8<mh * (A_BYTES / 2) + 48 * BM>(a);
+            });
+            return;
+        }
         const unsigned a0 = fa[0] + buf * BUF, a1 = fa[1] + buf * BUF;
         static_for<0, MT>([&](auto ic) {
             constexpr int i = decltype(ic)::value;
-            af[i][0] = lds_read16<(mh * QM + i * 16) * 128>(a0);
-            af[i][1] = lds_read16<(mh * QM + i * 16) * 128>(a1);
+            af[i][0].q = lds_read16<(mh * QM + i * 16) * 128>(a0);
+            af[i][1].q = lds_read16<(mh * QM + i * 16) * 128>(a1);
         });
     };
-    auto read_b = [&](int buf, auto nhc, uint4 (&bf)[NT][2]) {
+    auto read_b = [&](int buf, auto nhc, Frag (&bf)[NT][2]) {
         constexpr int nh = decltype(nhc)::value;
+        if constexpr (ROWS) {
+            static_for<0, NT>([&](auto ic) {
+                constexpr int n = decltype(ic)::value;
+                const unsigned b = ftb[n] + buf * BUF;
+                bf[n][0].t[0] = lds_read_tr8<nh * (B_BYTES / 2)>(b);
+                bf[n][0].t[1] = lds_read_tr8<nh * (B_BYTES / 2) + 16 * BN>(b);
+                bf[n][1].t[0] = lds_read_tr8<nh * (B_BYTES / 2) + 32 * BN>(b);
+                bf[n][1].t[1] = lds_read_tr8<nh * (B_BYTES / 2) + 48 * BN>(b);
+            });
+            return;
+        }
         const unsigned b0 = fb[0] + buf * BUF, b1 = fb[1] + buf * BUF;
         static_for<0, NT>([&](auto ic) {
             constexpr int n = decltype(ic)::value;
-            bf[n][0] = lds_read16<(nh * QN + n * 16) * 128>(b0);
-            bf[n][1] = lds_read16<(nh * QN + n * 16) * 128>(b1);
+            bf[n][0].q = lds_read16<(nh * QN + n * 16) * 128>(b0);
+            bf[n][1].q = lds_read16<(nh * QN + n * 16) * 128>(b1);
         });
     };
+    auto frag16 = [](const Frag &f) { return ROWS ? uint4{f.t[0].x, f.t[0].y, f.t[1].x, f.t[1].y} : f.q; };
     constexpr std::integral_constant<int, 0> I0{};
     constexpr std::integral_constant<int, 1> I1{};
 #define MFMA_BODY(mh, nh, BF)                                                                                              \
     do {                                                                                                                   \
         if constexpr (F8) {                                                                                                \
             _Pragma("unroll") for (int i = 0; i < MT; ++i) _Pragma("unroll") for (int n = 0; n < NT; ++n) {                \
-                const i32x8v av = pack8(af[i][0], af[i][1]);                                                               \
-                const i32x8v bv = pack8(BF[n][0], BF[n][1]);                                                               \
+                const i32x8v av = pack8(af[i][0].q, af[i][1].q);                                                           \
+                const i32x8v bv = pack8(BF[n][0].q, BF[n][1].q);                                                           \
                 acc[mh][i][nh][n] = SWAP ? __builtin_amdgcn_mfma_scale_f32_16x16x128_f8f6f4(bv, av, acc[mh][i][nh][n], 0, 0, 0, 0, 0, 0) \
                                          : __builtin_amdgcn_mfma_scale_f32_16x16x128_f8f6f4(av, bv, acc[mh][i][nh][n], 0, 0, 0, 0, 0, 0); \
             }                                                                                                              \
         } else {                                                                                                           \
             _Pragma("unroll") for (int s = 0; s < 2; ++s) _Pragma("unroll") for (int i = 0; i < MT; ++i) _Pragma("unroll") for (int n = 0; \
                                                                                                                    n < NT; ++n) { \
-                const bf16x8 av = __builtin_bit_cast(bf16x8, af[i][s]);                                                    \
-                const bf16x8 bv = __builtin_bit_cast(bf16x8, BF[n][s]);                                                    \
+                const bf16x8 av = __builtin_bit_cast(bf16x8, frag16(af[i][s]));                                            \
+                const bf16x8 bv = __builtin_bit_cast(bf16x8, frag16(BF[n][s]));                                            \
                 acc[mh][i][nh][n] = SWAP ? __builtin_amdgcn_mfma_f32_16x16x32_bf16(bv, av, acc[mh][i][nh][n], 0, 0, 0)     \
                                          : __builtin_amdgcn_mfma_f32_16x16x32_bf16(av, bv, acc[mh][i][nh][n], 0, 0, 0);    \
             }                                                                                                              \
@@ -317,7 +404,7 @@
         stage_b(nxt, 0, kn, live1);
         stage_b(nxt, 1, kn, live1);
         wait_vmcnt<APW + 2 * BPW>();
-        MFMA_PAIR(0, 0, bf0, 0, 1, bf1, 2 * NT);
+        MFMA_PAIR(0, 0, bf0, 0, 1, bf1, (ROWS ? 4 : 2) * NT);
         read_a(cur, I1);
         stage_a(nxt, 1, kn, live1);
         wait_vmcnt<APW>();
@@ -952,7 +1039,23 @@
         default: return hipErrorInvalidValue;
     }
 }
-
+hipError_t dispatch_rows(hipStream_t s, const GemmArgs &g, int cfg, int splitk) {
+    switch (cfg) {
+        case 0: return launch_one<2, 4, 4, 2, GEMM_A_ROWS, true>(s, g, splitk);
+        case 1: return launch_one<4, 2, 2, 2, GEMM_A_ROWS, true>(s, g, splitk);
+        default: return hipErrorInvalidValue;
+    }
+}
+
+}
+
+bool gemm_8p_rows_ok(const GemmArgs &g) {
+    if (g.dtype != GEMM_T_BF16 || g.a_mode != GEMM_A_ROWS || g.out_mode != GEMM_OUT_PLAIN || !g.zero_page || !g.c_f32 || g.relu) return false;
+    if (g.M < 1 || g.N < 1 || g.K < 1 || !g.A || !g.B || !g.C) return false;
+    if (((uintptr_t)g.A & 15) || ((uintptr_t)g.B & 15) || (g.lda % 8) || (g.ldb % 8)) return false;
+    if (g.lda < ((int64_t)g.M + 7) / 8 * 8 || g.ldb < ((int64_t)g.N + 7) / 8 * 8) return false;
+    if (g.lda >= (1 << 22) || g.ldb >= (1 << 22)) return false;
+    return true;
 }
 
 static bool gemm_8p_f8_ok(const GemmArgs &g) {
@@ -965,27 +1068,30 @@
 }
 
 int gemm_8p_config(const GemmArgs &g, int64_t *blocks) {
-    if (g.dtype == GEMM_T_F8) {
+    const bool rows = g.a_mode == GEMM_A_ROWS;
+    if (rows) {
+        if (!gemm_8p_rows_ok(g)) return -1;
+    } else if (g.dtype == GEMM_T_F8) {
         if (!gemm_8p_f8_ok(g)) return -1;
     } else if (g.dtype != GEMM_T_BF16 || !gemm_glds_eligible(g)) {
         return -1;
     }
-    {
+    if (!rows) {
         const int64_t es = g.dtype == GEMM_T_F8 ? 1 : 2;
         const int64_t a_bytes = (g.a_mode == GEMM_A_CONV3 ? (int64_t)g.M * g.Cin + (int64_t)(g.W + 1) * g.Cin : (int64_t)g.M * g.lda) * es;
         if (a_bytes >= 0xFFFF0000ll || (int64_t)g.N * g.ldb * es >= 0xFFFF0000ll) return -1;
     }
-    if ((g.M < 256 && g.dtype != GEMM_T_F8) || g.N < 128) return -1;
+    if (!rows && ((g.M < 256 && g.dtype != GEMM_T_F8) || g.N < 128)) return -1;
     const int ke = g.dtype == GEMM_T_F8 ? 128 : 64;
     const int kt = (g.a_mode == GEMM_A_CONV3) ? 9 * (g.Cin / ke) : g.K / ke;
-    if (kt < 2) return -1;
+    if (!rows && kt < 2) return -1;
     const int64_t b0 = (int64_t)cdiv(g.M, 256) * cdiv(g.N, 256), b1 = (int64_t)cdiv(g.M, 256) * cdiv(g.N, 128);
     int cfg = (g.N > 128 && (b0 >= 200 || g.N % 256 == 0 || g.N > 384)) ? 0 : 1;
     if (cfg == 0 && ((b0 < 200 && b1 >= 200) || (b0 < 128 && b1 >= 128))) cfg = 1;
     if (g.cfg_pref == 2 && g.N >= 128) cfg = 1;
     if (g.free_cus > 0 && g.N > 128 && b0 <= g.free_cus && b1 > g.free_cus) cfg = 0;
     *blocks = cfg == 0 ? b0 : b1;
-    if (cfg == 1 && g.N <= 128 && cdiv(g.M, 512) >= 400) {
+    if (!rows && cfg == 1 && g.N <= 128 && cdiv(g.M, 512) >= 400) {
         cfg = 2;
         *blocks = cdiv(g.M, 512);
     }
@@ -993,11 +1099,13 @@
 }
 
 int gemm_8p_splitk(const GemmArgs &g, int64_t *blocks) {
-    if (g.dtype != GEMM_T_BF16 || !gemm_glds_eligible(g) || g.M < 256 || g.N < 128 || (g.N % 4)) return 0;
+    const bool rows = g.a_mode == GEMM_A_ROWS;
+    if (rows ? !gemm_8p_rows_ok(g) || g.beta : g.dtype != GEMM_T_BF16 || !gemm_glds_eligible(g) || g.M < 256 || g.N < 128) return 0;
+    if (g.N % 4) return 0;
     const bool conv = g.a_mode == GEMM_A_CONV3 && g.out_mode != GEMM_OUT_PLAIN && !g.c_f32 && !g.beta && (g.M & 3) == 0;
-    if (!conv && (g.a_mode != GEMM_A_PLAIN || g.out_mode != GEMM_OUT_PLAIN)) return 0;
+    if (!conv && ((g.a_mode != GEMM_A_PLAIN && !rows) || g.out_mode != GEMM_OUT_PLAIN)) return 0;
     if (!g.ws || (g.ldc % 4) || ((uintptr_t)g.C & 15)) return 0;
-    const int kt = conv ? 9 * (g.Cin / 64) : g.K / 64;
+    const int kt = conv ? 9 * (g.Cin / 64) : rows ? cdiv(g.K, 64) : g.K / 64;
     const int64_t b1 = (int64_t)cdiv(g.M, 256) * cdiv(g.N, 128);
     int s = (int)((g.free_cus > 0 ? g.free_cus : 256) / b1);
     const int min_slice = conv ? 12 : 8;
@@ -1139,13 +1247,16 @@
     }
     if (splitk > 1) {
         if (!g.splitk_forced && gemm_8p_splitk(g, &blocks) != splitk) return hipErrorInvalidValue;
-        hipError_t e = g.a_mode == GEMM_A_CONV3 ? dispatch<GEMM_A_CONV3, true>(stream, g, 1, splitk) : dispatch<GEMM_A_PLAIN, true>(stream, g, 1, splitk);
+        hipError_t e = g.a_mode == GEMM_A_ROWS    ? dispatch_rows(stream, g, 1, splitk)
+                       : g.a_mode == GEMM_A_CONV3 ? dispatch<GEMM_A_CONV3, true>(stream, g, 1, splitk)
+                                                  : dispatch<GEMM_A_PLAIN, true>(stream, g, 1, splitk);
         if (e != hipSuccess) return e;
         if (g.splitk_no_reduce) return hipSuccess;
         return launch_splitk_reduce(stream, g, splitk);
     } else {
         splitk = 1;
     }
+    if (g.a_mode == GEMM_A_ROWS) return dispatch_rows(stream, g, cfg, 1);
     const bool swap = g.out_mode != GEMM_OUT_POOL;
     if (g.dtype == GEMM_T_F8)
         return swap ? dispatch<GEMM_A_CONV3, true, true>(stream, g, cfg, 1) : dispatch<GEMM_A_CONV3, false, true>(stream, g, cfg, 1);
diff --git a/long-term-recurrent-convolutional-nn_amd/csrc/gemm_route.hip b/long-term-recurrent-convolutional-nn_amd/csrc/gemm_route.hip
--- a/long-term-recurrent-convolutional-nn_amd/csrc/gemm_route.hip
+++ b/long-term-recurrent-convolutional-nn_amd/csrc/gemm_route.hip
@@ -29,10 +29,13 @@
     return h;
 }
 static bool bg_fits(const GemmArgs &g) {
-    if (g.bg_cus <= 0 || g.a_mode != GEMM_A_PLAIN || !bg_row_window(g.M) || g.N < kBgMinCols) return false;
+    if (g.bg_cus <= 0 || g.a_mode == GEMM_A_CONV3 || !bg_row_window(g.M) || g.N < kBgMinCols) return false;
     const int64_t b = blocks_8p(bg_args(g));
     return b > 0 && b <= 2 * g.bg_cus;
 }
+
+static bool p8_enabled() { return knob_char("LRCN_GLDS") != '0' && knob_char("LRCN_8P") != '0'; }
+bool gemm_rows_route_ok(const GemmArgs &g) { return p8_enabled() && gemm_8p_rows_ok(g); }
 
 static hipError_t launch_gemm_routed(hipStream_t stream, const GemmArgs &g, const char **route) {
     if (g.dtype == GEMM_T_F8) {
@@ -49,6 +52,16 @@
 
     const int64_t b8 = p8_on ? blocks_8p(g) : 0;
     const bool fills_free = g.free_cus > 0 && b8 * 100 >= (int64_t)g.free_cus * kFree8pMinPct && b8 <= g.free_cus;
+    if (g.a_mode == GEMM_A_ROWS) {
+        if (b8 <= 0) return hipErrorInvalidValue;
+        if (p8 == 'f' || b8 >= 128 || fills_free) { *route = "8p-rows"; return launch_gemm_8p(stream, g); }
+        if (bg_fits(g)) { *route = "8p-rows-bg"; return launch_gemm_8p(stream, bg_args(g)); }
+        int64_t bsk = 0;
+        const int sk = splitk_on ? gemm_8p_splitk(g, &bsk) : 0;
+        if (sk > 1) { *route = "8p-rows-splitk"; return launch_gemm_8p(stream, g, sk); }
+        *route = "8p-rows";
+        return launch_gemm_8p(stream, g);
+    }
     if (b8 > 0 && (p8 == 'f' || b8 >= 128 || fills_free)) { *route = "8p"; return launch_gemm_8p(stream, g); }
     if (p8_on && bg_fits(g)) { *route = "8p-bg"; return launch_gemm_8p(stream, bg_args(g)); }
     if (p8_on && skinny_ok && g.M <= 128) { *route = "skinny"; return launch_gemm_skinny(stream, g); }
diff --git a/long-term-recurrent-convolutional-nn_amd/csrc/lrcn_api.hip b/long-term-recurrent-convolutional-nn_amd/csrc/lrcn_api.hip
--- a/long-term-recurrent-convolutional-nn_amd/csrc/lrcn_api.hip
+++ b/long-term-recurrent-convolutional-nn_amd/csrc/lrcn_api.hip
@@ -10,8 +10,8 @@
 
 constexpr int kBgWgsPerFreeCu = 4;
 
-int lrcn_impl::gemm(lrcn_ctx *c, int dtype, const void *A, int64_t lda, const void *B, int64_t ldb, void *C, int64_t ldc, int M, int N,
-         int K, const float *bias, bool c_f32, bool beta, bool relu, bool c_is_zero, bool on_wg_stream) {
+static GemmArgs gemm_args(const lrcn_ctx *c, int dtype, const void *A, int64_t lda, const void *B, int64_t ldb, void *C, int64_t ldc, int M, int N,
+                          int K, const float *bias, bool c_f32, bool beta, bool relu, bool c_is_zero, bool on_wg_stream) {
     GemmArgs g{};
     g.dtype = dtype;
     g.A = A;
@@ -22,7 +22,7 @@
     g.ldc = ldc;
     g.M = M;
     g.N = N;
-    g.K = gemm_k(dtype, lda, ldb, K);
+    g.K = K;
     g.bias = bias;
     g.c_f32 = c_f32;
     g.beta = beta;
@@ -43,12 +43,41 @@
             if (free_cus >= 8) g.wg_cap = free_cus * kBgWgsPerFreeCu;
         }
     }
+    return g;
+}
+
+int lrcn_impl::gemm(lrcn_ctx *c, int dtype, const void *A, int64_t lda, const void *B, int64_t ldb, void *C, int64_t ldc, int M, int N,
+         int K, const float *bias, bool c_f32, bool beta, bool relu, bool c_is_zero, bool on_wg_stream) {
+    const GemmArgs g = gemm_args(c, dtype, A, lda, B, ldb, C, ldc, M, N, gemm_k(dtype, lda, ldb, K), bias, c_f32, beta, relu, c_is_zero, on_wg_stream);
     hipError_t e = launch_gemm(on_wg_stream ? c->wg_stream : c->stream, g);
     if (e != hipSuccess) FAIL(c, LRCN_EHIP, "gemm M=%d N=%d K=%d: %s", M, N, K, hipGetErrorString(e));
     if (knob_char("LRCN_TRACE_ROUTES") == '1') {
         fprintf(stderr, "gemm M=%d N=%d K=%d %s-> %s\n", M, N, K, on_wg_stream ? "(wg stream) " : "", gemm_debug_last_route());
     }
     return LRCN_OK;
+}
+
+namespace {
+GemmArgs rows_args(const lrcn_ctx *c, const void *A, int64_t lda, int Na, const void *B, int64_t ldb, int Nb, int R, float *C, int64_t ldc,
+                   bool on_wg_stream) {
+    GemmArgs g = gemm_args(c, GEMM_T_BF16, A, lda, B, ldb, C, ldc, Na, Nb, R, nullptr, true, false, false, false, on_wg_stream);
+    g.a_mode = GEMM_A_ROWS;
+    return g;
+}
+int gemm_rows(lrcn_ctx *c, const void *A, int64_t lda, int Na, const void *B, int64_t ldb, int Nb, int R, float *C, int64_t ldc, bool on_wg_stream) {
+    hipStream_t st = on_wg_stream ? c->wg_stream : c->stream;
+    if (R <= 0) {
+        HIPCHK(c, hipMemset2DAsync(C, sizeof(float) * (size_t)ldc, 0, sizeof(float) * (size_t)Nb, (size_t)Na, st));
+        return LRCN_OK;
+    }
+    const GemmArgs g = rows_args(c, A, lda, Na, B, ldb, Nb, R, C, ldc, on_wg_stream);
+    hipError_t e = launch_gemm(st, g);
+    if (e != hipSuccess) FAIL(c, LRCN_EHIP, "gemm over rows Na=%d Nb=%d R=%d: %s", Na, Nb, R, hipGetErrorString(e));
+    if (knob_char("LRCN_TRACE_ROUTES") == '1') {
+        fprintf(stderr, "gemm M=%d N=%d K=%d %s-> %s\n", Na, Nb, R, on_wg_stream ? "(wg stream) " : "", gemm_debug_last_route());
+    }
+    return LRCN_OK;
+}
 }
 
 namespace {
@@ -395,10 +424,27 @@
     if (!bwd) return LRCN_OK;
 
     const int64_t ldM = ld64(M), ldB = ld64(B);
+    bool rows = dt == GEMM_T_BF16 && !((H1 | H2 | X1) & 3);
+    if (rows) {
+        rows = gemm_rows_route_ok(rows_args(c, c->dLog, c->ldV, V, Htop, c->ldH2, H2, M, grads[7], H2, false)) &&
+               gemm_rows_route_ok(rows_args(c, c->dZ1, c->ld4H1, 4 * H1, c->Xemb, c->ldX1, X1, M, grads[0], X1 + H1, false));
+    }
+    if (!rows) {
+        int64_t ra = 4 * (H1 > H2 ? H1 : H2); if (V > ra) ra = V;
+        int64_t rb = 2 * H2; if (X1 + H1 > rb) rb = X1 + H1;
+        if (!c->TA) DALLOC(c, c->TA, es * ra * c->ldM);
+        if (!c->TB) DALLOC(c, c->TB, es * rb * c->ldM);
+        if (knob_char("LRCN_TRACE_ROUTES") == '1') fprintf(stderr, "weight gradients -> transpose_multi\n");
+    }
     auto tr = [&](TrPlan &pl, const void *src, int64_t ld_src, int R, int C, void *dst, int shift) {
         TrDesc &d = pl.d[pl.n++];
         d.src = src; d.ld_src = ld_src; d.R = R; d.C = C; d.dst = dst; d.ld_dst = ldM; d.shift = shift;
     };
+#define GEMM_ROWS(...)                  \
+    do {                                \
+        int _r = gemm_rows(__VA_ARGS__);\
+        if (_r) return _r;              \
+    } while (0)
     hipStream_t sw = par ? c->wg_stream : st;
     int nfork = 0;
     auto fork = [&]() -> int {
@@ -415,13 +461,15 @@
     } while (0)
     auto backward = [&]() -> int {
         FORK();
-        {
+        if (rows) {
+            GEMM_ROWS(c, c->dLog, c->ldV, V, Htop, c->ldH2, H2, M, grads[7], H2, par);
+        } else {
             TrPlan pl{};
             tr(pl, c->dLog, c->ldV, M, V, c->TA, 0);
             tr(pl, Htop, c->ldH2, M, H2, c->TB, 0);
             k_transpose_multi(sw, dt, pl);
-        }
-        GEMM(c, dt, c->TA, ldM, c->TB, ldM, grads[7], H2, V, H2, M, nullptr, true, false, false, false, par);
+            GEMM(c, dt, c->TA, ldM, c->TB, ldM, grads[7], H2, V, H2, M, nullptr, true, false, false, false, par);
+        }
         k_colsum(sw, dt, c->dLog, c->ldV, M, V, grads[8], c->opt_det);
         HIPCHK(c, hipEventRecord(c->grad_ev[0], sw));
         GEMM(c, dt, c->dLog, c->ldV, c->WoT, c->ldV, two ? c->dH2all : c->dH1all, H2, M, H2, V, nullptr, true);
@@ -429,14 +477,18 @@
             r = lstm_layer_bwd(c, S, B, H2, c->ld4H2, c->A2, c->C2, c->dH2all, c->W2hT, c->dZ2);
             if (r) return r;
             FORK();
-            {
+            if (rows) {
+                GEMM_ROWS(c, c->dZ2, c->ld4H2, 4 * H2, c->X2, c->ldH2, H2, M, grads[2], 2 * H2, par);
+                GEMM_ROWS(c, boff(c->dZ2, (int64_t)B * c->ld4H2, es), c->ld4H2, 4 * H2, c->H2all, c->ldH2, H2, M - B,
+                          grads[2] + H2, 2 * H2, par);
+            } else {
                 TrPlan pl{};
                 tr(pl, c->dZ2, c->ld4H2, M, 4 * H2, c->TA, 0);
                 tr(pl, c->X2, c->ldH2, M, H2, c->TB, 0);
                 tr(pl, c->H2all, c->ldH2, M - B, H2, boff(c->TB, (int64_t)H2 * ldM, es), M > B ? B : 0);
                 k_transpose_multi(sw, dt, pl);
+                GEMM(c, dt, c->TA, ldM, c->TB, ldM, grads[2], 2 * H2, 4 * H2, 2 * H2, M, nullptr, true, false, false, false, par);
             }
-            GEMM(c, dt, c->TA, ldM, c->TB, ldM, grads[2], 2 * H2, 4 * H2, 2 * H2, M, nullptr, true, false, false, false, par);
             k_colsum(sw, dt, c->dZ2, c->ld4H2, M, 4 * H2, grads[3], c->opt_det);
         }
         HIPCHK(c, hipEventRecord(c->grad_ev[1], sw));
@@ -444,13 +496,15 @@
             GEMM(c, dt, c->dZ2, c->ld4H2, c->W2xT, c->ld4H2, c->dX2, c->ldH2, M, H2, 4 * H2, nullptr, false);
             k_dx2_mask_reduce(st, dt, c->dX2, c->ldH2, S, B, h, h, d2, c->dxcnn, c->ldh);
             FORK();
-            {
+            if (rows) {
+                GEMM_ROWS(c, c->dX2, c->ldH2, h, c->H1all, c->ldH1, H1, M, grads[4], H1, par);
+            } else {
                 TrPlan pl{};
                 tr(pl, c->dX2, c->ldH2, M, h, c->TA, 0);
                 tr(pl, c->H1all, c->ldH1, M, H1, c->TB, 0);
                 k_transpose_multi(sw, dt, pl);
+                GEMM(c, dt, c->TA, ldM, c->TB, ldM, grads[4], H1, h, H1, M, nullptr, true, false, false, false, par);
             }
-            GEMM(c, dt, c->TA, ldM, c->TB, ldM, grads[4], H1, h, H1, M, nullptr, true, false, false, false, par);
             GEMM(c, dt, c->dX2, c->ldH2, c->WpT, c->ldh, c->dH1all, H1, M, H1, h, nullptr, true);
             k_transpose(sw, dt, 1, c->dxcnn, c->ldh, B, h, c->dxcT, ldB, 0);
             k_cast_rows(sw, dt, feats, B, LRCN_CNNOUT, B, c->FT, ldB);
@@ -460,14 +514,17 @@
         r = lstm_layer_bwd(c, S, B, H1, c->ld4H1, c->A1, c->C1, c->dH1all, c->W1hT, c->dZ1);
         if (r) return r;
         FORK();
-        {
+        if (rows) {
+            GEMM_ROWS(c, c->dZ1, c->ld4H1, 4 * H1, c->Xemb, c->ldX1, X1, M, grads[0], X1 + H1, par);
+            GEMM_ROWS(c, boff(c->dZ1, (int64_t)B * c->ld4H1, es), c->ld4H1, 4 * H1, c->H1all, c->ldH1, H1, M - B, grads[0] + X1, X1 + H1, par);
+        } else {
             TrPlan pl{};
             tr(pl, c->dZ1, c->ld4H1, M, 4 * H1, c->TA, 0);
             tr(pl, c->Xemb, c->ldX1, M, X1, c->TB, 0);
             tr(pl, c->H1all, c->ldH1, M - B, H1, boff(c->TB, (int64_t)X1 * ldM, es), M > B ? B : 0);
             k_transpose_multi(sw, dt, pl);
-        }
-        GEMM(c, dt, c->TA, ldM, c->TB, ldM, grads[0], X1 + H1, 4 * H1, X1 + H1, M, nullptr, true, false, false, false, par);
+            GEMM(c, dt, c->TA, ldM, c->TB, ldM, grads[0], X1 + H1, 4 * H1, X1 + H1, M, nullptr, true, false, false, false, par);
+        }
         k_colsum(sw, dt, c->dZ1, c->ld4H1, M, 4 * H1, grads[1], c->opt_det);
         HIPCHK(c, hipEventRecord(c->grad_ev[3], sw));
         GEMM(c, dt, c->dZ1, c->ld4H1, c->W1xT, c->ld4H1, c->dXemb, c->ldX1, M, X1, 4 * H1, nullptr, true);
@@ -512,6 +569,7 @@
     }
     if (r) return r;
 #undef FORK
+#undef GEMM_ROWS
     KCHK(c, "backward");
     return LRCN_OK;
 }
@@ -847,9 +905,6 @@
         const int Hm = H1 > H2 ? H1 : H2;
         DALLOC(c, c->dhrec, sizeof(float) * B * Hm); DALLOC(c, c->dc, sizeof(float) * B * Hm);
         DALLOC(c, c->dxcnn, sizeof(float) * B * c->ldh); DALLOC(c, c->dxcT, es * h * c->ldB);
-        int64_t ra = 4 * Hm; if (V > ra) ra = V;
-        int64_t rb = 2 * H2; if (X1 + H1 > rb) rb = X1 + H1;
-        DALLOC(c, c->TA, es * ra * c->ldM);        DALLOC(c, c->TB, es * rb * c->ldM);
         DALLOC(c, c->logp, sizeof(double) * 2);
         DALLOC(c, c->zero_page, 256);
         if (hipMemset(c->zero_page, 0, 256) != hipSuccess) return LRCN_EHIP;
```

Measured after the change: 37370. About the same (-0.4%).
